# lucadellalib/audiocodecs

Hardware: AMD Instinct MI355X
Metric: encode+decode audio-sec/s, EnCodec-24k 8cb (higher is better)
Workload: dtype f32 (GEMM-shaped kernels and LSTM products: operands as two scaled fp16 planes, 3 partial products, fp32 accumulate -- split16.h)

## Files before the change

audiocodecs_amd/csrc/ac_api.hip:

```cpp
#include "core.h"
#include "tap_route.h"

extern "C" {

int ac_version(void) { return 400; }

int ac_create(const ac_config* cfg, ac_handle** out) {
    if (!cfg || !out) return AC_EINVAL;
    *out = nullptr;
    if (cfg->struct_size != (int32_t)sizeof(ac_config)) return AC_EINVAL;
    if (cfg->num_ratios < 1 || cfg->num_ratios > AC_MAX_RATIOS || cfg->num_filters < 1 || cfg->hidden_size < 16 ||
        cfg->hidden_size % 16 || cfg->compress < 1 || cfg->num_lstm_layers < 1 || cfg->num_lstm_layers > 2 || cfg->codebook_size % 32 ||
        cfg->codebook_size < 16 || cfg->num_quantizers < 1 || cfg->kernel_size < 1 || cfg->kernel_size > 8 ||
        cfg->last_kernel_size < 1 || cfg->last_kernel_size > 8 || cfg->residual_kernel_size < 1 || cfg->residual_kernel_size > 8)
        return AC_EINVAL;
    int ndev = 0;
    if (hipGetDeviceCount(&ndev) != hipSuccess || ndev <= cfg->device || cfg->device < 0) return AC_ENODEV;
    ac_handle* h = new (std::nothrow) ac_handle();
    if (!h) return AC_ENOMEM;
    h->cfg = *cfg;
    h->hop = 1;
    for (int i = 0; i < cfg->num_ratios; ++i) h->hop *= cfg->upsampling_ratios[i];
    h->D = cfg->num_filters << cfg->num_ratios;
    *out = h;
    return AC_OK;
}







static std::string wavtok_key(const std::string& name) {
    static const std::string pre = "feature_extractor.encodec.encoder.model.";
    if (name.compare(0, pre.size(), pre) != 0) return name;
    std::string k = "encoder.layers." + name.substr(pre.size());
    const size_t cc = k.find(".conv.conv.");
    if (cc != std::string::npos) k = k.substr(0, cc) + ".conv." + k.substr(cc + 11);
    auto ends = [&](const char* sfx) { const size_t n = std::strlen(sfx); return k.size() >= n && k.compare(k.size() - n, n, sfx) == 0; };
    if (ends(".weight_g")) k = k.substr(0, k.size() - 9) + ".parametrizations.weight.original0";
    else if (ends(".weight_v")) k = k.substr(0, k.size() - 9) + ".parametrizations.weight.original1";
    return k;
}

int ac_load_weights(ac_handle* h, const char* name, const void* host_ptr, size_t bytes) {
    if (!h || !name || !host_ptr) return h ? fail(h, AC_EINVAL, "null argument") : AC_EINVAL;
    if (h->finalized) return fail(h, AC_ESTATE, "handle already finalized");
    if (bytes % 4) return fail(h, AC_EINVAL, "tensor '%s': byte size %zu is not a multiple of 4", name, bytes);
    const float* f = static_cast<const float*>(host_ptr);
    h->host[h->arch == ARCH_WAVTOK ? wavtok_key(name) : std::string(name)].assign(f, f + bytes / 4);
    return AC_OK;
}



static void latch_dev_switches(ac_handle* h) {
    auto num = [](const char* name, int dflt) { const char* v = std::getenv(name); return v && *v ? std::atoi(v) : dflt; };
    const char* e = std::getenv("AC_TAP_EPI");
    h->dev.tap_epi_staged = e && std::strcmp(e, "staged") == 0;
    h->dev.tap_dil = num("AC_TAP_DIL", 1);
    h->dev.tap_stagger = num("AC_TAP_STAGGER", 0);
    h->dev.tap_pick = num("AC_TAP_PICK", -1);
    h->dev.tap8 = num("AC_TAP8", -1);
    h->dev.tap8_form = num("AC_TAP8_FORM", 0);
    h->dev.tap8_spread = num("AC_TAP8_SPREAD", 1);
#ifdef AC_DEVELOPER
    h->dev.rb6_dbg = num("AC_RB6_DBG", 0);
    h->dev.lstm_dbg = num("AC_LSTM_DBG", 0);
#endif
    h->dev.rb_stream = num("AC_RB_STREAM", 1);
    h->dev.chain_stream = num("AC_CHAIN_STREAM", 1);
    h->dev.rb128_stream = num("AC_RB128_STREAM", 1);
    h->dev.rb256_fused = num("AC_RB256_FUSED", 1);
    h->dev.front_seg = std::max(0, num("AC_FRONT_SEG", 0));
    h->dev.tail_seg = std::max(0, num("AC_TAIL_SEG", 0));
    h->dev.front_ldspad = std::max(0, num("AC_FRONT_LDSPAD", 0));
    h->dev.lstm_fuse_in = num("AC_LSTM_FUSE_IN", 1);
    const char* r = std::getenv("AC_RVQ");
    h->dev.rvq_exact = r && std::strcmp(r, "fp32") == 0;
    h->dev.prof_detail = num("AC_PROF_DETAIL", 0);
    h->dev.head_seq = num("AC_HEAD_SEQ", 0);
    h->dev.attn_exact = num("AC_ATTN_EXACT", 0);
    h->dev.dac_unit = num("AC_DAC_UNIT", 1);
    h->dev.mimi_tail = num("AC_MIMI_TAIL", 1);
    h->dev.mstream_skinny = num("AC_MSTREAM_SKINNY", -1);
}

int ac_debug_set(ac_handle* h, const char* key, int value) {
    if (!h || !key) return AC_EINVAL;
    struct { const char* k; int* v; } tab[] = {
        {"tap_epi_staged", &h->dev.tap_epi_staged}, {"tap_dil", &h->dev.tap_dil}, {"tap_stagger", &h->dev.tap_stagger}, {"tap_pick", &h->dev.tap_pick}, {"tap8", &h->dev.tap8}, {"tap8_form", &h->dev.tap8_form}, {"tap8_spread", &h->dev.tap8_spread},
        {"rb6_dbg", &h->dev.rb6_dbg}, {"rb_stream", &h->dev.rb_stream}, {"chain_stream", &h->dev.chain_stream}, {"rb128_stream", &h->dev.rb128_stream}, {"rb256_fused", &h->dev.rb256_fused}, {"front_seg", &h->dev.front_seg}, {"tail_seg", &h->dev.tail_seg}, {"front_ldspad", &h->dev.front_ldspad},
        {"lstm_dbg", &h->dev.lstm_dbg}, {"lstm_fuse_in", &h->dev.lstm_fuse_in}, {"rvq_exact", &h->dev.rvq_exact}, {"prof_detail", &h->dev.prof_detail}, {"head_seq", &h->dev.head_seq}, {"attn_exact", &h->dev.attn_exact}, {"dac_unit", &h->dev.dac_unit}, {"mimi_tail", &h->dev.mimi_tail},
        {"mstream_skinny", &h->dev.mstream_skinny},
    };
#ifndef AC_DEVELOPER
    if (std::strcmp(key, "rb6_dbg") == 0 || std::strcmp(key, "lstm_dbg") == 0)
        return fail(h, AC_EINVAL, "ac_debug_set('%s'): a developer-build switch (timing modes with wrong results / fault injection); this is the product library", key);
#endif
    if (!h->finalized) return fail(h, AC_ESTATE, "ac_debug_set('%s'): the switches are latched by ac_finalize; set them afterwards", key);
    for (auto& t : tab)
        if (std::strcmp(t.k, key) == 0) {
            const bool nonneg = t.v == &h->dev.front_seg || t.v == &h->dev.tail_seg || t.v == &h->dev.front_ldspad || t.v == &h->dev.tap_stagger;
            if (nonneg && value < 0) return fail(h, AC_EINVAL, "ac_debug_set('%s', %d): the value must be >= 0", key, value);
            if (t.v == &h->dev.front_ldspad && value > 16384) return fail(h, AC_EINVAL, "ac_debug_set('front_ldspad', %d): at most 16384 bytes", value);
            if (t.v == &h->dev.tap8_form && (value < 0 || value > 5)) return fail(h, AC_EINVAL, "ac_debug_set('tap8_form', %d): 0 (cost model) .. 5", value);
            *t.v = value;
            return AC_OK;
        }
    return fail(h, AC_EINVAL, "ac_debug_set: unknown switch '%s'", key);
}

int ac_set_precision(ac_handle* h, int precision) {
    if (!h) return AC_EINVAL;
    if (h->finalized) return fail(h, AC_ESTATE, "ac_set_precision must precede ac_finalize (weights are packed for one arithmetic)");
    if (precision != AC_PRECISION_FP32 && precision != AC_PRECISION_FP32_EXACT) return fail(h, AC_EINVAL, "unknown precision %d", precision);
    h->precision = precision;
    return AC_OK;
}

int ac_finalize(ac_handle* h) {
    if (!h) return AC_EINVAL;
    if (h->finalized) return fail(h, AC_ESTATE, "handle already finalized");
    {
        int pr = h->precision;
        if (pr < 0) {
            const char* gm = std::getenv("AC_GEMM");
            if (gm && *gm && std::strcmp(gm, "fp32") != 0 && std::strcmp(gm, "split16") != 0)
                return fail(h, AC_EINVAL, "AC_GEMM=%s: unknown arithmetic (fp32 = exact fp32 products, split16 or unset = the default)", gm);
            pr = gm && std::strcmp(gm, "fp32") == 0 ? AC_PRECISION_FP32_EXACT : AC_PRECISION_FP32;
        }
        const char* fz = std::getenv("AC_FUSE");
        h->fuse_chains = !(fz && fz[0] == '0');
        latch_dev_switches(h);
        h->gemm_fp32 = pr == AC_PRECISION_FP32_EXACT;
    }
    if (h->arch == ARCH_MIMI) {
        Packer pk{h};
        if (int rc = mimi_finalize(h, pk)) return rc;
        return upload_blob(h, pk, h->mcfg.device);
    }
    if (h->arch == ARCH_DAC) {
        Packer pk{h};
        if (int rc = dac_finalize(h, pk)) return rc;
        return upload_blob(h, pk, h->dcfg.device);
    }
    if (h->arch == ARCH_WAVTOK) {
        Packer pk{h};
        if (int rc = wavtok_finalize(h, pk)) return rc;
        return upload_blob(h, pk, h->wcfg.device);
    }
    if (h->arch == ARCH_SPK) {
        Packer pk{h};
        if (int rc = spk_finalize(h, pk)) return rc;
        return upload_blob(h, pk, h->scfg.device);
    }
    if (h->arch == ARCH_LM) {
        Packer pk{h};
        if (int rc = lm_finalize(h, pk)) return rc;
        return upload_blob(h, pk, h->lcfg.device);
    }
    const ac_config& c = h->cfg;
    Arch a = make_arch(c);
    Packer pk{h};
    h->has_enc = h->has_dec = false;
    for (const auto& kv : h->host) {
        if (kv.first.compare(0, 8, "encoder.") == 0) h->has_enc = true;
        if (kv.first.compare(0, 8, "decoder.") == 0) h->has_dec = true;
    }
    bool has_q = false;
    for (const auto& kv : h->host) has_q = has_q || kv.first.compare(0, 10, "quantizer.") == 0;
    if (!h->has_enc && !h->has_dec && !has_q) return fail(h, AC_ESTATE, "no encoder.*, decoder.* or quantizer.* tensor was loaded");
    bool ok = true;
    h->enc_rb.resize(c.num_ratios);
    h->enc_down.resize(c.num_ratios);
    h->dec_up.resize(c.num_ratios);
    h->dec_rb.resize(c.num_ratios);
    if (h->has_enc) {
        ok = pk.conv(a.enc_stem, h->enc_stem);
        for (int i = 0; ok && i < c.num_ratios; ++i) {
            ok = ok && pk.resblock(a.enc_rb3[i], a.enc_rb1[i], a.enc_rbs[i], h->enc_rb[i]);
            ok = ok && pk.conv(a.enc_down[i], h->enc_down[i]);
        }
        ok = ok && pk.lstm(a.enc_lstm, a.D, c.num_lstm_layers, h->enc_lstm);
        ok = ok && pk.conv(a.enc_final, h->enc_final);
        if (ok) pk.chain_bounds(h->enc_stem, h->enc_rb[0], h->enc_down[0], h->enc_front);
        if (ok) pk.stream_enc(h->enc_stem, h->enc_rb[0], h->enc_down[0], h->simg);
    }
    if (h->has_dec) {
        ok = ok && pk.conv(a.dec_first, h->dec_first);
        ok = ok && pk.lstm(a.dec_lstm, a.D, c.num_lstm_layers, h->dec_lstm);
        for (int i = 0; ok && i < c.num_ratios; ++i) {
            ok = ok && pk.convtr(a.dec_up[i], h->dec_up[i]);
            ok = ok && pk.resblock(a.dec_rb3[i], a.dec_rb1[i], a.dec_rbs[i], h->dec_rb[i]);
        }
        ok = ok && pk.conv(a.dec_head, h->dec_head);
        if (ok) pk.tail_bounds(h->dec_up[c.num_ratios - 1], h->dec_rb[c.num_ratios - 1], h->dec_head, h->dec_tail);
        if (ok) pk.stream_dec(h->dec_up[c.num_ratios - 1], h->dec_rb[c.num_ratios - 1], h->dec_head, h->simg);
    }
    if (!ok) return pk.rc;
    const int C = c.codebook_size, H = c.hidden_size, Q = c.num_quantizers;
    h->cb_plain = pk.reserve((size_t)Q * C * H);
    h->cb_packed = pk.reserve((size_t)Q * C * H);
    h->cb_ee = pk.reserve((size_t)Q * C);
    for (int q = 0; q < Q; ++q) {
        const std::vector<float>* e = pk.get("quantizer.layers." + std::to_string(q) + ".codebook.embed", (size_t)C * H);
        if (!e) return pk.rc;
        std::copy(e->begin(), e->end(), pk.blob.begin() + h->cb_plain + (size_t)q * C * H);
        for (int code = 0; code < C; ++code) {
            double ss = 0.0;
            for (int d = 0; d < H; ++d) ss += (double)(*e)[(size_t)code * H + d] * (*e)[(size_t)code * H + d];
            pk.blob[h->cb_ee + (size_t)q * C + code] = (float)ss;
        }
        const int HV = H / 16;
        for (int ct = 0; ct < C / 16; ++ct)
            for (int v = 0; v < HV; ++v)
                for (int lane = 0; lane < 64; ++lane)
                    for (int u = 0; u < 4; ++u)
                        pk.blob[h->cb_packed + (size_t)q * C * H + (((size_t)ct * HV + v) * 64 + lane) * 4 + u] =
                            (*e)[(size_t)(ct * 16 + (lane & 15)) * H + v * 16 + 4 * (lane >> 4) + u];
    }
    if (pk.use16() && H % 32 == 0 && H / 16 == 8) pk.pack_cb16(h->cb_plain, Q, C, H, &h->cb16, &h->cb16_inv);
    return upload_blob(h, pk, c.device);
}

int ac_num_frames(const ac_handle* h, int T) {
    if (!h || T < 1) return AC_EINVAL;
    if (h->arch == ARCH_MIMI) return cdiv(mimi_num_frames25(h->mcfg, T), h->mcfg.resample_stride);
    if (h->arch == ARCH_DAC) return dac_num_frames(h->dcfg, T);
    long long L = T;
    for (int r = h->cfg.num_ratios - 1; r >= 0; --r) L = (L + h->cfg.upsampling_ratios[r] - 1) / h->cfg.upsampling_ratios[r];
    return (int)L;
}
long long ac_num_samples(const ac_handle* h, int N) {
    if (!h || N < 1) return AC_EINVAL;
    return h->arch == ARCH_DAC ? dac_num_samples(h->dcfg, N) : (long long)N * h->hop;
}
int ac_hop_length(const ac_handle* h) { return h ? h->hop : AC_EINVAL; }
int ac_hidden_size(const ac_handle* h) {
    if (!h) return AC_EINVAL;
    return h->arch == ARCH_MIMI ? h->mcfg.hidden_size : h->arch == ARCH_DAC ? h->dac.H : h->cfg.hidden_size;
}
int ac_codebook_dim(const ac_handle* h) {
    if (!h) return AC_EINVAL;
    return h->arch == ARCH_MIMI ? h->mcfg.codebook_dim : h->arch == ARCH_DAC ? DAC_CODE_DIM : h->cfg.hidden_size;
}
// ... 524 lines not shown
```

audiocodecs_amd/csrc/core.h:

```cpp
#pragma once
#include <hip/hip_runtime.h>

#include <algorithm>
#include <cmath>
#include <cstdarg>
#include <cstdio>
#include <cstdlib>
#include <cstring>
#include <map>
#include <string>
#include <vector>

#include "../../include/audiocodecs_amd.h"
#include "lstm_consts.h"
#include "rvq_types.h"
#include "split16.h"
#include "tap_gemm.h"

using namespace ac;

namespace ac {
constexpr int THIN_MAXK = 8;
struct RbFused6Params;
}

namespace acimpl {


struct ConvSpec {
    std::string prefix;
    int transposed, cin, cout, k, s;
};

struct PackedGemm {
    size_t w_off = 0, b_off = 0;
    int N = 0, Ktot = 0;
    bool has_bias = true;
};

struct ResBlockPlan {
    int C;
    PackedGemm c3;
    PackedGemm fused;
    size_t w3f_off = 0, wff_off = 0;
    size_t winv3_off = 0, winvf_off = 0;
    size_t w3p_off = 0, wfp_off = 0;
    float hb0 = 0.f, hb1 = 0.f;
    bool has6 = false;
    bool hb256 = false;
};

struct LstmPlan {
    int D, layers;
    std::vector<PackedGemm> ih;
    std::vector<size_t> hh_off;
    std::vector<size_t> ihpk_off;
    size_t persist_off = 0;
    size_t persist16_off = 0;
    size_t persist16_inv = 0;
    bool has_persist = false;
};

struct MimiTfLayer {
    PackedGemm qkv, o, fc1, fc2;
    size_t ln1_w = 0, ln1_b = 0, ln2_w = 0, ln2_b = 0, sc_a = 0, sc_m = 0;
};

struct MimiPlan {
    PackedGemm enc_stem, enc_final, down, dec_first, dec_head;
    std::vector<ResBlockPlan> enc_rb, dec_rb;
    std::vector<PackedGemm> enc_down, dec_up;
    std::vector<MimiTfLayer> enc_tf, dec_tf;
    size_t up_w = 0;
    PackedGemm in_proj;
    PackedGemm out_proj;
    size_t cb_plain = 0, cb_packed = 0, cb_ee = 0;
    size_t cb16 = 0, cb16_inv = 0;
    size_t rope_cos = 0, rope_sin = 0;
    int rope_T = 0;
    int D = 0;
    struct StreamM { size_t stem_f = 0, stem_inv = 0, head_f = 0, head_inv = 0; float sb0 = 0.f, sb1 = 0.f, fb0 = 0.f, fb1h = 0.f; bool stem_ok = false, head_ok = false; } sm;
};

struct DacResUnitPlan {
    PackedGemm c7, c1;
    size_t a1 = 0, a1i = 0, a2 = 0, a2i = 0;
    int dil = 1;
};

struct DacBlockPlan {
    int C = 0, stride = 1;
    std::vector<DacResUnitPlan> ru;
    size_t a = 0, ai = 0;
    PackedGemm conv;
};

struct DacPlan {
    PackedGemm enc_stem, enc_final, dec_first, dec_head, in_proj0;
    std::vector<DacBlockPlan> enc, dec;
    size_t enc_a = 0, enc_ai = 0, dec_a = 0, dec_ai = 0;
    size_t win = 0, bin = 0, wout = 0, bout = 0, cb = 0, cbn = 0, c2 = 0, proj = 0;
    int H = 0;
};

struct WtResnetPlan {
    size_t n1w = 0, n1b = 0, n2w = 0, n2b = 0;
    PackedGemm c1, c2;
};
struct WtCnxPlan {
    size_t dww = 0, dwb = 0, sc = 0, sh = 0, gamma = 0;
    PackedGemm p1, p2;
};
struct WavtokPlan {
    PackedGemm embed, qkv, proj, head, istft;
    WtResnetPlan rn[4];
    size_t an_w = 0, an_b = 0;
    size_t g5w = 0, g5b = 0;
    size_t nsc = 0, nsh = 0;
    size_t flw = 0, flb = 0;
    size_t w2 = 0;
    std::vector<WtCnxPlan> cnx;
    int bins = 0, npad = 0, hop_pad = 0, taps = 0;
    bool vocos = false;
    int tables = 1;
};

struct SpkTfLayer {
    PackedGemm qkv, o, fc1, fc2;
    size_t ln1_w = 0, ln1_b = 0, ln2_w = 0, ln2_b = 0;
    size_t gate_w = 0, gate_b = 0, gate_c = 0;
};

struct SpkPlan {
    size_t stem_w = 0, gn_w = 0, gn_b = 0;
    std::vector<PackedGemm> conv;
    size_t fp_ln_w = 0, fp_ln_b = 0, enc_ln_w = 0, enc_ln_b = 0;
    PackedGemm fp;
    size_t pos_img = 0, pos_inv = 0, pos_b = 0;
    std::vector<SpkTfLayer> tf;
    size_t bias_tab = 0;
    int R = 0;
    std::vector<float> lw;
    PackedGemm proj, fe;
    std::vector<PackedGemm> tdnn;
    int shrink = 0;
};

struct LmLayer {
    size_t an = 0, fn = 0, wqkv = 0, wo = 0, w1 = 0, w3 = 0, w2 = 0;
};

struct LmPlan {
    size_t emb = 0, prompt = 0, norm = 0, head = 0;
    size_t rope_cos = 0, rope_sin = 0;
    std::vector<LmLayer> layers;
};

struct ProfRec {
    int name_id;
    int count;
    hipEvent_t e0, e1;
    double flops, bytes;
};


}
using namespace acimpl;

enum { ARCH_ENCODEC = 0, ARCH_MIMI = 1, ARCH_DAC = 2, ARCH_WAVTOK = 3, ARCH_SPK = 4, ARCH_LM = 5 };

struct ac_handle {
    int arch = ARCH_ENCODEC;
    ac_config cfg{};
    ac_mimi_config mcfg{};
    MimiPlan mimi;
    ac_dac_config dcfg{};
    DacPlan dac;
    ac_wavtok_config wcfg{};
    WavtokPlan wt;
    ac_spk_config scfg{};
    SpkPlan spk;
    ac_lm_config lcfg{};
    LmPlan lm;
    std::string err;
    std::map<std::string, std::vector<float>> host;
    bool finalized = false;
    float* blob = nullptr;
    size_t blob_floats = 0;
    int hop = 1, D = 0;
    PackedGemm enc_stem, enc_final;
    std::vector<ResBlockPlan> enc_rb;
    std::vector<PackedGemm> enc_down;
    LstmPlan enc_lstm, dec_lstm;
    PackedGemm dec_first, dec_head;
    std::vector<PackedGemm> dec_up;
    std::vector<ResBlockPlan> dec_rb;
    size_t cb_plain = 0, cb_packed = 0, cb_ee = 0;
    size_t cb16 = 0, cb16_inv = 0;
    struct ChainBounds { float sb0 = 0.f, sb1 = 0.f, fb0 = 0.f, fb1h = 0.f, fb1x = 0.f; bool ok = false; } enc_front, dec_tail;
    struct StreamImgs { size_t stem_f = 0, stem_inv = 0, down_f = 0, down_inv = 0, up_f = 0, up_inv = 0, head_f = 0, head_inv = 0; bool enc_ok = false, dec_ok = false; } simg;
    struct DevSwitches {
        int tap_epi_staged = 0;
        int tap_dil = 1;
        int tap_stagger = 0;
        int tap_pick = -1;
        int tap8 = -1;
        int tap8_form = 0;
        int tap8_spread = 1;
        int rb6_dbg = 0;
        int rb_stream = 1;
        int rb256_fused = 1;
        int rb128_stream = 1;
        int chain_stream = 1;
        int front_seg = 0, tail_seg = 0;
        int front_ldspad = 0;
        int lstm_dbg = 0;
        int lstm_fuse_in = 1;
        int rvq_exact = 0;
        int prof_detail = 0;
        int attn_exact = 0;
        int dac_unit = 1;
        int mimi_tail = 1;
        int head_seq = 0;
        int mstream_skinny = -1;
    } dev;
    bool fuse_chains = true;
    float* dbg = nullptr;
    size_t dbg_cap = 0, dbg_used = 0;
    std::vector<const void*> lds_opted;
    std::map<size_t, size_t> w6_of;
    std::map<size_t, size_t> t6_of;
    std::map<size_t, size_t> t6inv_of;
    bool noncausal = false;
    bool has_enc = true, has_dec = true;
    bool gemm_fp32 = false;
    std::map<size_t, size_t> winv_of;
    std::map<const void*, int> mimi_streams;
    std::map<const void*, int> mimi_dstreams;
    struct EStreamReg {
        int B;
        std::vector<uint8_t> fresh;
    };
    std::map<const void*, EStreamReg> encodec_streams, encodec_dstreams;
    unsigned* amax_buf = nullptr;
    int amax_B = 0, amax_next = 0;
    unsigned* row_buf = nullptr;
    size_t row_cap = 0, row_next = 0;
    void* own_pool = nullptr;
    size_t own_pool_rows = 0;
    int precision = -1;
    unsigned* lp_ctl = nullptr;
    int num_cus = 0;
    bool lstm_step_only = false;
    unsigned long long* clk_dev = nullptr;
    unsigned* sticky = nullptr;
    unsigned* sticky_dev = nullptr;
    bool prof = false;
    bool prof_detail = false;
    std::vector<ProfRec> recs;
    std::vector<std::string> prof_names;
    std::vector<hipEvent_t> ev_pool;
    size_t ev_used = 0;
};

namespace acimpl {

int fail(ac_handle* h, int code, const char* fmt, ...);


#define HIPCHK(h, call)                                                                         \
    do {                                                                                        \
        hipError_t e_ = (call);                                                                 \
        if (e_ != hipSuccess) return fail(h, AC_EHIP, "%s failed: %s", #call, hipGetErrorString(e_)); \
    } while (0)


inline int cdiv(int a, int b) { return (a + b - 1) / b; }

int ensure_lds(ac_handle* h, const void* func, size_t bytes);

inline size_t align_up(size_t v, size_t a) { return (v + a - 1) / a * a; }


struct Arch {
    std::vector<ConvSpec> enc_rb3, enc_rb1, enc_rbs, enc_down;
    ConvSpec enc_stem, enc_final, dec_first, dec_head;
    std::vector<ConvSpec> dec_up, dec_rb3, dec_rb1, dec_rbs;
    std::string enc_lstm, dec_lstm;
    int D;
};

Arch make_arch(const ac_config& c);


struct Packer {
    ac_handle* h;
    std::vector<float> blob;
    int rc = AC_OK;

    const std::vector<float>* get(const std::string& name, size_t n) {
        auto it = h->host.find(name);
        if (it == h->host.end()) {
            rc = fail(h, AC_ESTATE, "missing tensor '%s'", name.c_str());
            return nullptr;
        }
        if (it->second.size() != n) {
            rc = fail(h, AC_EINVAL, "tensor '%s' has %zu elements, expected %zu", name.c_str(), it->second.size(), n);
            return nullptr;
        }
        return &it->second;
    }
    bool weight(const ConvSpec& s, std::vector<float>& w) {
        const size_t n = (size_t)s.cin * s.cout * s.k;
        auto it = h->host.find(s.prefix + ".weight");
        if (it != h->host.end()) {
            if (it->second.size() != n) {
                rc = fail(h, AC_EINVAL, "tensor '%s.weight' has %zu elements, expected %zu", s.prefix.c_str(), it->second.size(), n);
                return false;
            }
            w = it->second;
            return true;
        }
        const int d0 = s.transposed ? s.cin : s.cout;
        const std::vector<float>* g = get(s.prefix + ".parametrizations.weight.original0", d0);
        if (!g) return false;
        const std::vector<float>* v = get(s.prefix + ".parametrizations.weight.original1", n);
        if (!v) return false;
        w.resize(n);
        const size_t inner = n / d0;
        for (int i = 0; i < d0; ++i) {
            double ss = 0.0;
            for (size_t j = 0; j < inner; ++j) ss += (double)(*v)[i * inner + j] * (*v)[i * inner + j];
            const float scale = (*g)[i] / (float)std::sqrt(ss);
            for (size_t j = 0; j < inner; ++j) w[i * inner + j] = (*v)[i * inner + j] * scale;
        }
        return true;
    }
    size_t reserve(size_t n) {
        const size_t off = align_up(blob.size(), 64);
        blob.resize(off + n, 0.f);
        return off;
    }
    static uint16_t bf16_rn(float v) {
        uint32_t b;
        std::memcpy(&b, &v, 4);
        if ((b & 0x7f800000u) == 0x7f800000u) return (uint16_t)(b >> 16);
        return (uint16_t)((b + 0x7fffu + ((b >> 16) & 1u)) >> 16);
    }
    static uint16_t f16_rn(float f) {
        uint32_t x;
        std::memcpy(&x, &f, 4);
        const uint16_t sign = (uint16_t)((x >> 16) & 0x8000u);
        x &= 0x7fffffffu;
        if (x >= 0x7f800000u) return (uint16_t)(sign | 0x7c00u | (x > 0x7f800000u ? 0x200u : 0u));
        if (x >= 0x477ff000u) return (uint16_t)(sign | 0x7c00u);
        if (x <= 0x33000000u) return sign;
        const int e = (int)(x >> 23) - 127;
        const uint32_t m = (x & 0x7fffffu) | 0x800000u;
        const int shift = e >= -14 ? 13 : 13 + (-14 - e);
        uint32_t q = m >> shift;
        const uint32_t rem = m & ((1u << shift) - 1u), half = 1u << (shift - 1);
        if (rem > half || (rem == half && (q & 1u))) ++q;
        if (e >= -14) return (uint16_t)(sign | (uint16_t)(((uint32_t)(e + 15) << 10) + (q - 0x400u)));
        return (uint16_t)(sign | (uint16_t)q);
    }
    static float f16_f32(uint16_t hbits) {
        const int e = (hbits >> 10) & 31, m = hbits & 0x3ff;
        float v;
        if (e == 0) v = std::ldexp((float)m, -24);
        else if (e == 31) v = m ? NAN : INFINITY;
// ... 223 lines not shown
            for (int k = 0; k < 7; ++k) k7[k] = k;
            sm.stem_f = frag16(stem.w_off, 64, 7, k7, &sm.stem_inv);
            sm.sb0 = sm.sb1 = 0.f;
            for (int n = 0; n < 64; ++n) {
                double l1 = 0.0;
                for (int k = 0; k < 7; ++k) l1 += std::fabs((double)blob[stem.w_off + (size_t)n * 7 + k]);
                sm.sb1 = std::max(sm.sb1, (float)(l1 * 1.000001));
                sm.sb0 = std::max(sm.sb0, std::fabs(blob[stem.b_off + n]));
            }
            sm.stem_ok = true;
        }
        if (head.N == 1 && head_k >= 1 && head_k <= 8 && head.Ktot == head_k * 64 && head.has_bias && dec_rb.C == 64 && dec_rb.w3p_off && dec_rb.fused.Ktot == 32) {
            std::vector<int> kh(64);
            for (int k = 0; k < 64; ++k) kh[k] = k;
            const size_t pad = reserve(16 * 64);
            for (int i = 0; i < 16 * 64; ++i) blob[pad + i] = i < head_k * 64 ? blob[head.w_off + i] : 0.f;
            sm.head_f = frag16(pad, 16, 64, perm32(kh), &sm.head_inv);
            sm.fb0 = sm.fb1h = 0.f;
            for (int n = 0; n < 64; ++n) {
                double lh = 0.0;
                for (int k = 0; k < 32; ++k) lh += std::fabs((double)blob[dec_rb.fused.w_off + (size_t)n * 32 + k]);
                sm.fb1h = std::max(sm.fb1h, (float)(lh * 1.000001));
                sm.fb0 = std::max(sm.fb0, std::fabs(blob[dec_rb.fused.b_off + n]));
            }
            sm.head_ok = true;
        }
    }
    void stream_enc(const PackedGemm& stem, const ResBlockPlan& rb, const PackedGemm& down, ac_handle::StreamImgs& si) {
        si.enc_ok = false;
        if (!use16() || !h->enc_front.ok || !rb.w3p_off || stem.N != 32 || stem.Ktot != 7 || down.N != 64 || down.Ktot != 128) return;
        std::vector<int> k7(32, -1), kd(128);
        for (int k = 0; k < 7; ++k) k7[k] = k;
        for (int k = 0; k < 128; ++k) kd[k] = k;
        si.stem_f = frag16(stem.w_off, 32, 7, k7, &si.stem_inv);
        si.down_f = frag16(down.w_off, 64, 128, perm32(kd), &si.down_inv);
        si.enc_ok = true;
    }
    void stream_dec(const PackedGemm& up, const ResBlockPlan& rb, const PackedGemm& head, ac_handle::StreamImgs& si) {
        si.dec_ok = false;
        if (!use16() || !h->dec_tail.ok || !rb.w3p_off || up.N != 64 || up.Ktot != 128 || head.N != 1 || head.Ktot != 7 * 32) return;
        std::vector<int> ku(128), kh(32);
        for (int k = 0; k < 128; ++k) ku[k] = k;
        for (int k = 0; k < 32; ++k) kh[k] = k;
        si.up_f = frag16(up.w_off, 64, 128, perm32(ku), &si.up_inv);
        const size_t pad = reserve(16 * 32);
        for (int i = 0; i < 16 * 32; ++i) blob[pad + i] = i < 7 * 32 ? blob[head.w_off + i] : 0.f;
        si.head_f = frag16(pad, 16, 32, perm32(kh), &si.head_inv);
        si.dec_ok = true;
    }
    void chain_bounds(const PackedGemm& stem, const ResBlockPlan& rb, const PackedGemm& down, ac_handle::ChainBounds& cb) {
        cb.ok = false;
        if (!use16() || !rb.has6 || !rb.winv3_off || rb.C != 32 || stem.N != 32 || !h->t6inv_of.count(down.w_off)) return;
        const int hid = rb.C / 2;
        cb.sb0 = cb.sb1 = cb.fb0 = cb.fb1h = cb.fb1x = 0.f;
        for (int n = 0; n < stem.N; ++n) {
            double l1 = 0.0;
            for (int k = 0; k < stem.Ktot; ++k) l1 += std::fabs((double)blob[stem.w_off + (size_t)n * stem.Ktot + k]);
            cb.sb1 = std::max(cb.sb1, (float)(l1 * 1.000001));
            cb.sb0 = std::max(cb.sb0, std::fabs(blob[stem.b_off + n]));
        }
        for (int n = 0; n < rb.C; ++n) {
            double lh = 0.0, lx = 0.0;
            for (int k = 0; k < hid; ++k) lh += std::fabs((double)blob[rb.fused.w_off + (size_t)n * rb.fused.Ktot + k]);
            for (int k = hid; k < rb.fused.Ktot; ++k) lx += std::fabs((double)blob[rb.fused.w_off + (size_t)n * rb.fused.Ktot + k]);
            cb.fb1h = std::max(cb.fb1h, (float)(lh * 1.000001));
            cb.fb1x = std::max(cb.fb1x, (float)(lx * 1.000001));
            cb.fb0 = std::max(cb.fb0, std::fabs(blob[rb.fused.b_off + n]));
        }
        cb.ok = true;
    }
    void tail_bounds(const PackedGemm& up, const ResBlockPlan& rb, const PackedGemm& head, ac_handle::ChainBounds& cb) {
        cb.ok = false;
        if (!use16() || !rb.has6 || !rb.winv3_off || rb.C != 32 || up.N != 64 || up.Ktot != 128 || !h->t6inv_of.count(up.w_off) || head.N != 1 || head.Ktot != 7 * 32) return;
        cb.sb0 = cb.sb1 = 0.f;
        for (int n = 0; n < up.N; ++n) {
            double l1 = 0.0;
            for (int k = 0; k < up.Ktot; ++k) l1 += std::fabs((double)blob[up.w_off + (size_t)n * up.Ktot + k]);
            cb.sb1 = std::max(cb.sb1, (float)(l1 * 1.000001));
            cb.sb0 = std::max(cb.sb0, std::fabs(blob[up.b_off + n]));
        }
        const int hid = rb.C / 2;
        cb.fb0 = cb.fb1h = cb.fb1x = 0.f;
        for (int n = 0; n < rb.C; ++n) {
            double lh = 0.0, lx = 0.0;
            for (int k = 0; k < hid; ++k) lh += std::fabs((double)blob[rb.fused.w_off + (size_t)n * rb.fused.Ktot + k]);
            for (int k = hid; k < rb.fused.Ktot; ++k) lx += std::fabs((double)blob[rb.fused.w_off + (size_t)n * rb.fused.Ktot + k]);
            cb.fb1h = std::max(cb.fb1h, (float)(lh * 1.000001));
            cb.fb1x = std::max(cb.fb1x, (float)(lx * 1.000001));
            cb.fb0 = std::max(cb.fb0, std::fabs(blob[rb.fused.b_off + n]));
        }
        cb.ok = true;
    }
    bool lstm(const std::string& prefix, int D, int layers, LstmPlan& lp) {
        lp.D = D;
        lp.layers = layers;
        for (int l = 0; l < layers; ++l) {
            const std::string sfx = "_l" + std::to_string(l);
            const std::vector<float>* wih = get(prefix + ".weight_ih" + sfx, (size_t)4 * D * D);
            const std::vector<float>* whh = get(prefix + ".weight_hh" + sfx, (size_t)4 * D * D);
            const std::vector<float>* bih = get(prefix + ".bias_ih" + sfx, (size_t)4 * D);
            const std::vector<float>* bhh = get(prefix + ".bias_hh" + sfx, (size_t)4 * D);
            if (!wih || !whh || !bih || !bhh) return false;
            PackedGemm g;
            g.N = 4 * D;
            g.Ktot = D;
            g.w_off = reserve((size_t)4 * D * D);
            std::copy(wih->begin(), wih->end(), blob.begin() + g.w_off);
            g.b_off = reserve((size_t)4 * D);
            for (int n = 0; n < 4 * D; ++n) blob[g.b_off + n] = (*bih)[n] + (*bhh)[n];
            if (l == 0) pack6(g);
            lp.ih.push_back(g);
            const size_t off = reserve((size_t)4 * D * D);
            for (int ug = 0; ug < D / 4; ++ug)
                for (int ks = 0; ks < D / 16; ++ks)
                    for (int lane = 0; lane < 64; ++lane)
                        for (int u = 0; u < 4; ++u) {
                            const int j = lane & 15, kq = lane >> 4;
                            const int row = (j >> 2) * D + ug * 4 + (j & 3);
                            const int k = ks * 16 + 4 * kq + u;
                            blob[off + (((size_t)ug * (D / 16) + ks) * 64 + lane) * 4 + u] = (*whh)[(size_t)row * D + k];
                        }
            lp.hh_off.push_back(off);
            const size_t off2 = reserve((size_t)4 * D * D);
            for (int ug = 0; ug < D / 4; ++ug)
                for (int ks = 0; ks < D / 16; ++ks)
                    for (int lane = 0; lane < 64; ++lane)
                        for (int u = 0; u < 4; ++u) {
                            const int j = lane & 15, kq = lane >> 4;
                            const int row = (j >> 2) * D + ug * 4 + (j & 3);
                            const int k = ks * 16 + 4 * kq + u;
                            blob[off2 + (((size_t)ug * (D / 16) + ks) * 64 + lane) * 4 + u] = (*wih)[(size_t)row * D + k];
                        }
            lp.ihpk_off.push_back(off2);
        }
        if (D == LP_D && layers == 2) {
            const std::vector<float>* mats[3] = {get(prefix + ".weight_hh_l0", (size_t)4 * D * D), get(prefix + ".weight_ih_l1", (size_t)4 * D * D),
                                                 get(prefix + ".weight_hh_l1", (size_t)4 * D * D)};
            const size_t mat = (size_t)LP_SLICES * 4 * 4 * 8 * 256;
            lp.persist_off = reserve(3 * mat);
            for (int m = 0; m < 3; ++m)
                for (int idx = 0; idx < LP_SLICES; ++idx)
                    for (int w = 0; w < 4; ++w)
                        for (int n = 0; n < 4; ++n)
                            for (int ks = 0; ks < 8; ++ks)
                                for (int lane = 0; lane < 64; ++lane)
                                    for (int e = 0; e < 4; ++e)
                                        blob[lp.persist_off + m * mat + ((((size_t)idx * 4 + w) * 4 + n) * 8 + ks) * 256 + lane * 4 + e] =
                                            (*mats[m])[(size_t)(n * D + idx * 16 + (lane & 15)) * D + (w * 8 + ks) * 16 + 4 * (lane >> 4) + e];
            const std::vector<float>* mats6[4] = {mats[0], mats[1], mats[2], get(prefix + ".weight_ih_l0", (size_t)4 * D * D)};
            if (use16()) {
                const size_t mat16 = (size_t)LP_SLICES * 4 * 4 * 4 * 2 * 512;
                lp.persist16_off = reserve((4 * mat16 + 1) / 2);
                lp.persist16_inv = reserve((size_t)2 * 4 * D);
                std::vector<int> sc((size_t)2 * 4 * D);
                const int layer_of[4] = {0, 1, 1, 0};
                for (int l = 0; l < 2; ++l)
                    for (int row = 0; row < 4 * D; ++row) {
                        uint32_t mx = 0;
                        for (int m = 0; m < 4; ++m)
                            if (layer_of[m] == l)
                                for (int k = 0; k < D; ++k) {
                                    uint32_t b;
                                    std::memcpy(&b, &(*mats6[m])[(size_t)row * D + k], 4);
                                    mx = std::max(mx, b & 0x7fffffffu);
                                }
                        sc[(size_t)l * 4 * D + row] = s16_exponent(mx, 40);
                        blob[lp.persist16_inv + (size_t)l * 4 * D + row] = s16_pow2(-sc[(size_t)l * 4 * D + row]);
                    }
                std::vector<uint16_t> pl16(4 * mat16);
                for (int m = 0; m < 4; ++m)
                    for (int idx = 0; idx < LP_SLICES; ++idx)
                        for (int w = 0; w < 4; ++w)
                            for (int n = 0; n < 4; ++n)
                                for (int ks = 0; ks < 4; ++ks)
                                    for (int lane = 0; lane < 64; ++lane)
                                        for (int e = 0; e < 8; ++e) {
                                            const int row = n * D + idx * 16 + (lane & 15);
                                            uint16_t t[3];
                                            split16h((*mats6[m])[(size_t)row * D + w * 128 + ks * 32 + 8 * (lane >> 4) + e], sc[(size_t)layer_of[m] * 4 * D + row], t);
                                            const size_t base = m * mat16 + (((((size_t)idx * 4 + w) * 4 + n) * 4 + ks) * 2) * 512 + (size_t)lane * 8 + e;
                                            pl16[base] = t[0];
                                            pl16[base + 512] = t[1];
                                        }
                std::memcpy(&blob[lp.persist16_off], pl16.data(), pl16.size() * 2);
            }
            lp.has_persist = true;
        }
        return true;
    }
};


struct Act {
    const float* p;
    long long bs, ts;
    int L, C;
    const unsigned* amax = nullptr;
    int amax_n = 0;
};

int prof_name(ac_handle* h, const char* nm);

hipEvent_t next_event(ac_handle* h);


struct ProfScope {
    ac_handle* h;
    hipStream_t st;
    ProfRec r{};
    bool on;
    ProfScope(ac_handle* h_, hipStream_t st_, const char* nm, double flops, double bytes, int count = 1)
        : h(h_), st(st_), on(h_->prof) {
        if (!on) return;
        r.name_id = prof_name(h, nm);
        r.count = count;
        r.flops = flops;
        r.bytes = bytes;
        r.e0 = next_event(h);
        r.e1 = next_event(h);
        (void)hipEventRecord(r.e0, st);
    }
    ~ProfScope() {
        if (!on) return;
        (void)hipEventRecord(r.e1, st);
        h->recs.push_back(r);
    }
};


constexpr int AMAX_SLOTS = 512;

inline size_t pool_bytes(int pool_B, size_t rows) {
    return (size_t)AMAX_SLOTS * std::max(pool_B, 1) * AMAX_STRIDE * 4 + 8 * align_up(std::max<size_t>(rows, 64), 64) * 4 + 256;
}

void pool_bind(ac_handle* h, void* mem, int pool_B, size_t rows);

int amax_begin(ac_handle* h, hipStream_t st, int B);

unsigned* amax_new(ac_handle* h);

const unsigned* amax_of(ac_handle* h, hipStream_t st, const float* x, long long bs, long long ts, int L, int C, int B, const unsigned* known);

unsigned* rowmax_new(ac_handle* h, hipStream_t st, long long rows, bool zero);

const unsigned* amax_plus(ac_handle* h, hipStream_t st, const Act& x, float add, int B);

TapSeg make_seg(const Act& x, int s, int J, int pad , int extra, int kofs, const float* rel_len, int left = -1, int right = 0);


inline bool aligned16(const void* p) { return (reinterpret_cast<uintptr_t>(p) & 15) == 0; }

int run_tap(ac_handle* h, hipStream_t st, TapGemmParams& p);


struct Out {
    float* raw = nullptr;
    float* elu = nullptr;
};

struct Act2 {
    Act raw{}, elu{};
};

int try_thin6(ac_handle* h, hipStream_t st, const PackedGemm& g, const Act& x, int width, int edge, Out out, int B, const unsigned** amax_out = nullptr);

int conv_fwd(ac_handle* h, hipStream_t st, const PackedGemm& g, const Act& x, int k, int s, const float* rel_len, Out out,
             long long out_bs, long long out_rs, int B, Act2* y);

int convtr_fwd(ac_handle* h, hipStream_t st, const PackedGemm& g, const Act& x, int s, Out out, int B, Act2* y);

bool rb128_ok(const ac_handle* h, const ResBlockPlan& rb);

int resblock_fwd(ac_handle* h, hipStream_t st, const ResBlockPlan& rb, const Act2& x, float* hbuf, Out out, int B, Act2* y);
bool rb256_ok(const ac_handle* h, const ResBlockPlan& rb, int L);

bool thin_ok(const ac_config& c, int k);

int thin_stem(ac_handle* h, hipStream_t st, const PackedGemm& g, int F, int k, int pad, const float* sig, const float* rel_len, int B, int T,
              Out out, Act2* y, int padl = -1, const float* alpha = nullptr, const float* alpha_inv = nullptr, int Lp = -1);

int stem_fwd(ac_handle* h, hipStream_t st, const float* sig, const float* rel_len, int B, int T, Out out, Act2* y);

int thin_head(ac_handle* h, hipStream_t st, const PackedGemm& g, int F, int k, int pad, const Act& x, int B, float* sig, int padl = -1,
              int tanh_out = 0);

int head_fwd(ac_handle* h, hipStream_t st, const Act& x, int B, float* sig);

bool enc_front_ok(const ac_handle* h, int T);

int enc_front_fwd(ac_handle* h, hipStream_t st, const float* sig, const float* rel_len, int B, int T, float* y, float* dbg_x0, float* dbg_y1, Act2* out);

bool dec_tail_ok(const ac_handle* h, const Act& xe);

int dec_tail_fwd(ac_handle* h, hipStream_t st, const Act& xe, int B, float* sig, float* dbg_u, float* dbg_v);

void capture(ac_handle* h, hipStream_t st, const Act& a, int B);


struct LstmWs {
    float *gin, *gin1, *hseq0, *hseq1, *c;
};

int lstm_fwd(ac_handle* h, hipStream_t st, const LstmPlan& lp, const Act& x, const LstmWs& ws, Out out, int B, Act2* y);

int rvq_encode_fwd(ac_handle* h, hipStream_t st, const float* feats, int F, int K, long long* toks);

int rvq_decode_fwd(ac_handle* h, hipStream_t st, const long long* toks, int F, int K, float* out);


constexpr int NACT = 6;


struct Workspace {
    size_t act_floats = 0;
    size_t gin = 0, hseq = 0, c = 0;
    int pool_B = 0;
    size_t pool_rows = 0;
    size_t total_bytes = 0;
};

inline void add_pool(Workspace& w, int pool_B, size_t rows) {
    w.pool_B = pool_B;
    w.pool_rows = rows;
    w.total_bytes += pool_bytes(pool_B, rows);
}

Workspace plan_ws(const ac_handle* h, int B, int T_in , int N_frames , bool enc);


struct WsPtrs {
    float* act[NACT];
    bool used[NACT];
    LstmWs lstm;
    float* take() {
        for (int i = 0; i < NACT; ++i)
            if (!used[i]) { used[i] = true; return act[i]; }
        return nullptr;
    }
    void give(const float* p) {
        for (int i = 0; i < NACT; ++i)
            if (act[i] == p) used[i] = false;
    }
    void give(const Act2& a) { give(a.raw.p); give(a.elu.p); }
};

int carve(ac_handle* h, const Workspace& w, void* ws, size_t ws_bytes, WsPtrs* o);

int check_ready(ac_handle* h);

int check_len(ac_handle* h, long long samples);

int encoder_fwd(ac_handle* h, hipStream_t st, const float* sig, const float* rel_len, int B, int T, float* feats, WsPtrs& ws);

int decoder_fwd(ac_handle* h, hipStream_t st, const long long* toks, int B, int N, int K, float* sig, WsPtrs& ws);

bool rb64_identity_head_fwd(ac_handle* h, hipStream_t st, const ResBlockPlan& rb, const Act2& x, const PackedGemm& head, int head_k, float* sig, int B, int* rc);
int enc_stream_fwd(ac_handle* h, hipStream_t st, const float* sig, const float* rel_len, int B, int T, float* y, float* dbg_x0, float* dbg_y1, const unsigned* amax_sig, unsigned* amax_out);
int dec_stream_fwd(ac_handle* h, hipStream_t st, const Act& xe, int B, float* sig, float* dbg_u, float* dbg_v, const unsigned* amax_x);
int launch_rb_stream6m(ac_handle* h, hipStream_t st, const ResBlockPlan& rb, const float* xr, const float* sig, int B, int L, Out out, float* head_y, int head_k,
                       const unsigned* amax_in, unsigned* amax_out);
int launch_rb_stream128m(ac_handle* h, hipStream_t st, RbFused6Params& p, const ResBlockPlan& rb, bool sc, Out out, int B);
int launch_rb_stream6(ac_handle* h, hipStream_t st, RbFused6Params& p, const ResBlockPlan& rb, bool sc, Out out, int B);
int rb64_identity_fwd(ac_handle* h, hipStream_t st, const ResBlockPlan& rb, const Act2& x, Out out, int B, const unsigned** amax_out);
int rb128_identity_fwd(ac_handle* h, hipStream_t st, const ResBlockPlan& rb, const Act2& x, Out out, int B, const unsigned** amax_out);
int rvq_encode_cdist_launch(ac_handle* h, hipStream_t st, const RvqEncParams& p, unsigned blocks, const _Float16* epk16 = nullptr, const float* einv = nullptr);
void rvq_decode_launch(hipStream_t st, const RvqDecParams& p, unsigned blocks);
void amax_fill_launch(hipStream_t st, unsigned* slot, unsigned bits, int B);
int resample_launch(const float* x, int B, int L, const float* kern, int n, int o, int taps, int width, float* y, int L_out, hipStream_t st);
constexpr int RSTREAM_MAX_TAPS = 8192;
long long resample_stream_groups(long long total, int o, int width);
long long resample_stream_out_len(long long consumed, int L, int n, int o, int width, int finish);
size_t resample_stream_state_bytes(int B, int taps);
int resample_stream_reset_launch(void* state, int B, int n, int o, int taps, int width, hipStream_t st);
int resample_stream_push_launch(void* state, const float* x, long long x_pitch, int B, int L, long long consumed, const float* kern, int n, int o, int taps,
                                int width, float* y, long long y_pitch, int m, int finish, hipStream_t st);
int resample_stream_reset_slots_launch(void* state, int B, int n, int o, int taps, int width, const int* slots_dev, int rows, hipStream_t st);
int resample_stream_push_slots_launch(void* state, int B, const int* slots_dev, const long long* consumed_dev, int rows, const float* x, long long x_pitch,
                                      int L, const float* kern, int n, int o, int taps, int width, float* y, long long y_pitch, int m, int finish,
                                      hipStream_t st);

struct Epi {
    const float* scale = nullptr;
    const float* res = nullptr;
    long long res_bs = 0, res_rs = 0;
    int gelu = 0;
    const unsigned* rowmax_in = nullptr;
    const unsigned** rowmax_out = nullptr;
};

int mimi_finalize(ac_handle* h, Packer& pk);
Workspace mimi_plan_ws(const ac_handle* h, int B, int T_in, int N_frames, bool enc);
int mimi_num_frames25(const ac_mimi_config& c, long long T);
int mimi_encoder_fwd(ac_handle* h, hipStream_t st, const float* sig, int B, int T, float* feats, WsPtrs& ws);
int mimi_decoder_fwd(ac_handle* h, hipStream_t st, const float* qfeats, int B, int N, float* sig, WsPtrs& ws);
int mimi_linear(ac_handle* h, hipStream_t st, const PackedGemm& g, const float* x, long long rows, int cin, int x_pitch, int kofs,
                float* y, int y_pitch, const Epi& epi = Epi{});
int layernorm_fwd(ac_handle* h, hipStream_t st, const float* x, size_t w_off, size_t b_off, float* y, long long rows, int H, float eps,
                  const unsigned** rows_out = nullptr);
int mimi_rvq_encode(ac_handle* h, hipStream_t st, const float* proj, int F, int K, long long* toks);
int mimi_rvq_decode(ac_handle* h, hipStream_t st, const long long* toks, int F, int K, float* qsum, float* qfeats);
int dac_finalize(ac_handle* h, Packer& pk);
Workspace dac_plan_ws(const ac_handle* h, int B, long long T_in, long long N_frames, bool enc);
int dac_chunk_clips(const ac_handle* h, int B, long long T_in, long long N_frames, bool enc);
int dac_num_frames(const ac_dac_config& c, long long T);
long long dac_num_samples(const ac_dac_config& c, long long N);
int dac_encoder_fwd(ac_handle* h, hipStream_t st, const float* sig, int B, int T, float* z, WsPtrs& ws);
int dac_decoder_fwd(ac_handle* h, hipStream_t st, const float* zq, int B, int N, float* sig, WsPtrs& ws);
int dac_latent_proj(ac_handle* h, hipStream_t st, const float* z, int N, int nb, float* zlat);
int dac_vq_encode(ac_handle* h, hipStream_t st, const float* z, int F, int K, long long* toks, float* qsum);
int dac_from_codes(ac_handle* h, hipStream_t st, const long long* toks, int F, int K, float* zq);
int wavtok_finalize(ac_handle* h, Packer& pk);
Workspace wavtok_plan_ws(const ac_handle* h, int B, int T_in, int N_frames, bool enc);
int wavtok_decoder_fwd(ac_handle* h, hipStream_t st, const float* feats, int B, int N, float* sig, WsPtrs& ws);
int spk_finalize(ac_handle* h, Packer& pk);
int lm_finalize(ac_handle* h, Packer& pk);
int upload_blob(ac_handle* h, Packer& pk, int device);
constexpr int DAC_CODE_DIM = 8;

}
```

audiocodecs_amd/csrc/core.hip:

```cpp
#include "core.h"
#include "split16_kernels.h"
#include "lstm.h"
#include "lstm_persist.h"
#include "lstm_persist16.h"
#include "rvq.h"
#include "rvq16.h"
#include "tap_gemm4.h"
#include "tap_gemm6.h"
#include "tap_gemm8.h"
#include "tap_route.h"
#include "thin.h"
#include "rb_fused.h"
#include "rb_fused6.h"
#include "thin_conv6.h"
#include "rb_fused6_128.h"
#include "rb256_fused.h"
#include "enc_front.h"
#include "dec_tail.h"

namespace acimpl {


int fail(ac_handle* h, int code, const char* fmt, ...) {
    char buf[1024];
// ... 56 lines not shown


int prof_name(ac_handle* h, const char* nm) {
    for (size_t i = 0; i < h->prof_names.size(); ++i)
        if (h->prof_names[i] == nm) return (int)i;
    h->prof_names.push_back(nm);
    return (int)h->prof_names.size() - 1;
}


hipEvent_t next_event(ac_handle* h) {
    if (h->ev_used == h->ev_pool.size()) {
        hipEvent_t e;
        (void)hipEventCreate(&e);
        h->ev_pool.push_back(e);
    }
    return h->ev_pool[h->ev_used++];
}

void pool_bind(ac_handle* h, void* mem, int pool_B, size_t rows) {
    h->amax_buf = reinterpret_cast<unsigned*>(mem);
    h->amax_B = mem ? std::max(pool_B, 1) : 0;
    h->amax_next = 0;
    h->row_buf = mem ? h->amax_buf + (size_t)AMAX_SLOTS * h->amax_B * AMAX_STRIDE : nullptr;
    h->row_cap = mem ? 8 * align_up(std::max<size_t>(rows, 64), 64) : 0;
    h->row_next = 0;
}


static void zero_words(hipStream_t st, unsigned* p, size_t words) {
    const size_t n16 = words / 4;
    const unsigned grid = (unsigned)std::min<size_t>(std::max<size_t>((n16 + 255) / 256, 1), 2048);
    hipLaunchKernelGGL(zero16_kernel, dim3(grid), dim3(256), 0, st, reinterpret_cast<s16_f32x4*>(p), n16);
}


int amax_begin(ac_handle* h, hipStream_t st, int B) {
    h->amax_next = 0;
    if (h->gemm_fp32 || !h->amax_buf) return AC_OK;
    if (B > h->amax_B) return fail(h, AC_ENOMEM, "workspace pool holds amax slots for %d clips, the pass has %d", h->amax_B, B);
    zero_words(st, h->amax_buf, (size_t)AMAX_SLOTS * h->amax_B * AMAX_STRIDE);
    HIPCHK(h, hipGetLastError());
    return AC_OK;
}

unsigned* amax_new(ac_handle* h) {
    if (h->gemm_fp32 || !h->amax_buf || h->amax_next >= AMAX_SLOTS) return nullptr;
    return h->amax_buf + (size_t)(h->amax_next++) * h->amax_B * AMAX_STRIDE;
}

const unsigned* amax_of(ac_handle* h, hipStream_t st, const float* x, long long bs, long long ts, int L, int C, int B, const unsigned* known) {
    if (known) return known;
    if (B > h->amax_B) return nullptr;
    unsigned* slot = amax_new(h);
    if (!slot) return nullptr;
    const long long n = (long long)L * C;
    const int gx = (int)std::max<long long>(1, std::min<long long>((n / 4 + 256 * 8 - 1) / (256 * 8), std::max(4, 8192 / std::max(1, B))));
    ProfScope ps(h, st, "amax_kernel", 0.0, (double)B * n * 4.0);
    hipLaunchKernelGGL(amax_kernel, dim3(gx, B), dim3(256), 0, st, x, bs, ts, L, C, slot);
    return slot;
}


unsigned* rowmax_new(ac_handle* h, hipStream_t st, long long rows, bool zero) {
    const size_t need = ((size_t)rows + 63) / 64 * 64;
    if (!h->row_buf || need > h->row_cap) return nullptr;
    if (h->row_next + need > h->row_cap) h->row_next = 0;
    unsigned* r = h->row_buf + h->row_next;
    h->row_next += need;
    if (zero) {
        zero_words(st, r, need);
        if (hipGetLastError() != hipSuccess) return nullptr;
    }
    return r;
}


const unsigned* amax_plus(ac_handle* h, hipStream_t st, const Act& x, float add, int B) {
    if (!x.amax || x.amax_n != B) return nullptr;
    unsigned* slot = amax_new(h);
    if (!slot) return nullptr;
    hipLaunchKernelGGL(amax_add_kernel, dim3(cdiv(B, 64)), dim3(64), 0, st, x.amax, add, slot, B);
    return slot;
}



template <int WGM, int WGN, int WM, int WN>
static int launch_tap(ac_handle* h, hipStream_t st, TapGemmParams p, TapFamily f, const char* name, double flops, double bytes) {
    ProfScope ps(h, st, name, flops, bytes);
    if (f == TapFamily::tap4) {
        using Cfg = Tap4Cfg<WGM, WGN, WM, WN>;
        p.mtiles = cdiv(p.M, Cfg::BM);
        p.ntiles = cdiv(p.N, Cfg::BN);
        if (int rc = ensure_lds(h, reinterpret_cast<const void*>(tap_gemm4_kernel<WGM, WGN, WM, WN>), Cfg::lds_bytes)) return rc;
        const long long blocks = (long long)p.B * p.mtiles * p.ntiles;
        hipLaunchKernelGGL((tap_gemm4_kernel<WGM, WGN, WM, WN>), dim3((unsigned)blocks), dim3(Cfg::NT), Cfg::lds_bytes, st, p);
        return AC_OK;
    }
    constexpr int BM = WGM * WM * 16, BN = WGN * WN * 16;
    p.mtiles = cdiv(p.M, BM);
    p.ntiles = cdiv(p.N, BN);
    const size_t lds = tap_gemm_lds_bytes<WGM, WGN, WM, WN>();
    const long long blocks = (long long)p.B * p.mtiles * p.ntiles;
    if (f == TapFamily::vec) hipLaunchKernelGGL((tap_gemm_kernel<WGM, WGN, WM, WN, true>), dim3((unsigned)blocks), dim3(WGM * WGN * 64), lds, st, p);
    else hipLaunchKernelGGL((tap_gemm_kernel<WGM, WGN, WM, WN, false>), dim3((unsigned)blocks), dim3(WGM * WGN * 64), lds, st, p);
    return AC_OK;
}

static int launch_tap_fp32(ac_handle* h, hipStream_t st, const TapGemmParams& p, const TapRoute& r, const char* name, double flops, double bytes) {
    switch (r.key()) {
    case tap_key(4, 1, 2, 1): return launch_tap<4, 1, 2, 1>(h, st, p, r.family, name, flops, bytes);
    case tap_key(4, 1, 2, 2): return launch_tap<4, 1, 2, 2>(h, st, p, r.family, name, flops, bytes);
    case tap_key(2, 2, 2, 2): return launch_tap<2, 2, 2, 2>(h, st, p, r.family, name, flops, bytes);
    case tap_key(2, 2, 4, 3): return launch_tap<2, 2, 4, 3>(h, st, p, r.family, name, flops, bytes);
    case tap_key(2, 2, 4, 4): return launch_tap<2, 2, 4, 4>(h, st, p, r.family, name, flops, bytes);
    }
    return fail(h, AC_EINVAL, "run_tap: no instantiation of %s", r.name);
}

template <int WGM, int WGN, int WMT, int WN, int HALO>
static int launch_tap6(ac_handle* h, hipStream_t st, TapGemmParams& p, const __bf16* w6, const char* name, double flops, double bytes) {
    using Cfg = Tap6Cfg<WGM, WGN, WMT, WN, HALO>;
    p.mtiles = cdiv(p.M, Cfg::BM);
    p.ntiles = p.N / Cfg::BN;
    const long long blocks = (long long)p.B * p.mtiles * p.ntiles;
    if (int rc = ensure_lds(h, reinterpret_cast<const void*>(tap_gemm6_kernel<WGM, WGN, WMT, WN, 2, HALO>), Cfg::lds_for(2))) return rc;
    ProfScope ps(h, st, name, flops, bytes);
    hipLaunchKernelGGL((tap_gemm6_kernel<WGM, WGN, WMT, WN, 2, HALO>), dim3((unsigned)blocks), dim3(Cfg::NT), Cfg::lds_for(2), st, p, w6);
    return AC_OK;
}

static int launch_tap6_family(ac_handle* h, hipStream_t st, TapGemmParams& p, const TapRoute& r, const __bf16* w6, const char* name, double flops, double bytes) {
    if (r.family == TapFamily::tap6_dil) {
        switch (r.key()) {
        case tap_key(1, 4, 4, 2): return launch_tap6<1, 4, 4, 2, T6_DIL_HALO>(h, st, p, w6, name, flops, bytes);
        case tap_key(1, 4, 4, 1): return launch_tap6<1, 4, 4, 1, T6_DIL_HALO>(h, st, p, w6, name, flops, bytes);
        case tap_key(2, 2, 2, 3): return launch_tap6<2, 2, 2, 3, T6_DIL_HALO>(h, st, p, w6, name, flops, bytes);
        case tap_key(4, 1, 1, 3): return launch_tap6<4, 1, 1, 3, T6_DIL_HALO>(h, st, p, w6, name, flops, bytes);
        }
    } else {
        switch (r.key()) {
        case tap_key(1, 4, 4, 2): return launch_tap6<1, 4, 4, 2, 7>(h, st, p, w6, name, flops, bytes);
        case tap_key(1, 8, 4, 1): return launch_tap6<1, 8, 4, 1, 7>(h, st, p, w6, name, flops, bytes);
        case tap_key(1, 4, 4, 1): return launch_tap6<1, 4, 4, 1, 7>(h, st, p, w6, name, flops, bytes);
        case tap_key(2, 2, 2, 3): return launch_tap6<2, 2, 2, 3, 7>(h, st, p, w6, name, flops, bytes);
        case tap_key(4, 1, 1, 3): return launch_tap6<4, 1, 1, 3, 7>(h, st, p, w6, name, flops, bytes);
        case tap_key(2, 2, 2, 1): return launch_tap6<2, 2, 2, 1, 7>(h, st, p, w6, name, flops, bytes);
        }
    }
    return fail(h, AC_EINVAL, "run_tap: no instantiation of %s", r.name);
}

template <int WGM, int WGN, int WMT, int WN, bool RM, bool J1, bool SP>
static int launch_tap8(ac_handle* h, hipStream_t st, TapGemmParams& p, const __bf16* w6, const char* name, double flops, double bytes) {
    using Cfg = Tap8Cfg<WGM, WGN, WMT, WN>;
    p.mtiles = cdiv(p.M, Cfg::BM);
    p.ntiles = p.N / Cfg::BN;
    const long long blocks = (long long)p.B * p.mtiles * p.ntiles;
    ProfScope ps(h, st, name, flops, bytes);
    if (int rc = ensure_lds(h, reinterpret_cast<const void*>(tap_gemm8_kernel<WGM, WGN, WMT, WN, RM, J1, SP>), Cfg::lds_bytes)) return rc;
    hipLaunchKernelGGL((tap_gemm8_kernel<WGM, WGN, WMT, WN, RM, J1, SP>), dim3((unsigned)blocks), dim3(Cfg::NT), Cfg::lds_bytes, st, p, w6);
    return AC_OK;
}

static int launch_tap8_family(ac_handle* h, hipStream_t st, TapGemmParams& p, const TapRoute& r, const __bf16* w6, const char* name, double flops, double bytes) {
    constexpr int RJ = TK_RM | TK_J1, J = TK_J1, S = TK_SPREAD;
    switch (r.key()) {
    case tap_key(2, 4, 4, 2, RJ): return launch_tap8<2, 4, 4, 2, true, true, false>(h, st, p, w6, name, flops, bytes);
    case tap_key(2, 4, 4, 2, RJ | S): return launch_tap8<2, 4, 4, 2, true, true, true>(h, st, p, w6, name, flops, bytes);
    case tap_key(2, 4, 4, 2, J): return launch_tap8<2, 4, 4, 2, false, true, false>(h, st, p, w6, name, flops, bytes);
    case tap_key(2, 4, 4, 2, J | S): return launch_tap8<2, 4, 4, 2, false, true, true>(h, st, p, w6, name, flops, bytes);
    case tap_key(2, 4, 4, 2): return launch_tap8<2, 4, 4, 2, false, false, false>(h, st, p, w6, name, flops, bytes);
    case tap_key(2, 4, 4, 2, S): return launch_tap8<2, 4, 4, 2, false, false, true>(h, st, p, w6, name, flops, bytes);
    case tap_key(2, 4, 2, 2, RJ): return launch_tap8<2, 4, 2, 2, true, true, false>(h, st, p, w6, name, flops, bytes);
    case tap_key(2, 4, 2, 2, RJ | S): return launch_tap8<2, 4, 2, 2, true, true, true>(h, st, p, w6, name, flops, bytes);
    case tap_key(2, 4, 2, 2, J): return launch_tap8<2, 4, 2, 2, false, true, false>(h, st, p, w6, name, flops, bytes);
    case tap_key(2, 4, 2, 2, J | S): return launch_tap8<2, 4, 2, 2, false, true, true>(h, st, p, w6, name, flops, bytes);
    case tap_key(2, 4, 2, 2): return launch_tap8<2, 4, 2, 2, false, false, false>(h, st, p, w6, name, flops, bytes);
    case tap_key(2, 4, 2, 2, S): return launch_tap8<2, 4, 2, 2, false, false, true>(h, st, p, w6, name, flops, bytes);
    case tap_key(4, 2, 2, 2, RJ): return launch_tap8<4, 2, 2, 2, true, true, false>(h, st, p, w6, name, flops, bytes);
    case tap_key(4, 2, 2, 2, RJ | S): return launch_tap8<4, 2, 2, 2, true, true, true>(h, st, p, w6, name, flops, bytes);
    case tap_key(4, 2, 2, 2, J): return launch_tap8<4, 2, 2, 2, false, true, false>(h, st, p, w6, name, flops, bytes);
    case tap_key(4, 2, 2, 2, J | S): return launch_tap8<4, 2, 2, 2, false, true, true>(h, st, p, w6, name, flops, bytes);
    case tap_key(4, 2, 2, 2): return launch_tap8<4, 2, 2, 2, false, false, false>(h, st, p, w6, name, flops, bytes);
    case tap_key(4, 2, 2, 2, S): return launch_tap8<4, 2, 2, 2, false, false, true>(h, st, p, w6, name, flops, bytes);
    }
    return fail(h, AC_EINVAL, "run_tap: no instantiation of %s", r.name);
}


TapSeg make_seg(const Act& x, int s, int J, int pad , int extra, int kofs, const float* rel_len, int left, int right) {
    TapSeg g{};
    g.x = x.p;
    g.amax = x.amax;
    g.amax_n = x.amax_n;
    g.bs = x.bs;
    g.ts = x.ts;
    g.rel_len = rel_len;
    g.L = x.L;
    g.cin = x.C;
    g.cin_shift = -1;
    for (int sh = 0; sh < 30; ++sh)
        if ((1 << sh) == x.C) g.cin_shift = sh;
    g.s = s;
    g.J = J;
    const int pad_left = left < 0 ? (J - 1) * s : left;
    const int max_pad = std::max(pad_left, right + extra);
    g.Lp = (pad == PAD_REFLECT && x.L <= max_pad) ? max_pad + 1 : x.L;
    g.lim = pad != PAD_ZERO ? x.L + right + extra : x.L;
    g.reflect = pad;
    g.elu = 0;
    g.kofs = kofs;
    g.pad = pad_left;
    g.dil = 1;
    return g;
}


int run_tap(ac_handle* h, hipStream_t st, TapGemmParams& p) {
    const auto w6_it = h->w6_of.find((size_t)(p.w - h->blob));
    const auto iv = h->winv_of.find((size_t)(p.w - h->blob));
    TapRouteInputs in;
    in.w6 = w6_it != h->w6_of.end();
    in.winv = iv != h->winv_of.end();
    in.want_rowmode = p.amax_rows != 0;
    in.want_rows = p.amax_out_rows != nullptr;
    in.gemm_fp32 = h->gemm_fp32;
    const TapRoute r = route_tap(p, in, h->dev);
    if (r.reject_taps) return fail(h, AC_EINVAL, "conv with %d taps exceeds the kernel limit of 8", r.reject_taps);
    double kk = 0, inb = 0;
    for (int i = 0; i < p.nseg; ++i) {
        kk += (double)p.seg[i].J * p.seg[i].s * p.seg[i].cin;
        inb += (double)p.B * p.seg[i].L * p.seg[i].cin * 4.0;
    }
    const double flops = 2.0 * p.B * (double)p.M * p.N * kk;
    const double bytes = inb + (double)p.B * p.M * p.N * 4.0 * ((p.y ? 1 : 0) + (p.y_elu ? 1 : 0)) + (double)p.N * p.Ktot * 4.0;
    std::string name = r.name;
    if (h->prof && h->prof_detail && r.family != TapFamily::scalar && r.family != TapFamily::vec) {
        char shape[64];
        std::snprintf(shape, sizeof shape, " B%d M%d N%d K%d J%d s%d%s", p.B, p.M, p.N, (int)kk, p.seg[0].J, p.seg[0].s, p.seg[0].dil == 1 ? "" : p.seg[0].dil == 3 ? " d3" : " d9");
        name += shape;
    }
    p.amax_out_rows = nullptr;
    p.amax_rows = 0;
    int rc;
    if (r.family == TapFamily::scalar || r.family == TapFamily::vec || r.family == TapFamily::tap4) {
        rc = launch_tap_fp32(h, st, p, r, name.c_str(), flops, bytes);
    } else {
        p.clk = h->clk_dev;
#ifdef T6_TRACE
        if (const char* ts = std::getenv("AC_TRACE_SHAPE")) {
            int tm = 0, tn = 0, tk = 0;
            if (std::sscanf(ts, "%d,%d,%d", &tm, &tn, &tk) == 3 && !((tm == 0 || tm == p.M) && tn == p.N && tk == (int)kk)) p.clk = nullptr;
        }
#endif
        if (r.rowmode) {
            TapSeg& sg = p.seg[0];
            if (!(sg.amax && sg.amax_n == -p.M)) {
                unsigned* rm = rowmax_new(h, st, p.M, false);
                if (!rm) return fail(h, AC_ENOMEM, "the workspace pool's row ring is too small for %d rows", p.M);
                ProfScope ps(h, st, "rowmax_kernel", 0.0, (double)p.M * sg.cin * 4.0);
                hipLaunchKernelGGL(rowmax_kernel, dim3((unsigned)cdiv(p.M, 4)), dim3(256), 0, st, sg.x, sg.ts, (long long)p.M, sg.cin, rm);
                sg.amax = rm;
            }
            p.amax_rows = 1;
            p.winv = h->blob + iv->second;
            if (r.rows_out) {
                p.amax_out_rows = rowmax_new(h, st, p.M, true);
                if (!p.amax_out_rows) return fail(h, AC_ENOMEM, "the workspace pool's row ring is too small for %d rows", p.M);
            }
        } else if (in.winv) {
            for (int i = 0; i < p.nseg; ++i) {
                TapSeg& sg = p.seg[i];
                sg.amax = amax_of(h, st, sg.x, sg.bs, sg.ts, sg.L, sg.cin, p.B, sg.amax_n == p.B ? sg.amax : nullptr);
                if (!sg.amax) return fail(h, AC_ESTATE, "out of amax slots (split16.h)");
            }
            p.winv = h->blob + iv->second;
            p.amax_out = amax_new(h);
            p.epi_direct = r.epi_direct;
        }
        p.stagger = h->dev.tap_stagger;
        const __bf16* w6 = reinterpret_cast<const __bf16*>(h->blob + w6_it->second);
        rc = r.family == TapFamily::tap8 ? launch_tap8_family(h, st, p, r, w6, name.c_str(), flops, bytes)
                                         : launch_tap6_family(h, st, p, r, w6, name.c_str(), flops, bytes);
    }
    if (rc) return rc;
    HIPCHK(h, hipGetLastError());
    return AC_OK;
}


int try_thin6(ac_handle* h, hipStream_t st, const PackedGemm& g, const Act& x, int width, int edge, Out out, int B, const unsigned** amax_out) {
    if (h->gemm_fp32 || g.N != 64 || g.Ktot != 128 || x.C != width || x.ts != width || x.bs != (long long)x.L * width ||
        (x.L * width) % 64 || x.L * width < 256 || !aligned16(x.p) || (long long)x.L * width * 4 > 0x70000000LL)
        return 1;
    auto it = h->t6_of.find(g.w_off);
    if (it == h->t6_of.end()) return 1;
    ThinConv6Params p{};
    p.x = x.p;
    p.wf = reinterpret_cast<const __bf16*>(h->blob + it->second);
    p.bias = h->blob + g.b_off;
    p.y = out.raw;
    p.y_elu = out.elu;
    p.B = B;
    p.Ls = x.L * width / 64;
    p.M = p.Ls;
    p.ntiles = cdiv(p.M, T6_BM);
    p.edge = edge;
    const bool s16 = h->t6inv_of.count(g.w_off) != 0;
    if (s16) {
        p.amax_in = amax_of(h, st, x.p, x.bs, x.ts, x.L, x.C, B, x.amax_n == B ? x.amax : nullptr);
        if (!p.amax_in) return fail(h, AC_ESTATE, "out of amax slots (split16.h)");
        p.winv = h->blob + h->t6inv_of[g.w_off];
        p.amax_out = amax_new(h);
        if (amax_out) *amax_out = p.amax_out;
    }
    const long long total = (long long)B * p.ntiles;
    const int grid = (int)std::min<long long>(total, 4 * 256);
    ProfScope ps(h, st, "thin_conv6_kernel<2>", 2.0 * B * p.M * 64.0 * 128.0,
                 (double)B * p.M * 256.0 * (1 + (out.raw ? 1 : 0) + (out.elu ? 1 : 0)));
    hipLaunchKernelGGL(thin_conv6_kernel<2>, dim3(grid), dim3(256), T6_LDS, st, p);
    return AC_OK;
}


int conv_fwd(ac_handle* h, hipStream_t st, const PackedGemm& g, const Act& x, int k, int s, const float* rel_len, Out out,
             long long out_bs, long long out_rs, int B, Act2* y) {
    const int M = cdiv(x.L, s);
    const int extra = M * s - x.L;
    if (s == 2 && k == 4 && !rel_len && extra == 0 && x.L >= 4 && out_rs == 64 && out_bs == (long long)M * 64 && !h->noncausal) {
        const unsigned* am = nullptr;
        const int rc = try_thin6(h, st, g, x, 32, 1, out, B, &am);
        if (rc <= 0) {
            if (y && !rc) {
                y->raw = Act{out.raw, out_bs, out_rs, M, g.N, am, B};
                y->elu = Act{out.elu, out_bs, out_rs, M, g.N, am, B};
            }
            if (!rc) HIPCHK(h, hipGetLastError());
            return rc;
        }
    }
    TapGemmParams p{};
    p.nseg = 1;
    if (s != 1 && k != 2 * s) return fail(h, AC_EINVAL, "strided conv needs kernel == 2*stride (got k=%d, s=%d)", k, s);
    if (h->noncausal) {
        const int total = k - s, right = total / 2;
        p.seg[0] = make_seg(x, s, s == 1 ? k : 2, PAD_REFLECT, extra, 0, rel_len, total - right, right);
    } else {
        p.seg[0] = make_seg(x, s, s == 1 ? k : 2, PAD_REFLECT, extra, 0, rel_len);
    }
    p.w = h->blob + g.w_off;
    p.bias = g.has_bias ? h->blob + g.b_off : nullptr;
    p.y = out.raw;
    p.y_elu = out.elu;
    p.y_bs = out_bs;
    p.y_rs = out_rs;
    p.B = B;
    p.M = M;
    p.N = g.N;
    p.Ktot = g.Ktot;
    const int rc = run_tap(h, st, p);
    if (y) {
        y->raw = Act{out.raw, out_bs, out_rs, M, g.N, p.amax_out, p.B};
        y->elu = Act{out.elu, out_bs, out_rs, M, g.N, p.amax_out, p.B};
    }
    return rc;
}


int convtr_fwd(ac_handle* h, hipStream_t st, const PackedGemm& g, const Act& x, int s, Out out, int B, Act2* y) {
    const int cout = g.N / s;
    if (s == 2) {
        const unsigned* am = nullptr;
        const int rc = try_thin6(h, st, g, x, 64, 0, out, B, &am);
        if (rc <= 0) {
            if (!rc) {
                y->raw = Act{out.raw, (long long)x.L * s * cout, cout, x.L * s, cout, am, B};
                y->elu = Act{out.elu, (long long)x.L * s * cout, cout, x.L * s, cout, am, B};
                HIPCHK(h, hipGetLastError());
            }
            return rc;
        }
    }
    TapGemmParams p{};
    p.nseg = 1;
    p.seg[0] = make_seg(x, 1, 2, PAD_ZERO, 0, 0, nullptr);
    p.w = h->blob + g.w_off;
    p.bias = h->blob + g.b_off;
    p.y = out.raw;
    p.y_elu = out.elu;
    p.y_bs = (long long)x.L * g.N;
    p.y_rs = g.N;
    p.B = B;
    p.M = x.L;
    p.N = g.N;
    p.Ktot = g.Ktot;
    const int rc = run_tap(h, st, p);
    y->raw = Act{out.raw, (long long)x.L * s * cout, cout, x.L * s, cout, p.amax_out, p.B};
    y->elu = Act{out.elu, (long long)x.L * s * cout, cout, x.L * s, cout, p.amax_out, p.B};
    return rc;
}


template <int C, int BM, int NSPLIT, bool SC = true>
int launch_rb_fused(ac_handle* h, hipStream_t st, const ResBlockPlan& rb, const Act2& x, Out out, int B, int pad = PAD_REFLECT) {
    using Cfg = RbCfg<C, BM, NSPLIT, SC>;
    RbFusedParams p{};
    p.xe = x.elu.p;
    p.xr = x.raw.p;
    p.w3 = h->blob + rb.c3.w_off;
    p.b3 = h->blob + rb.c3.b_off;
    p.wf = h->blob + rb.fused.w_off;
    p.bf = h->blob + rb.fused.b_off;
    p.y = out.raw;
    p.y_elu = out.elu;
    p.B = B;
    p.L = x.raw.L;
    p.Lp = x.raw.L > 2 ? x.raw.L : 3;
    p.ntiles = cdiv(x.raw.L, BM);
    p.pad = pad;
    if (int rc = ensure_lds(h, reinterpret_cast<const void*>(rb_fused_kernel<C, BM, NSPLIT, SC>), Cfg::lds_bytes)) return rc;
    const long long total = (long long)B * p.ntiles;
    const int grid = (int)std::min<long long>(total, 512);
    const size_t lds = Cfg::lds_bytes;
    const double L = x.raw.L;
    ProfScope ps(h, st, !SC ? "rb_fused_kernel<64, 64, 2, false>" : C == 32 ? "rb_fused_kernel<32, 128, 1>" : "rb_fused_kernel<64, 64, 2>",
                 2.0 * B * L * ((double)(C / 2) * 3 * C + (double)C * Cfg::KF),
                 (double)B * L * C * 4.0 * ((x.elu.p ? 2 : 1) + (out.raw ? 1 : 0) + (out.elu ? 1 : 0)));
    hipLaunchKernelGGL((rb_fused_kernel<C, BM, NSPLIT, SC>), dim3(grid), dim3(256), lds, st, p);
    return AC_OK;
}


bool rb_split16(ac_handle* h, hipStream_t st, const ResBlockPlan& rb, const Act2& x, int B, RbFused6Params& p, const unsigned** amax_out) {
    if (h->gemm_fp32 || !rb.winv3_off) return false;
    p.amax_in = amax_of(h, st, x.raw.p, x.raw.bs, x.raw.ts, x.raw.L, x.raw.C, B, x.raw.amax_n == B ? x.raw.amax : nullptr);
    p.winv3 = h->blob + rb.winv3_off;
    p.winvf = h->blob + rb.winvf_off;
    p.hb0 = rb.hb0;
    p.hb1 = rb.hb1;
    p.amax_out = amax_new(h);
    if (amax_out) *amax_out = p.amax_out;
    return true;
}


template <int C, bool SC>
int launch_rb_fused6(ac_handle* h, hipStream_t st, const ResBlockPlan& rb, const Act2& x, Out out, int B, int pad = PAD_REFLECT, const unsigned** amax_out = nullptr,
                     const PackedGemm* head = nullptr, int head_k = 0, float* head_y = nullptr) {
    using Cfg = Rb6Cfg<C, SC>;
    RbFused6Params p{};
    const bool with_head = head && C == 64 && !SC;
    if (with_head) {
        p.head_w = h->blob + head->w_off;
        p.head_b = h->blob + head->b_off;
        p.head_y = head_y;
        p.head_k = head_k;
    }
    p.xr = x.raw.p;
    p.w3f = reinterpret_cast<const __bf16*>(h->blob + rb.w3f_off);
    p.wff = reinterpret_cast<const __bf16*>(h->blob + rb.wff_off);
    p.b3 = h->blob + rb.c3.b_off;
    p.bf = h->blob + rb.fused.b_off;
    p.y = out.raw;
    p.y_elu = out.elu;
    p.B = B;
    p.L = x.raw.L;
    p.lpad = h->noncausal ? 1 : 2;
    p.Lp = x.raw.L > p.lpad ? x.raw.L : p.lpad + 1;
    p.ntiles = cdiv(x.raw.L, with_head ? Cfg::BM - (head_k - 1) : Cfg::BM);
    p.pad = pad;
    p.dbg = h->dev.rb6_dbg;
    if (!rb_split16(h, st, rb, x, B, p, amax_out)) return fail(h, AC_ESTATE, "fused residual block without split16 images");
    if (!p.amax_in) return fail(h, AC_ESTATE, "out of amax slots (split16.h)");
    if (with_head) p.amax_out = nullptr;
    const double L = x.raw.L;
    if (C == 64 && !with_head && h->dev.rb_stream && p.lpad == 2 && rb.w3p_off && (long long)x.raw.L * 256 < 0x70000000LL)
        return launch_rb_stream6(h, st, p, rb, SC, out, B);
    const size_t lds6 = with_head ? Cfg::lds_bytes16_head : Cfg::lds_bytes16;
    if (int rc = ensure_lds(h, with_head ? reinterpret_cast<const void*>(rb_fused6_head_kernel) : reinterpret_cast<const void*>(rb_fused6_kernel<C, SC, 2>), lds6)) return rc;
    const long long total = (long long)B * p.ntiles;
    const int per_cu = with_head ? RB6_HEAD_OCC : rb6_occupancy<C, SC, 2>();
    const int grid = (int)std::min<long long>(total, (long long)per_cu * 256);
    ProfScope ps(h, st, with_head ? "rb_fused6_head_kernel" : !SC ? "rb_fused6_kernel<64, false, 2>" : C == 32 ? "rb_fused6_kernel<32, true, 2>" : "rb_fused6_kernel<64, true, 2>",
                 2.0 * B * L * ((double)(C / 2) * 3 * C + (double)C * (C / 2 + (SC ? C : 0)) + (with_head ? (double)head_k * C : 0.0)),
                 with_head ? (double)B * L * (C + 1) * 4.0 : (double)B * L * C * 4.0 * (1 + (out.raw ? 1 : 0) + (out.elu ? 1 : 0)));
    if (with_head) hipLaunchKernelGGL(rb_fused6_head_kernel, dim3(grid), dim3(256), lds6, st, p);
    else hipLaunchKernelGGL((rb_fused6_kernel<C, SC, 2>), dim3(grid), dim3(256), lds6, st, p);
    return AC_OK;
}


template <bool SC>
int launch_rb128_fused6(ac_handle* h, hipStream_t st, const ResBlockPlan& rb, const Act2& x, Out out, int B, int pad = PAD_REFLECT, const unsigned** amax_out = nullptr) {
    using Cfg = Rb128Cfg<SC>;
    RbFused6Params p{};
    p.xr = x.raw.p;
    p.w3f = reinterpret_cast<const __bf16*>(h->blob + rb.w3f_off);
    p.wff = reinterpret_cast<const __bf16*>(h->blob + rb.wff_off);
    p.b3 = h->blob + rb.c3.b_off;
    p.bf = h->blob + rb.fused.b_off;
    p.y = out.raw;
    p.y_elu = out.elu;
    p.B = B;
    p.L = x.raw.L;
    p.lpad = h->noncausal ? 1 : 2;
    p.Lp = x.raw.L > p.lpad ? x.raw.L : p.lpad + 1;
    p.ntiles = cdiv(x.raw.L, Cfg::BM);
    p.pad = pad;
    if (!rb_split16(h, st, rb, x, B, p, amax_out)) return fail(h, AC_ESTATE, "fused residual block without split16 images");
    if (!p.amax_in) return fail(h, AC_ESTATE, "out of amax slots (split16.h)");
    if (h->dev.rb_stream && h->dev.rb128_stream && p.lpad == 2 && pad == (SC ? PAD_REFLECT : PAD_ZERO) && rb.w3p_off && (long long)x.raw.L * 512 < 0x70000000LL)
        return launch_rb_stream128m(h, st, p, rb, SC, out, B);
    if (int rc = ensure_lds(h, reinterpret_cast<const void*>(rb128_fused6_kernel<SC, 2>), Cfg::lds_bytes)) return rc;
    const long long total = (long long)B * p.ntiles;
    const int grid = (int)std::min<long long>(total, 256);
    const double L = x.raw.L;
    ProfScope ps(h, st, SC ? "rb128_fused6_kernel<true, 2>" : "rb128_fused6_kernel<false, 2>",
                 2.0 * B * L * (64.0 * 384 + 128.0 * (64 + (SC ? 128 : 0))),
                 (double)B * L * 128 * 4.0 * (1 + (out.raw ? 1 : 0) + (out.elu ? 1 : 0)));
    hipLaunchKernelGGL((rb128_fused6_kernel<SC, 2>), dim3(grid), dim3(512), Cfg::lds_bytes, st, p);
    return AC_OK;
}

// ... 180 lines not shown
        const size_t lds4 = ((size_t)(HEAD4_TT + THIN_MAXK) * (F + 4) + (size_t)THIN_MAXK * F) * sizeof(float);
        if (int rc = ensure_lds(h, reinterpret_cast<const void*>(head4_kernel), lds4)) return rc;
        ProfScope ps(h, st, "head4_kernel", 2.0 * B * (double)x.L * F * k, (double)B * x.L * 4.0 * (F + 1));
        hipLaunchKernelGGL(head4_kernel, dim3(cdiv(x.L, HEAD4_TT), B), dim3(256), lds4, st, p);
        HIPCHK(h, hipGetLastError());
        return AC_OK;
    }
    const size_t lds = ((size_t)(HEAD_TT + THIN_MAXK) * (F + 4) + (size_t)THIN_MAXK * F) * sizeof(float);
    if (int rc = ensure_lds(h, reinterpret_cast<const void*>(head_kernel), lds)) return rc;
    {
        ProfScope ps(h, st, "head_kernel", 2.0 * B * (double)x.L * F * k, (double)B * x.L * 4.0 * (F + 1));
        hipLaunchKernelGGL(head_kernel, dim3(cdiv(x.L, HEAD_TT), B), dim3(256), lds, st, p);
    }
    HIPCHK(h, hipGetLastError());
    return AC_OK;
}


int head_fwd(ac_handle* h, hipStream_t st, const Act& x, int B, float* sig) {
    return thin_head(h, st, h->dec_head, h->cfg.num_filters, h->cfg.last_kernel_size, PAD_REFLECT, x, B, sig);
}


bool enc_front_ok(const ac_handle* h, int T) {
    const ac_config& c = h->cfg;
    return h->fuse_chains && h->arch == ARCH_ENCODEC && !h->noncausal && !h->gemm_fp32 && h->enc_front.ok &&
           c.num_filters == 32 && c.kernel_size == 7 && c.residual_kernel_size == 3 && c.compress == 2 && c.num_ratios >= 1 &&
           c.upsampling_ratios[c.num_ratios - 1] == 2 && T >= 64 && (long long)T * 128 < 0x70000000LL;
}


int enc_front_fwd(ac_handle* h, hipStream_t st, const float* sig, const float* rel_len, int B, int T, float* y, float* dbg_x0, float* dbg_y1, Act2* out) {
    const ResBlockPlan& rb = h->enc_rb[0];
    const PackedGemm& gd = h->enc_down[0];
    EncFrontParams p{};
    p.sig = sig;
    p.rel_len = rel_len;
    p.w0 = h->blob + h->enc_stem.w_off;
    p.b0 = h->blob + h->enc_stem.b_off;
    p.w3f = reinterpret_cast<const __bf16*>(h->blob + rb.w3f_off);
    p.wff = reinterpret_cast<const __bf16*>(h->blob + rb.wff_off);
    p.wdf = reinterpret_cast<const __bf16*>(h->blob + h->t6_of[gd.w_off]);
    p.b3 = h->blob + rb.c3.b_off;
    p.winv3 = h->blob + rb.winv3_off;
    p.bf = h->blob + rb.fused.b_off;
    p.winvf = h->blob + rb.winvf_off;
    p.bd = h->blob + gd.b_off;
    p.winvd = h->blob + h->t6inv_of[gd.w_off];
    p.y = y;
    p.dbg_x0 = dbg_x0;
    p.dbg_y1 = dbg_y1;
    p.B = B;
    p.T = T;
    p.M = cdiv(T, 2);
    const int nchunks = cdiv(T, EF_ROWS);
    p.seg_chunks = std::max(8, cdiv(nchunks, std::max(1, 6144 / B)));
    if (h->dev.front_seg > 0) p.seg_chunks = h->dev.front_seg;
    p.segs_per_clip = cdiv(nchunks, p.seg_chunks);
    const bool v4 = T % 4 == 0 && aligned16(sig);
    p.amax_sig = amax_of(h, st, sig, T, v4 ? 4 : 1, v4 ? T / 4 : T, v4 ? 4 : 1, B, nullptr);
    if (!p.amax_sig) return fail(h, AC_ESTATE, "out of amax slots (split16.h)");
    p.amax_out = amax_new(h);
    p.sb0 = h->enc_front.sb0; p.sb1 = h->enc_front.sb1;
    p.hb0 = rb.hb0; p.hb1 = rb.hb1;
    p.fb0 = h->enc_front.fb0; p.fb1h = h->enc_front.fb1h; p.fb1x = h->enc_front.fb1x;
    if (h->dev.chain_stream && h->simg.enc_ok) {
        if (int rc = enc_stream_fwd(h, st, sig, rel_len, B, T, y, dbg_x0, dbg_y1, p.amax_sig, p.amax_out)) return rc;
        HIPCHK(h, hipGetLastError());
        out->raw = Act{y, (long long)p.M * 64, 64, p.M, 64, p.amax_out, B};
        out->elu = Act{nullptr, (long long)p.M * 64, 64, p.M, 64, p.amax_out, B};
        return AC_OK;
    }
    size_t lds = EF_LDS;
    lds += (size_t)h->dev.front_ldspad;
    if (int rc = ensure_lds(h, reinterpret_cast<const void*>(enc_front_kernel), lds)) return rc;
    const long long streams = (long long)B * p.segs_per_clip;
    {
        ProfScope ps(h, st, "enc_front_kernel", 2.0 * B * (double)T * (7.0 * 32 + 16.0 * 96 + 32.0 * 48 + 64.0 * 128 / 2),
                     (double)B * T * 4.0 + (double)B * p.M * 256.0);
        hipLaunchKernelGGL(enc_front_kernel, dim3((unsigned)cdiv((int)streams, EF_WAVES)), dim3(64 * EF_WAVES), lds, st, p);
    }
    HIPCHK(h, hipGetLastError());
    out->raw = Act{y, (long long)p.M * 64, 64, p.M, 64, p.amax_out, B};
    out->elu = Act{nullptr, (long long)p.M * 64, 64, p.M, 64, p.amax_out, B};
    return AC_OK;
}


bool dec_tail_ok(const ac_handle* h, const Act& xe) {
    const ac_config& c = h->cfg;
    return h->fuse_chains && h->arch == ARCH_ENCODEC && !h->noncausal && !h->gemm_fp32 && h->dec_tail.ok &&
           c.num_filters == 32 && c.last_kernel_size == 7 && c.residual_kernel_size == 3 && c.compress == 2 && c.num_ratios >= 1 &&
           c.upsampling_ratios[c.num_ratios - 1] == 2 && xe.p && xe.C == 64 && xe.ts == 64 && xe.bs == (long long)xe.L * 64 && aligned16(xe.p) &&
           xe.L >= 32 && (long long)xe.L * 256 < 0x70000000LL;
}


int dec_tail_fwd(ac_handle* h, hipStream_t st, const Act& xe, int B, float* sig, float* dbg_u, float* dbg_v) {
    const int last = h->cfg.num_ratios - 1;
    const ResBlockPlan& rb = h->dec_rb[last];
    const PackedGemm& gu = h->dec_up[last];
    DecTailParams p{};
    p.xe = xe.p;
    p.wuf = reinterpret_cast<const __bf16*>(h->blob + h->t6_of[gu.w_off]);
    p.w3f = reinterpret_cast<const __bf16*>(h->blob + rb.w3f_off);
    p.wff = reinterpret_cast<const __bf16*>(h->blob + rb.wff_off);
    p.bu = h->blob + gu.b_off;
    p.winvu = h->blob + h->t6inv_of[gu.w_off];
    p.b3 = h->blob + rb.c3.b_off;
    p.winv3 = h->blob + rb.winv3_off;
    p.bf = h->blob + rb.fused.b_off;
    p.winvf = h->blob + rb.winvf_off;
    p.wh = h->blob + h->dec_head.w_off;
    p.bh = h->blob + h->dec_head.b_off;
    p.sig = sig;
    p.dbg_u = dbg_u;
    p.dbg_v = dbg_v;
    p.B = B;
    p.L = xe.L;
    const int nchunks = cdiv(xe.L, DT_ROWS);
    p.seg_chunks = std::max(8, cdiv(nchunks, std::max(1, 6144 / B)));
    if (h->dev.tail_seg > 0) p.seg_chunks = h->dev.tail_seg;
    p.segs_per_clip = cdiv(nchunks, p.seg_chunks);
    p.amax_x = amax_of(h, st, xe.p, xe.bs, xe.ts, xe.L, xe.C, B, xe.amax_n == B ? xe.amax : nullptr);
    if (!p.amax_x) return fail(h, AC_ESTATE, "out of amax slots (split16.h)");
    p.ub0 = h->dec_tail.sb0; p.ub1 = h->dec_tail.sb1;
    p.hb0 = rb.hb0; p.hb1 = rb.hb1;
    if (h->dev.chain_stream && h->simg.dec_ok) {
        if (int rc = dec_stream_fwd(h, st, xe, B, sig, dbg_u, dbg_v, p.amax_x)) return rc;
        HIPCHK(h, hipGetLastError());
        return AC_OK;
    }
    if (int rc = ensure_lds(h, reinterpret_cast<const void*>(dec_tail_kernel), DT_LDS)) return rc;
    const long long streams = (long long)B * p.segs_per_clip;
    {
        ProfScope ps(h, st, "dec_tail_kernel", 2.0 * B * (double)xe.L * (64.0 * 128 + 2.0 * (16.0 * 96 + 32.0 * 48 + 7.0 * 32)),
                     (double)B * xe.L * 256.0 + (double)B * xe.L * 8.0);
        hipLaunchKernelGGL(dec_tail_kernel, dim3((unsigned)cdiv((int)streams, 8)), dim3(512), DT_LDS, st, p);
    }
    HIPCHK(h, hipGetLastError());
    return AC_OK;
}


void capture(ac_handle* h, hipStream_t st, const Act& a, int B) {
    if (!h->dbg) return;
    const size_t n = (size_t)B * a.L * a.C;
    if (h->dbg_used + n <= h->dbg_cap)
        (void)hipMemcpyAsync(h->dbg + h->dbg_used, a.p, n * sizeof(float), hipMemcpyDeviceToDevice, st);
    h->dbg_used += n;
}


int lstm_fwd(ac_handle* h, hipStream_t st, const LstmPlan& lp, const Act& x, const LstmWs& ws, Out out, int B, Act2* y) {
    const int D = lp.D, T = x.L, L = lp.layers;
    if (D % 64 != 0 || D > 512) return fail(h, AC_EINVAL, "LSTM width %d unsupported (need 64, 128, 256 or 512)", D);
    if (L < 1 || L > 2) return fail(h, AC_EINVAL, "%d LSTM layers unsupported (1 or 2)", L);
    hipStreamCaptureStatus cap = hipStreamCaptureStatusNone;
    (void)hipStreamIsCapturing(st, &cap);
    const bool persist = lp.has_persist && h->lp_ctl && h->num_cus == 256 && !h->lstm_step_only && x.ts == D && cap == hipStreamCaptureStatusNone;
    const bool fuse_env = h->dev.lstm_fuse_in != 0;
    const bool fuse_in = persist && !h->gemm_fp32 && fuse_env && aligned16(x.p) && x.bs % 4 == 0;
    if (!fuse_in) {
        TapGemmParams p{};
        p.nseg = 1;
        p.seg[0] = make_seg(x, 1, 1, PAD_ZERO, 0, 0, nullptr);
        p.w = h->blob + lp.ih[0].w_off;
        p.bias = h->blob + lp.ih[0].b_off;
        p.y = ws.gin;
        p.y_bs = 4LL * D;
        p.y_rs = (long long)B * 4 * D;
        p.B = B;
        p.M = T;
        p.N = 4 * D;
        p.Ktot = D;
        int rc = run_tap(h, st, p);
        if (rc) return rc;
    }
    const int nroles = 2 * L - 1, nlaunch = T + 2 * (L - 1);
    const long long BD = (long long)((B + 31) / 32 * 32) * D, B4D = (long long)B * 4 * D;
    if (persist) {
        const int chunks = cdiv(B, 64);
        const unsigned* x_amax = nullptr;
        if (fuse_in && lp.persist16_inv) {
            x_amax = amax_of(h, st, x.p, x.bs, x.ts, x.L, x.C, B, x.amax_n == B ? x.amax : nullptr);
            if (!x_amax) return fail(h, AC_ESTATE, "out of amax slots (split16.h)");
        }
        int* poison = reinterpret_cast<int*>(ws.c);
        if (!h->gemm_fp32) HIPCHK(h, hipMemsetAsync(poison, 0x7f, (size_t)B * sizeof(int), st));
        ProfScope ps(h, st, h->gemm_fp32 ? "lstm_persist_kernel" : fuse_in ? "lstm_persist16_kernel<true>" : "lstm_persist16_kernel<false>", 2.0 * T * (double)B * 4 * D * D * (nroles + (fuse_in ? 1 : 0)),
                     (double)T * ((double)B * 4 * D * 4 + 3.0 * B * D * 4) + 12.0 * D * D * 4, chunks);
        auto tail = [&](int c0, int nb, const int* pz) {
            LstmTailParams tp{};
            tp.ctl = h->lp_ctl;
            tp.sticky = h->sticky_dev;
            tp.poison = pz;
            tp.yout = out.raw;
            tp.yout_elu = out.elu;
            tp.y_bs = (long long)T * D;
            tp.clip0 = c0;
            tp.B = nb;
            tp.T = T;
            tp.D = D;
            tp.xcds_used = 8;
            hipLaunchKernelGGL(lstm_tail_kernel, dim3(nb, 4), dim3(256), 0, st, tp);
        };
        for (int c0 = 0; c0 < B; c0 += 64) {
            LstmPersistParams q{};
            q.gin0 = ws.gin;
            q.w_pk = h->blob + lp.persist_off;
            q.bias1 = h->blob + lp.ih[1].b_off;
            q.hseq0 = ws.hseq0;
            q.hseq1 = ws.hseq1;
            q.skip = x.p;
            q.yout = out.raw;
            q.yout_elu = out.elu;
            q.ctl = h->lp_ctl;
            q.gin_ts = B4D;
            q.h_ts = BD;
            q.skip_bs = x.bs;
            q.y_bs = (long long)T * D;
            q.B = std::min(64, B - c0);
            q.T = T;
            q.group0 = c0 / 16;
            q.clip0 = c0;
            q.dbg = h->dev.lstm_dbg;
            if (!h->gemm_fp32) {
                LstmPersist16Params q6{};
                q6.base = q;
                q6.base.h_ts = (long long)((B + 31) / 32 * 2) * LP16_GROUP_BYTES;
                q6.winv = h->blob + lp.persist16_inv;
                q6.amax_x = fuse_in ? x_amax : nullptr;
                q6.w_pk6 = reinterpret_cast<const __bf16*>(h->blob + lp.persist16_off);
                q6.bias0 = h->blob + lp.ih[0].b_off;
                q6.fuse_in = fuse_in ? 1 : 0;
                q6.poison = poison;
                q6.hseq0_local = ws.gin1;
                HIPCHK(h, hipMemsetAsync(h->lp_ctl, 0, LP_CTL_WORDS * sizeof(unsigned), st));
                const size_t hbytes = (size_t)T * (size_t)q6.base.h_ts;
                const size_t rbytes = (size_t)std::min(T, LP16_RING) * (size_t)q6.base.h_ts;
                HIPCHK(h, hipMemsetAsync(ws.hseq0, 0xFF, hbytes, st));
                HIPCHK(h, hipMemsetAsync(ws.hseq1, 0xFF, rbytes, st));
                HIPCHK(h, hipMemsetAsync(ws.gin1, 0xFF, rbytes, st));
                void* args6[] = {&q6};
                const void* kfn = fuse_in ? reinterpret_cast<const void*>(lstm_persist16_kernel<true>) : reinterpret_cast<const void*>(lstm_persist16_kernel<false>);
                HIPCHK(h, hipLaunchCooperativeKernel(kfn, dim3(256), dim3(512), args6, 0, st));
                tail(c0, q.B, poison);
                if (AC_DEV_MODE(q.dbg, 32)) {
                    HIPCHK(h, hipStreamSynchronize(st));
                    std::vector<unsigned long long> tr(8 * 64);
                    HIPCHK(h, hipMemcpy(tr.data(), h->lp_ctl + LP_CTL_FLAGS, tr.size() * 8, hipMemcpyDeviceToHost));
                    for (int role = 0; role < 2; ++role) {
                        std::fprintf(stderr, "lstm trace role %d (layer %d), 10 ns units from step start: ", role, role & 1);
                        for (int s_ = 0; s_ < 4; ++s_) {
                            const unsigned long long* r = &tr[role * 64 + s_ * 8];
                            std::fprintf(stderr, "| t=%d:", 100 + s_);
                            for (int k = 1; k < 8; ++k) std::fprintf(stderr, " %lld", r[k] ? (long long)(r[k] - r[0]) : -1LL);
                            if (s_ < 3) std::fprintf(stderr, " next %lld ", (long long)(r[8] - r[0]));
                        }
                        const double us3 = (double)(tr[role * 64 + 24] - tr[role * 64]) * 0.01;
                        std::fprintf(stderr, " | steps that had to poll: %llu of %d | shader clock %.0f MHz\n", tr[role * 64 + 63], T,
                                     us3 > 0 ? (double)(tr[role * 64 + 33] - tr[role * 64 + 32]) / us3 : 0.0);
                    }
                }
                continue;
            }
            HIPCHK(h, hipMemsetAsync(h->lp_ctl, 0, LP_CTL_WORDS * sizeof(unsigned), st));
            void* args[] = {&q};
            HIPCHK(h, hipLaunchCooperativeKernel(reinterpret_cast<const void*>(lstm_persist_kernel), dim3(256), dim3(256), args, 0, st));
            tail(c0, q.B, nullptr);
        }
        HIPCHK(h, hipGetLastError());
        const unsigned* am = amax_plus(h, st, x, 1.0f, B);
        y->raw = Act{out.raw, (long long)T * D, D, T, D, am, B};
        y->elu = Act{out.elu, (long long)T * D, D, T, D, am, B};
        return AC_OK;
    }
    {
        ProfScope ps(h, st, "lstm_step_kernel", 2.0 * T * (double)B * 4 * D * D * nroles,
                     (double)T * nroles * ((double)B * 4 * D * 4 + 4.0 * D * D * 4 + 2.0 * B * D * 4), nlaunch);
        for (int s = 0; s < nlaunch; ++s) {
            LstmLaunchParams q{};
            q.B = B;
            q.D = D;
            auto fill_last = [&](LstmRole& r, int t) {
                r.skip = x.p + (long long)t * x.ts;
                r.skip_bs = x.bs;
                r.yout = out.raw ? out.raw + (long long)t * D : nullptr;
                r.yout_elu = out.elu ? out.elu + (long long)t * D : nullptr;
                r.y_bs = (long long)T * D;
            };
            {
                LstmRole& r = q.role[0];
                r.active = s < T;
                r.kind = 0;
                r.a = s > 0 ? ws.hseq0 + (long long)(s - 1) * BD : nullptr;
                r.wpk = h->blob + lp.hh_off[0];
                r.gin = ws.gin + (long long)s * B4D;
                r.hnext = ws.hseq0 + (long long)s * BD;
                r.c = ws.c;
                r.first = s == 0;
                if (L == 1 && r.active) fill_last(r, s);
            }
            if (L == 2) {
                const int t1 = s - 1, t2 = s - 2;
                LstmRole& pr = q.role[1];
                pr.active = t1 >= 0 && t1 < T;
                pr.kind = 1;
                pr.a = ws.hseq0 + (long long)std::max(t1, 0) * BD;
                pr.wpk = h->blob + lp.ihpk_off[1];
                pr.bias = h->blob + lp.ih[1].b_off;
                pr.gout = ws.gin1 + (long long)std::max(t1, 0) * B4D;
                LstmRole& r = q.role[2];
                r.active = t2 >= 0 && t2 < T;
                r.kind = 0;
                r.a = t2 > 0 ? ws.hseq1 + (long long)(t2 - 1) * BD : nullptr;
                r.wpk = h->blob + lp.hh_off[1];
                r.gin = ws.gin1 + (long long)std::max(t2, 0) * B4D;
                r.hnext = ws.hseq1 + (long long)std::max(t2, 0) * BD;
                r.c = ws.c + (long long)B * D;
                r.first = t2 == 0;
                if (r.active) fill_last(r, t2);
            }
            const dim3 grid(D / 4, cdiv(B, 32), nroles), block(256);
            switch (D / 32) {
                case 2: hipLaunchKernelGGL(lstm_step_kernel<2>, grid, block, 0, st, q); break;
                case 4: hipLaunchKernelGGL(lstm_step_kernel<4>, grid, block, 0, st, q); break;
                case 8: hipLaunchKernelGGL(lstm_step_kernel<8>, grid, block, 0, st, q); break;
                default: hipLaunchKernelGGL(lstm_step_kernel<16>, grid, block, 0, st, q); break;
            }
        }
    }
    HIPCHK(h, hipGetLastError());
    const unsigned* am = amax_plus(h, st, x, 1.0f, B);
    y->raw = Act{out.raw, (long long)T * D, D, T, D, am, B};
    y->elu = Act{out.elu, (long long)T * D, D, T, D, am, B};
    return AC_OK;
}


int rvq_encode_fwd(ac_handle* h, hipStream_t st, const float* feats, int F, int K, long long* toks) {
    RvqEncParams p{};
    p.x = feats;
    p.epk = h->blob + h->cb_packed;
    p.e = h->blob + h->cb_plain;
    p.ee = h->blob + h->cb_ee;
    p.toks = toks;
    p.F = F;
    p.H = h->cfg.hidden_size;
    p.C = h->cfg.codebook_size;
    p.K = K;
    p.xs = p.H;
    p.tK = K;
    p.tk0 = 0;
    const int HV = p.H / 16;
    const int MS = (HV <= 8 && F >= 1024 * 32) ? 3 : 1;
    const dim3 grid(cdiv(F, 16 * MS)), block(64);
    const bool exact_env = h->dev.rvq_exact != 0;
    if (h->cb16 && (HV == 8 || (HV == 32 && K == 1)) && !exact_env) {
        RvqEnc16Params q{};
        q.base = p;
        q.epk16 = reinterpret_cast<const _Float16*>(h->blob + h->cb16);
        q.einv = h->blob + h->cb16_inv;
        ProfScope ps(h, st, "rvq_encode16_kernel", 2.0 * F * (double)p.C * p.H * K,
                     (double)F * p.H * 4 + (double)F * K * 8 + (double)K * p.C * p.H * 4);
        if (HV == 32) hipLaunchKernelGGL((rvq_encode16_kernel<32, 1, false, true>), dim3(cdiv(F, 16)), block, 0, st, q);
        else if (MS == 3) hipLaunchKernelGGL((rvq_encode16_kernel<8, 3, false>), grid, block, 0, st, q);
        else if (F <= 4096 && p.C % 128 == 0) hipLaunchKernelGGL((rvq_encode16_kernel<8, 1, false, false, 4>), grid, dim3(256), 0, st, q);
        else hipLaunchKernelGGL((rvq_encode16_kernel<8, 1, false>), grid, block, 0, st, q);
        HIPCHK(h, hipGetLastError());
        return AC_OK;
    }
    ProfScope ps(h, st, "rvq_encode_kernel", 2.0 * F * (double)p.C * p.H * K,
                 (double)F * p.H * 4 + (double)F * K * 8 + (double)K * p.C * p.H * 4);
#define RVQ_CASE(HV_, MS_) hipLaunchKernelGGL((rvq_encode_kernel<HV_, MS_, false>), grid, block, 0, st, p)
    switch (HV * 10 + MS) {
        case 11: RVQ_CASE(1, 1); break;
        case 13: RVQ_CASE(1, 3); break;
        case 21: RVQ_CASE(2, 1); break;
        case 23: RVQ_CASE(2, 3); break;
        case 41: RVQ_CASE(4, 1); break;
        case 43: RVQ_CASE(4, 3); break;
        case 81: RVQ_CASE(8, 1); break;
        case 83: RVQ_CASE(8, 3); break;
        case 161: RVQ_CASE(16, 1); break;
        case 321: RVQ_CASE(32, 1); break;
        default: return fail(h, AC_EINVAL, "hidden_size %d unsupported by the RVQ kernel (need 16*{1,2,4,8,16,32})", p.H);
    }
#undef RVQ_CASE
    HIPCHK(h, hipGetLastError());
    return AC_OK;
}


int rvq_decode_fwd(ac_handle* h, hipStream_t st, const long long* toks, int F, int K, float* out) {
    RvqDecParams p{};
    p.toks = toks;
    p.e = h->blob + h->cb_plain;
    p.out = out;
    p.F = F;
    p.H = h->cfg.hidden_size;
    p.C = h->cfg.codebook_size;
    p.K = K;
    p.tK = K;
    p.tk0 = 0;
    p.os = p.H;
    const long long n = (long long)F * (p.H / 4);
    p.bad = h->sticky_dev ? h->sticky_dev + ST_BAD_TOKEN : nullptr;
    ProfScope ps(h, st, "rvq_decode_kernel", (double)F * p.H * K, (double)F * K * 8 + (double)F * p.H * 4 * (K + 1));
    hipLaunchKernelGGL(rvq_decode_kernel, dim3((unsigned)((n + 255) / 256)), dim3(256), 0, st, p);
    HIPCHK(h, hipGetLastError());
    return AC_OK;
}


Workspace plan_ws(const ac_handle* h, int B, int T_in , int N_frames , bool enc) {
    const ac_config& c = h->cfg;
    Workspace w;
    size_t mx = 0;
    int N;
    if (enc) {
        long long L = T_in;
        int ch = c.num_filters;
        mx = std::max(mx, (size_t)L * ch);
        for (int r = c.num_ratios - 1; r >= 0; --r) {
            L = (L + c.upsampling_ratios[r] - 1) / c.upsampling_ratios[r];
            ch *= 2;
            mx = std::max(mx, (size_t)L * ch);
        }
        N = (int)L;
    } else {
        N = N_frames;
        long long L = N;
        int ch = h->D;
        mx = std::max(mx, (size_t)L * ch);
        for (int r = 0; r < c.num_ratios; ++r) {
            L *= c.upsampling_ratios[r];
            ch /= 2;
            mx = std::max(mx, (size_t)L * ch);
        }
    }
    mx = std::max(mx, (size_t)N * std::max(h->D, c.hidden_size));
    w.act_floats = align_up(mx * B, 64);
    w.hseq = align_up((size_t)N * ((B + 31) / 32 * 32) * h->D * 3 / 2, 64);
    w.gin = std::max(align_up((size_t)N * B * 4 * h->D, 64), w.hseq);
    w.c = align_up((size_t)2 * B * h->D, 64);
    w.total_bytes = (NACT * w.act_floats + 2 * w.gin + 2 * w.hseq + w.c) * sizeof(float) + 256;
    add_pool(w, B, 0);
    return w;
}


int carve(ac_handle* h, const Workspace& w, void* ws, size_t ws_bytes, WsPtrs* o) {
    if (!ws) return fail(h, AC_EINVAL, "workspace pointer is null");
    if (ws_bytes < w.total_bytes) return fail(h, AC_ENOMEM, "workspace too small: %zu < %zu bytes", ws_bytes, w.total_bytes);
    char* base = reinterpret_cast<char*>(align_up(reinterpret_cast<uintptr_t>(ws), 256));
    pool_bind(h, base, w.pool_B, w.pool_rows);
    float* p = reinterpret_cast<float*>(base + align_up(pool_bytes(w.pool_B, w.pool_rows), 256));
    for (int i = 0; i < NACT; ++i) { o->act[i] = p; o->used[i] = false; p += w.act_floats; }
    o->lstm.gin = p; p += w.gin;
    o->lstm.gin1 = p; p += w.gin;
    o->lstm.hseq0 = p; p += w.hseq;
    o->lstm.hseq1 = p; p += w.hseq;
    o->lstm.c = p;
    return AC_OK;
}


int check_ready(ac_handle* h) {
    if (!h) return AC_EINVAL;
    if (!h->finalized) return fail(h, AC_ESTATE, "ac_finalize has not been called");
    if (h->sticky) {
        volatile unsigned* s = h->sticky;
        const unsigned a = s[ST_LSTM_TIMEOUT], b = s[ST_LSTM_PLACEMENT], t = s[ST_BAD_TOKEN];
        if (a || b || t) {
            s[ST_LSTM_TIMEOUT] = 0;
            s[ST_LSTM_PLACEMENT] = 0;
            s[ST_BAD_TOKEN] = 0;
            char lstm[400] = "", tok[200] = "";
            if (a || b) {
                h->lstm_step_only = true;
                std::snprintf(lstm, sizeof lstm,
                              "an EARLIER call's persistent LSTM launch failed (%u bounded waits expired, %u launches without 32 workgroups on "
                              "every XCD -- is the GPU shared?): that call's outputs were set to NaN; the handle now uses the per-step LSTM "
                              "kernels, repeat the call", a, b);
            }
            if (t) std::snprintf(tok, sizeof tok, "an EARLIER ac_decode / ac_dequantize call got %u token ids outside [0, codebook_size): those frames were set to NaN", t);
            return fail(h, (a || b) ? AC_EHIP : AC_EINVAL, "%s%s%s", lstm, (a || b) && t ? "; ALSO: " : "", tok);
        }
    }
    return AC_OK;
}


int check_len(ac_handle* h, long long samples) {
    if (h->arch == ARCH_SPK) return fail(h, AC_EINVAL, "a speaker-encoder handle has no codec entry points (ac_spk_embed)");
    if (h->arch == ARCH_LM) return fail(h, AC_EINVAL, "a Llama decoder handle has no codec entry points (ac_lm_forward, ac_lm_step)");
    const long long lim = 0x70000000LL / (h->arch == ARCH_DAC ? 512 : 256) - 1;
    if (samples > lim) return fail(h, AC_EINVAL, "clip of %lld samples is too long for one call (limit %lld): split it", samples, lim);
    return AC_OK;
}


int encoder_fwd(ac_handle* h, hipStream_t st, const float* sig, const float* rel_len, int B, int T, float* feats, WsPtrs& ws) {
    const ac_config& c = h->cfg;
    const bool dbg = h->dbg != nullptr;
    Act xin{sig, (long long)T, 1, T, 1};
    Act2 x, y;
    int rc;
    auto rb_self_elu = [&](int C) {
        if (h->noncausal && h->gemm_fp32) return false;
        return (C == 32 || C == 64 || (C == 128 && c.num_ratios > 2 && rb128_ok(h, h->enc_rb[2]))) && c.residual_kernel_size == 3 && c.compress == 2;
    };
    auto rb256_self_elu = [&](int i, int L) { return i < c.num_ratios && h->enc_rb[i].C == h->enc_down[i - 1].N && rb256_ok(h, h->enc_rb[i], L); };
    int i0 = 0;
    if (enc_front_ok(h, T)) {
        float* d0 = dbg ? ws.take() : nullptr;
        float* d1 = dbg ? ws.take() : nullptr;
        rc = enc_front_fwd(h, st, sig, rel_len, B, T, ws.take(), d0, d1, &x);
        if (rc) return rc;
        if (dbg) {
            capture(h, st, Act{d0, (long long)T * 32, 32, T, 32}, B);
            capture(h, st, Act{d1, (long long)T * 32, 32, T, 32}, B);
            ws.give(d0);
            ws.give(d1);
        }
        capture(h, st, x.raw, B);
        i0 = 1;
    } else {
    if (thin_ok(c, c.kernel_size))
        rc = stem_fwd(h, st, sig, rel_len, B, T, Out{ws.take(), rb_self_elu(c.num_filters) ? nullptr : ws.take()}, &x);
    else
        rc = conv_fwd(h, st, h->enc_stem, xin, c.kernel_size, 1, rel_len, Out{ws.take(), ws.take()},
                      (long long)T * c.num_filters, c.num_filters, B, &x);
    if (rc) return rc;
    capture(h, st, x.raw, B);
    }
    for (int i = i0; i < c.num_ratios; ++i) {
        const int ratio = c.upsampling_ratios[c.num_ratios - 1 - i];
        float* hb = ws.take();
        rc = resblock_fwd(h, st, h->enc_rb[i], x, hb, Out{dbg ? ws.take() : nullptr, ws.take()}, B, &y);
        if (rc) return rc;
        ws.give(hb);
        ws.give(x);
        if (dbg) { capture(h, st, y.raw, B); ws.give(y.raw.p); y.raw.p = nullptr; }
        x = y;
        const int M = cdiv(x.elu.L, ratio);
        const bool last = i == c.num_ratios - 1;
        rc = conv_fwd(h, st, h->enc_down[i], x.elu, 2 * ratio, ratio, nullptr,
                      Out{ws.take(), (last || rb_self_elu(h->enc_down[i].N) || rb256_self_elu(i + 1, M)) ? nullptr : ws.take()},
                      (long long)M * h->enc_down[i].N, h->enc_down[i].N, B, &y);
        if (rc) return rc;
        ws.give(x);
        x = y;
        capture(h, st, x.raw, B);
    }
    rc = lstm_fwd(h, st, h->enc_lstm, x.raw, ws.lstm, Out{dbg ? ws.take() : nullptr, ws.take()}, B, &y);
    if (rc) return rc;
    ws.give(x);
    if (dbg) { capture(h, st, y.raw, B); ws.give(y.raw.p); y.raw.p = nullptr; }
    x = y;
    rc = conv_fwd(h, st, h->enc_final, x.elu, c.last_kernel_size, 1, nullptr, Out{feats, nullptr},
                  (long long)x.elu.L * c.hidden_size, c.hidden_size, B, nullptr);
    ws.give(x);
    return rc;
}


int decoder_fwd(ac_handle* h, hipStream_t st, const long long* toks, int B, int N, int K, float* sig, WsPtrs& ws) {
    const ac_config& c = h->cfg;
    const bool dbg = h->dbg != nullptr;
    float* zb = ws.take();
    int rc = rvq_decode_fwd(h, st, toks, B * N, K, zb);
    if (rc) return rc;
    Act z{zb, (long long)N * c.hidden_size, c.hidden_size, N, c.hidden_size};
    Act2 x, y;
    rc = conv_fwd(h, st, h->dec_first, z, c.kernel_size, 1, nullptr, Out{ws.take(), nullptr}, (long long)N * h->D, h->D, B, &x);
    if (rc) return rc;
    ws.give(zb);
    capture(h, st, x.raw, B);
    rc = lstm_fwd(h, st, h->dec_lstm, x.raw, ws.lstm, Out{dbg ? ws.take() : nullptr, ws.take()}, B, &y);
    if (rc) return rc;
    ws.give(x);
    if (dbg) { capture(h, st, y.raw, B); ws.give(y.raw.p); y.raw.p = nullptr; }
    x = y;
    for (int i = 0; i < c.num_ratios; ++i) {
        if (i == c.num_ratios - 1 && dec_tail_ok(h, x.elu)) {
            const long long T2 = 2LL * x.elu.L;
            float* d0 = dbg ? ws.take() : nullptr;
            float* d1 = dbg ? ws.take() : nullptr;
            rc = dec_tail_fwd(h, st, x.elu, B, sig, d0, d1);
            if (rc) return rc;
            if (dbg) {
                capture(h, st, Act{d0, T2 * 32, 32, (int)T2, 32}, B);
                capture(h, st, Act{d1, T2 * 32, 32, (int)T2, 32}, B);
                ws.give(d0);
                ws.give(d1);
            }
            ws.give(x);
            return AC_OK;
        }
        const int cup = h->dec_up[i].N / c.upsampling_ratios[i];
        const bool self_elu = ((cup == 32 || cup == 64 || (cup == 128 && rb128_ok(h, h->dec_rb[i]))) && c.residual_kernel_size == 3 &&
                               c.compress == 2) ||
                              (cup == h->dec_rb[i].C && rb256_ok(h, h->dec_rb[i], x.elu.L * c.upsampling_ratios[i]));
        rc = convtr_fwd(h, st, h->dec_up[i], x.elu, c.upsampling_ratios[i], Out{ws.take(), self_elu ? nullptr : ws.take()}, B, &y);
        if (rc) return rc;
        ws.give(x);
        x = y;
        capture(h, st, x.raw, B);
        float* hb = ws.take();
        rc = resblock_fwd(h, st, h->dec_rb[i], x, hb, Out{dbg ? ws.take() : nullptr, ws.take()}, B, &y);
        if (rc) return rc;
        ws.give(hb);
        ws.give(x);
        if (dbg) { capture(h, st, y.raw, B); ws.give(y.raw.p); y.raw.p = nullptr; }
        x = y;
    }
    if (thin_ok(c, c.last_kernel_size) && x.elu.ts == c.num_filters)
        rc = head_fwd(h, st, x.elu, B, sig);
    else
        rc = conv_fwd(h, st, h->dec_head, x.elu, c.last_kernel_size, 1, nullptr, Out{sig, nullptr}, (long long)x.elu.L, 1, B, nullptr);
    ws.give(x);
    return rc;
}

int mimi_linear(ac_handle* h, hipStream_t st, const PackedGemm& g, const float* x, long long rows, int cin, int x_pitch, int kofs,
                float* y, int y_pitch, const Epi& epi) {
    const long long widest = std::max<long long>(std::max(x_pitch, y_pitch), g.N);
    long long chunk = ((1LL << 31) / 4 - 4096) / widest / 128 * 128;
    if (chunk < 128) return fail(h, AC_EINVAL, "linear layer too wide for the tap-GEMM (%lld)", widest);
    for (long long r0 = 0; r0 < rows; r0 += chunk) {
        const long long n = std::min(chunk, rows - r0);
        TapGemmParams p{};
        p.nseg = 1;
        Act xa{x + r0 * x_pitch, 0, x_pitch, (int)n, cin};
        const bool one = r0 == 0 && n == rows;
        if (one && epi.rowmax_in) { xa.amax = epi.rowmax_in; xa.amax_n = -(int)n; }
        p.seg[0] = make_seg(xa, 1, 1, PAD_ZERO, 0, kofs, nullptr);
        if (one && epi.rowmax_out) p.amax_out_rows = reinterpret_cast<unsigned*>(1);
        p.amax_rows = 1;
        p.w = h->blob + g.w_off;
        p.bias = g.has_bias ? h->blob + g.b_off : nullptr;
        p.y = y + r0 * y_pitch;
        p.y_bs = 0;
        p.y_rs = y_pitch;
        p.B = 1;
        p.M = (int)n;
        p.N = g.N;
        p.Ktot = g.Ktot;
        p.scale = epi.scale;
        p.res = epi.res ? epi.res + r0 * epi.res_rs : nullptr;
        p.res_bs = 0;
        p.res_rs = epi.res_rs;
        p.gelu = epi.gelu;
        if (int rc = run_tap(h, st, p)) return rc;
        if (epi.rowmax_out) *epi.rowmax_out = one ? p.amax_out_rows : nullptr;
    }
    return AC_OK;
}

int upload_blob(ac_handle* h, Packer& pk, int device) {
    HIPCHK(h, hipSetDevice(device));
    hipDeviceProp_t prop;
    HIPCHK(h, hipGetDeviceProperties(&prop, device));
    if (std::strncmp(prop.gcnArchName, "gfx950", 6) != 0)
        return fail(h, AC_ENODEV, "device %d is %s; this library is built for gfx950 only", device, prop.gcnArchName);
    h->num_cus = prop.multiProcessorCount;
    const char* lm = std::getenv("AC_LSTM");
    h->lstm_step_only = lm && std::strcmp(lm, "step") == 0;
    HIPCHK(h, hipMalloc(reinterpret_cast<void**>(&h->lp_ctl), LP_CTL_WORDS * sizeof(unsigned)));
    HIPCHK(h, hipMemset(h->lp_ctl, 0, LP_CTL_WORDS * sizeof(unsigned)));
    HIPCHK(h, hipHostMalloc(reinterpret_cast<void**>(&h->sticky), ST_WORDS * sizeof(unsigned), hipHostMallocMapped));
    std::memset(h->sticky, 0, ST_WORDS * sizeof(unsigned));
    HIPCHK(h, hipHostGetDevicePointer(reinterpret_cast<void**>(&h->sticky_dev), h->sticky, 0));
    if (h->num_cus == 256 && !h->lstm_step_only) {
        unsigned* hist = h->lp_ctl;
        void* args[] = {&hist};
        unsigned got[16] = {0};
        bool ok = hipLaunchCooperativeKernel(reinterpret_cast<const void*>(lstm_persist_probe_kernel), dim3(256), dim3(256), args, 0, nullptr) == hipSuccess &&
                  hipDeviceSynchronize() == hipSuccess && hipMemcpy(got, hist, sizeof got, hipMemcpyDeviceToHost) == hipSuccess;
        for (int i = 0; ok && i < 16; ++i) ok = got[i] == (i < 8 ? 32u : 0u);
        if (!ok) { (void)hipGetLastError(); h->lstm_step_only = true; }
        HIPCHK(h, hipMemset(h->lp_ctl, 0, LP_CTL_WORDS * sizeof(unsigned)));
    }
    if (h->arch == ARCH_MIMI) {
        h->own_pool_rows = (size_t)h->mcfg.codebook_size;
        HIPCHK(h, hipMalloc(&h->own_pool, pool_bytes(1, h->own_pool_rows)));
    }
    h->blob_floats = pk.blob.size();
    HIPCHK(h, hipMalloc(reinterpret_cast<void**>(&h->blob), h->blob_floats * sizeof(float)));
    HIPCHK(h, hipMemcpy(h->blob, pk.blob.data(), h->blob_floats * sizeof(float), hipMemcpyHostToDevice));
    h->host.clear();
    h->finalized = true;
    return AC_OK;
}

bool rb64_identity_head_fwd(ac_handle* h, hipStream_t st, const ResBlockPlan& rb, const Act2& x, const PackedGemm& head, int head_k, float* sig, int B, int* rc) {
    if (!rb.has6 || h->gemm_fp32 || h->dbg || h->dev.mimi_tail == 0 || head_k < 1 || head_k > 8 || head.N != 1 || head.Ktot != head_k * 64 || !head.has_bias) return false;
    *rc = launch_rb_fused6<64, false>(h, st, rb, x, Out{}, B, PAD_ZERO, nullptr, &head, head_k, sig);
    return true;
}
int rb64_identity_fwd(ac_handle* h, hipStream_t st, const ResBlockPlan& rb, const Act2& x, Out out, int B, const unsigned** amax_out) {
    return rb.has6 && !h->gemm_fp32 ? launch_rb_fused6<64, false>(h, st, rb, x, out, B, PAD_ZERO, amax_out) : launch_rb_fused<64, 64, 2, false>(h, st, rb, x, out, B, PAD_ZERO);
}
int rb128_identity_fwd(ac_handle* h, hipStream_t st, const ResBlockPlan& rb, const Act2& x, Out out, int B, const unsigned** amax_out) {
    return launch_rb128_fused6<false>(h, st, rb, x, out, B, PAD_ZERO, amax_out);
}
int rvq_encode_cdist_launch(ac_handle* h, hipStream_t st, const RvqEncParams& p, unsigned blocks, const _Float16* epk16, const float* einv) {
    const dim3 grid(blocks), block(64);
    if (epk16 && p.H == 256 && !h->dev.rvq_exact) {
        RvqEnc16Params q{};
        q.base = p;
        q.epk16 = epk16;
        q.einv = einv;
        hipLaunchKernelGGL((rvq_encode16_kernel<16, 1, true>), grid, block, 0, st, q);
        return AC_OK;
    }
    switch (p.H / 16) {
        case 1: hipLaunchKernelGGL((rvq_encode_kernel<1, 1, true>), grid, block, 0, st, p); break;
        case 2: hipLaunchKernelGGL((rvq_encode_kernel<2, 1, true>), grid, block, 0, st, p); break;
        case 4: hipLaunchKernelGGL((rvq_encode_kernel<4, 1, true>), grid, block, 0, st, p); break;
        case 8: hipLaunchKernelGGL((rvq_encode_kernel<8, 1, true>), grid, block, 0, st, p); break;
        case 16: hipLaunchKernelGGL((rvq_encode_kernel<16, 1, true>), grid, block, 0, st, p); break;
        default: return fail(h, AC_EINVAL, "codebook_dim %d unsupported by the RVQ kernel (need 16*{1,2,4,8,16})", p.H);
    }
    return AC_OK;
}
void rvq_decode_launch(hipStream_t st, const RvqDecParams& p, unsigned blocks) {
    hipLaunchKernelGGL(rvq_decode_kernel, dim3(blocks), dim3(256), 0, st, p);
}
int resample_launch(const float* x, int B, int L, const float* kern, int n, int o, int taps, int width, float* y, int L_out, hipStream_t st) {
    ResampleParams p{x, kern, y, B, L, L_out, n, o, taps, width};
    hipLaunchKernelGGL(resample_kernel, dim3((unsigned)((L_out + 255) / 256), B), dim3(256), 0, st, p);
// ... 56 lines not shown
```

audiocodecs_amd/csrc/lstm_persist.h:

```cpp
#pragma once
#include "lstm_consts.h"
#include <hip/hip_runtime.h>
#include "lstm.h"

namespace ac {


struct LstmPersistParams {
    const float* gin0;
    const float* w_pk;
    const float* bias1;
    float* hseq0;
    float* hseq1;
    const float* skip;
    float* yout;
    float* yout_elu;
    unsigned* ctl;
    long long gin_ts, h_ts, skip_bs, y_bs;
    int B, T;
    int group0;
    int clip0;
    int dbg;
};

constexpr int LP_CTL_SLOTS = 0;
constexpr int LP_CTL_TIMEOUT = 8 * 16;
constexpr int LP_CTL_FLAGS = 9 * 16;
constexpr int LP_CTL_WORDS = LP_CTL_FLAGS + 4 * 2 * LP_SLICES * LP_FLAG_STRIDE;

typedef unsigned u32x4_lp __attribute__((ext_vector_type(4)));
#define LP_RLX __ATOMIC_RELAXED, __HIP_MEMORY_SCOPE_AGENT
constexpr int LP_SC1 = 16;
constexpr int LP_SC0 = 1;

__device__ __forceinline__ unsigned lp_xcc_id() { return __builtin_amdgcn_s_getreg((3 << 11) | 20) & 0xf; }

__global__ __launch_bounds__(256) void lstm_persist_probe_kernel(unsigned* hist) {
    if (threadIdx.x == 0) atomicAdd(&hist[lp_xcc_id() & 15], 1u);
}

constexpr int LP_NEVER = 0x7f7f7f7f;

struct LstmTailParams {
    const unsigned* ctl;
    unsigned* sticky;
    const int* poison;
    float* yout;
    float* yout_elu;
    long long y_bs;
    int clip0, B, T, D;
    int xcds_used;
};

__global__ __launch_bounds__(256) void lstm_tail_kernel(const LstmTailParams p) {
    const int b = blockIdx.x;
    const unsigned tmo = p.ctl[LP_CTL_TIMEOUT];
    bool placed = true;
    for (int x = 0; x < 8; ++x) {
        const unsigned n = p.ctl[LP_CTL_SLOTS + x * 16];
        placed = placed && (x < p.xcds_used ? n == 32u : n <= 32u);
    }
    const bool failed = tmo != 0u || !placed;
    if (failed && b == 0 && blockIdx.y == 0 && threadIdx.x == 0)
        __hip_atomic_fetch_add(&p.sticky[(tmo == 2u || !placed) ? ST_LSTM_PLACEMENT : ST_LSTM_TIMEOUT], 1u, __ATOMIC_RELAXED, __HIP_MEMORY_SCOPE_SYSTEM);
    int t0 = p.T;
    if (failed) t0 = 0;
    else if (p.poison) {
        const int q = p.poison[p.clip0 + b];
        if (q < p.T) {
            t0 = q;
            if (blockIdx.y == 0 && threadIdx.x == 0)
                __hip_atomic_fetch_add(&p.sticky[ST_NONFINITE_CLIPS], 1u, __ATOMIC_RELAXED, __HIP_MEMORY_SCOPE_SYSTEM);
        }
    }
    if (t0 >= p.T) return;
    const float nan = __uint_as_float(0x7fc00000u);
    const long long n = (long long)(p.T - t0) * p.D;
    const long long o = (long long)(p.clip0 + b) * p.y_bs + (long long)t0 * p.D;
    for (long long i = (long long)blockIdx.y * 256 + threadIdx.x; i < n; i += 256LL * gridDim.y) {
        if (p.yout) p.yout[o + i] = nan;
        if (p.yout_elu) p.yout_elu[o + i] = nan;
    }
}

__device__ __forceinline__ bool lp_wait(unsigned* flags, unsigned want, unsigned* tmo, int lane, int dbg = 0) {
    if (AC_DEV_MODE(dbg, 4)) return true;
    for (unsigned spins = 0;; ++spins) {
        const unsigned f = lane < LP_SLICES ? __hip_atomic_load(&flags[lane * LP_FLAG_STRIDE], LP_RLX) : 0xffffffffu;
        if (__all(f >= want)) return true;
        if ((spins & 1023) == 1023 && __hip_atomic_load(tmo, LP_RLX)) return false;
        if (spins > (1u << 22)) { __hip_atomic_store(tmo, 1u, LP_RLX); return false; }
    }
}

__global__ __launch_bounds__(256) void lstm_persist_kernel(const LstmPersistParams p) {
    constexpr int D = LP_D;
    __shared__ float part[4][4][16][17];
    __shared__ unsigned s_x, s_slot;
    __shared__ int s_okp, s_okr;
    const int tid = threadIdx.x, lane = tid & 63, wave = tid >> 6;
    const int li = lane & 15, kq = lane >> 4;
    unsigned* tmo = p.ctl + LP_CTL_TIMEOUT;
    if (tid == 0) {
        s_x = lp_xcc_id();
        s_slot = __hip_atomic_fetch_add(&p.ctl[LP_CTL_SLOTS + (s_x & 7) * 16], 1u, LP_RLX);
    }
    __syncthreads();
    const int x = s_x & 7, slot = s_slot;
    const int g = x >> 1;
    const int G = (p.B + 15) >> 4;
    if (slot >= 32) {
        if (tid == 0) __hip_atomic_store(tmo, 2u, LP_RLX);
        return;
    }
    if (g >= G) return;
    if (AC_DEV_MODE(p.dbg, 1) && (slot >> 4) == 1) return;
    const int layer = slot >> 4, idx = (x & 1) * 16 + (slot & 15), u0 = idx * 16;

    f32x4 wa[4][8], wb[4][8];
    {
        const long long mat = (long long)LP_SLICES * 4 * 4 * 8 * 256;
        const float* base = p.w_pk + ((long long)idx * 4 + wave) * (4 * 8 * 256) + lane * 4;
        const float* pa = base + (layer == 0 ? 0 : mat);
        const float* pb = base + 2 * mat;
#pragma unroll
        for (int n = 0; n < 4; ++n)
#pragma unroll
            for (int ks = 0; ks < 8; ++ks) {
                wa[n][ks] = *reinterpret_cast<const f32x4*>(pa + (n * 8 + ks) * 256);
                wb[n][ks] = layer ? *reinterpret_cast<const f32x4*>(pb + (n * 8 + ks) * 256) : f32x4{0.f, 0.f, 0.f, 0.f};
            }
    }
    unsigned* flags0 = p.ctl + LP_CTL_FLAGS + ((g * 2 + 0) * LP_SLICES) * LP_FLAG_STRIDE;
    unsigned* flags1 = p.ctl + LP_CTL_FLAGS + ((g * 2 + 1) * LP_SLICES) * LP_FLAG_STRIDE;
    unsigned* myflag = (layer ? flags1 : flags0) + idx * LP_FLAG_STRIDE;
    float* hmine = layer ? p.hseq1 : p.hseq0;
    const long long goff = (long long)(p.group0 + g) * (D / 16) * 256;

    const int ec = tid >> 4, ej = tid & 15;
    const int eb = g * 16 + ec;
    const bool live = eb < p.B;
    const long long erow = (long long)(p.clip0 + eb);
    const int eu = u0 + ej;
    float cstate = 0.f;
    float bq[4] = {0.f, 0.f, 0.f, 0.f};
    if (layer == 1) {
#pragma unroll
        for (int q = 0; q < 4; ++q) bq[q] = p.bias1[q * D + eu];
    }
    const int hpos = (((ej >> 2) << 4) + ec) * 4 + (ej & 3);

    auto load_a = [&](const float* seq, int t, f32x4 (&a)[8]) {
        const float* src = seq + (long long)t * p.h_ts + goff + (long long)(wave * 8) * 256;
        const __amdgpu_buffer_rsrc_t rs = __builtin_amdgcn_make_buffer_rsrc((void*)src, 0, 8 * 1024, 0x00020000);
#pragma unroll
        for (int ks = 0; ks < 8; ++ks) a[ks] = __builtin_bit_cast(f32x4, __builtin_amdgcn_raw_buffer_load_b128(rs, (ks * 64 + lane) * 16, 0, LP_SC1));
    };
    f32x4 accP[4];
    auto project = [&](int t) -> bool {
        if (wave == 0) { const bool ok = lp_wait(flags0, (unsigned)(t + 1), tmo, lane, p.dbg); if (lane == 0) s_okp = ok; }
        __syncthreads();
        if (!s_okp) return false;
        f32x4 a[8];
        load_a(p.hseq0, t, a);
#pragma unroll
        for (int n = 0; n < 4; ++n) accP[n] = f32x4{0.f, 0.f, 0.f, 0.f};
#pragma unroll
        for (int ks = 0; ks < 8; ++ks)
#pragma unroll
            for (int u = 0; u < 4; ++u)
#pragma unroll
                for (int n = 0; n < 4; ++n) accP[n] = __builtin_amdgcn_mfma_f32_16x16x4f32(a[ks][u], wa[n][ks][u], accP[n], 0, 0, 0);
        return true;
    };
#pragma unroll
    for (int n = 0; n < 4; ++n) accP[n] = f32x4{0.f, 0.f, 0.f, 0.f};
    if (layer == 1 && !project(0)) return;

    for (int t = 0; t < p.T; ++t) {
        float gpre[4] = {bq[0], bq[1], bq[2], bq[3]};
        float skipv = 0.f;
        if (live) {
            if (layer == 0) {
                const float* gp = p.gin0 + (long long)t * p.gin_ts + erow * (4 * D);
#pragma unroll
                for (int q = 0; q < 4; ++q) gpre[q] = gp[q * D + eu];
            } else if (p.skip) {
                skipv = p.skip[erow * p.skip_bs + (long long)t * D + eu];
            }
        }
        f32x4 acc[4];
#pragma unroll
        for (int n = 0; n < 4; ++n) acc[n] = accP[n];
        if (t > 0) {
            if (wave == 0) { const bool ok = lp_wait(layer ? flags1 : flags0, (unsigned)t, tmo, lane, p.dbg); if (lane == 0) s_okr = ok; }
            __syncthreads();
            if (!s_okr) return;
            f32x4 a[8];
            load_a(hmine, t - 1, a);
            if (AC_DEV_MODE(p.dbg, 2)) {
                acc[0] += a[0] + a[7];
            } else if (layer == 0) {
#pragma unroll
                for (int ks = 0; ks < 8; ++ks)
#pragma unroll
                    for (int u = 0; u < 4; ++u)
#pragma unroll
                        for (int n = 0; n < 4; ++n) acc[n] = __builtin_amdgcn_mfma_f32_16x16x4f32(a[ks][u], wa[n][ks][u], acc[n], 0, 0, 0);
            } else {
#pragma unroll
                for (int ks = 0; ks < 8; ++ks)
#pragma unroll
                    for (int u = 0; u < 4; ++u)
#pragma unroll
                        for (int n = 0; n < 4; ++n) acc[n] = __builtin_amdgcn_mfma_f32_16x16x4f32(a[ks][u], wb[n][ks][u], acc[n], 0, 0, 0);
            }
        }
#pragma unroll
        for (int n = 0; n < 4; ++n)
#pragma unroll
            for (int r = 0; r < 4; ++r) part[wave][n][kq * 4 + r][li] = acc[n][r];
        __syncthreads();
        float pre[4];
#pragma unroll
        for (int q = 0; q < 4; ++q) pre[q] = gpre[q] + ((part[0][q][ec][ej] + part[1][q][ec][ej]) + (part[2][q][ec][ej] + part[3][q][ec][ej]));
        const float ig = sigmoidf_(pre[0]), fg = sigmoidf_(pre[1]), gg = tanhf_(pre[2]), og = sigmoidf_(pre[3]);
        cstate = fg * cstate + ig * gg;
        const float hn = og * tanhf_(cstate);
        {
            float* dst = hmine + (long long)t * p.h_ts + goff + (long long)idx * 256;
            const __amdgpu_buffer_rsrc_t rs = __builtin_amdgcn_make_buffer_rsrc((void*)dst, 0, 1024, 0x00020000);
            __builtin_amdgcn_raw_buffer_store_b32(__builtin_bit_cast(unsigned, hn), rs, hpos * 4, 0, LP_SC1);
        }
        asm volatile("s_waitcnt vmcnt(0)" ::: "memory");
// ... 16 lines not shown
```

audiocodecs_amd/csrc/lstm_persist16.h:

```cpp
#pragma once
#include "lstm_persist.h"
#include "tap_gemm6.h"
#include "rb_fused6.h"
#include <type_traits>

namespace ac {

constexpr int LP16_SLICE_BYTES = 2 * 16 * 16 * 2;
constexpr long long LP16_GROUP_BYTES = (long long)LP_SLICES * LP16_SLICE_BYTES;
#ifndef LP16_RING_N
#define LP16_RING_N 8
#endif
constexpr int LP16_RING = LP16_RING_N;
static_assert(LP16_RING >= 4 && (LP16_RING & (LP16_RING - 1)) == 0, "ring of the recurrent exchange: a power of two, >= 4 (see above)");

struct LstmPersist16Params {
    LstmPersistParams base;
    const __bf16* w_pk6;
    const float* bias0;
    int fuse_in;
    int* poison;
    const float* winv;
    const unsigned* amax_x;
    void* hseq0_local;
};

#ifndef LP16_HEXP
#define LP16_HEXP 1
#endif
constexpr float LP16_HSCALE = LP16_HEXP ? 2.0f : 1.0f, LP16_HINV = LP16_HEXP ? 0.5f : 1.0f;
#ifndef LP16_BATCH_N
#define LP16_BATCH_N 4
#endif
constexpr int LP16_BATCH = LP16_BATCH_N;
#ifndef LP16_PART_PITCH
#define LP16_PART_PITCH 16
#endif
#ifndef LP16_LATE_FLAG
#define LP16_LATE_FLAG 1
#endif
#ifndef LP16_LATE_SLEEP
#define LP16_LATE_SLEEP 0
#endif

template <bool FUSE>
__global__ __launch_bounds__(512) void lstm_persist16_kernel(const LstmPersist16Params pp) {
    const LstmPersistParams& p = pp.base;
    constexpr int D = LP_D, NP = 2;
    constexpr int SLICE_BYTES = LP16_SLICE_BYTES;
    constexpr long long GROUP_BYTES = LP16_GROUP_BYTES;
    __shared__ f32x4 part[2][8][16][LP16_PART_PITCH];
    __shared__ unsigned s_x, s_slot;
    __shared__ __attribute__((aligned(16))) unsigned pubflag[4];
    __shared__ unsigned short hist[LP16_BATCH][2][256];
    const int tid = threadIdx.x, lane = tid & 63;
    const int wave = __builtin_amdgcn_readfirstlane(tid >> 6);
    const int li = lane & 15, kq = lane >> 4;
    unsigned* tmo = p.ctl + LP_CTL_TIMEOUT;
    if (tid < 4) pubflag[tid] = 0;
    if (tid == 0) {
        s_x = lp_xcc_id();
        s_slot = __hip_atomic_fetch_add(&p.ctl[LP_CTL_SLOTS + (s_x & 7) * 16], 1u, LP_RLX);
    }
    __syncthreads();
    const int x = s_x & 7, slot = s_slot;
    const int g = x >> 1;
    const int G = (p.B + 15) >> 4;
    if (slot >= 32) {
        if (tid == 0) __hip_atomic_store(tmo, 2u, LP_RLX);
        return;
    }
    if (g >= G) return;
    if (AC_DEV_MODE(p.dbg, 16)) {
        if (tid == 0) __hip_atomic_store(tmo, 1u, LP_RLX);
        return;
    }
    if (AC_DEV_MODE(p.dbg, 1) && (x & 1) == 1) return;
    const int layer_rt = x & 1, idx = slot, u0 = idx * 16;
    auto body = [&](auto layer_tag, auto late_tag) {
    constexpr int layer = decltype(layer_tag)::value;
    constexpr bool LATE = decltype(late_tag)::value;
    auto await_publish = [&](int t) {
#if LP16_LATE_FLAG
        for (int spins = 0; spins < (1 << 12); ++spins) {
            const u32x4_t f = *reinterpret_cast<volatile u32x4_t*>(pubflag);
            const unsigned lo = f.x < f.y ? f.x : f.y, lo2 = f.z < f.w ? f.z : f.w;
            if ((lo < lo2 ? lo : lo2) > (unsigned)t) break;
            if ((spins & 63) == 63 && __hip_atomic_load(tmo, LP_RLX)) break;
            __builtin_amdgcn_s_sleep(1);
        }
#else
        (void)t;
#endif
        __builtin_amdgcn_s_sleep(LP16_LATE_SLEEP);
    };

    bf16x8 wa[4][2][2], wb[4][2][2];
    {
        const long long mat = (long long)LP_SLICES * 4 * 4 * 4 * NP * 512;
        const __bf16* base = pp.w_pk6 + ((long long)idx * 4 + (wave >> 1)) * (4 * 4 * NP * 512) + lane * 8;
        const __bf16* pa = base + (layer == 0 ? 0 : mat);
        const __bf16* pb = base + (layer == 0 ? 3 : 2) * mat;
#pragma unroll
        for (int n = 0; n < 4; ++n)
#pragma unroll
            for (int ks = 0; ks < 2; ++ks)
#pragma unroll
                for (int pl = 0; pl < NP; ++pl) {
                    const int o = ((n * 4 + (wave & 1) * 2 + ks) * NP + pl) * 512;
                    wa[n][ks][pl] = *reinterpret_cast<const bf16x8*>(pa + o);
                    if (layer || FUSE) wb[n][ks][pl] = *reinterpret_cast<const bf16x8*>(pb + o);
                    else wb[n][ks][pl] = wa[n][ks][pl];
                }
    }
    char* h0b = reinterpret_cast<char*>(p.hseq0);
    char* h1b = reinterpret_cast<char*>(p.hseq1);
    char* hmine = layer ? h1b : reinterpret_cast<char*>(pp.hseq0_local);
    const long long goff = (long long)(p.group0 + g) * GROUP_BYTES;
    auto rt = [](int t) { return t & (LP16_RING - 1); };

    const bool gate_thr = tid < 256;
    const int ec = (tid & 255) >> 4, ej = tid & 15;
    const int eb = g * 16 + ec;
    const bool live = gate_thr && eb < p.B;
    const long long erow = (long long)(p.clip0 + eb);
    const int eu = u0 + ej;
    float cstate = 0.f;
    float bq[4] = {0.f, 0.f, 0.f, 0.f};
    const bool fuse0 = layer == 0 && FUSE;
    if (layer == 1 || fuse0) {
#pragma unroll
        for (int q = 0; q < 4; ++q) bq[q] = (layer ? p.bias1 : pp.bias0)[q * D + eu];
    }
    float wiv[4];
#pragma unroll
    for (int q = 0; q < 4; ++q) wiv[q] = LP16_HINV * pp.winv[layer * 4 * D + q * D + eu];
    const int hpos = ec * 32 + ej * 2;

    auto load_a = [&](const char* seq, int t, bf16x8 (&a)[2][2]) {
        const char* src = seq + (long long)t * p.h_ts + goff + (long long)(wave * 4) * SLICE_BYTES;
        const __amdgpu_buffer_rsrc_t rs = __builtin_amdgcn_make_buffer_rsrc((void*)src, 0, 4 * SLICE_BYTES, 0x00020000);
        const int lo = (kq >> 1) * SLICE_BYTES + li * 32 + (kq & 1) * 16;
#pragma unroll
        for (int ks = 0; ks < 2; ++ks)
#pragma unroll
            for (int pl = 0; pl < NP; ++pl)
                a[ks][pl] = __builtin_bit_cast(bf16x8, __builtin_amdgcn_raw_buffer_load_b128(rs, ks * 2 * SLICE_BYTES + pl * 512 + lo, 0, LP_SC1));
    };
    auto mac = [&](const bf16x8 (&a)[2][2], const bf16x8 (&w)[4][2][2], f32x4 (&acc)[4], int ks0 = 0, int ks1 = 2) {
#pragma unroll
        for (int ks = ks0; ks < ks1; ++ks)
#pragma unroll
            for (int n = 0; n < 4; ++n) {
                f32x4 v = acc[n];
                v = __builtin_amdgcn_mfma_f32_16x16x32_f16(__builtin_bit_cast(f16x8, a[ks][1]), __builtin_bit_cast(f16x8, w[n][ks][0]), v, 0, 0, 0);
                v = __builtin_amdgcn_mfma_f32_16x16x32_f16(__builtin_bit_cast(f16x8, a[ks][0]), __builtin_bit_cast(f16x8, w[n][ks][1]), v, 0, 0, 0);
                acc[n] = __builtin_amdgcn_mfma_f32_16x16x32_f16(__builtin_bit_cast(f16x8, a[ks][0]), __builtin_bit_cast(f16x8, w[n][ks][0]), v, 0, 0, 0);
            }
    };
    auto valid = [&](const bf16x8 (&a)[2][2]) -> bool {
        unsigned bad = 0;
#pragma unroll
        for (int ks = 0; ks < 2; ++ks)
#pragma unroll
            for (int pl = 0; pl < NP; ++pl) {
                const u32x4_t w = __builtin_bit_cast(u32x4_t, a[ks][pl]);
                bad |= (w.x | w.y) | (w.z | w.w);
            }
        return __all((bad & 0x40004000u) == 0u);
    };
    auto load_valid = [&](const char* seq, int t, bf16x8 (&a)[2][2]) -> bool {
        for (unsigned spins = 0;; ++spins) {
            load_a(seq, t, a);
            if (valid(a) || AC_DEV_MODE(p.dbg, 4)) return true;
            if ((spins & 63) == 63 && __hip_atomic_load(tmo, LP_RLX)) return false;
            if (spins > (1u << 18)) { __hip_atomic_store(tmo, 1u, LP_RLX); return false; }
            __builtin_amdgcn_s_sleep(4);
        }
    };
    bf16x8 arec[2][2];
    float skip_next = 0.f;
    f32x4 accP[4];
    const bool xlive = g * 16 + li < p.B;
    const __amdgpu_buffer_rsrc_t xrs = __builtin_amdgcn_make_buffer_rsrc(
        (void*)(p.skip + (long long)(p.clip0 + g * 16) * p.skip_bs), 0, (int)(((long long)(p.B - g * 16 < 16 ? p.B - g * 16 : 16)) * p.skip_bs * 4), 0x00020000);
    const int xoff = xlive ? (int)((long long)li * p.skip_bs * 4) + (wave * 64 + 8 * kq) * 4 : 0x7fff0000;
    f32x4 xr[2][2];
    auto fetch0 = [&](int t) {
#pragma unroll
        for (int ks = 0; ks < 2; ++ks)
#pragma unroll
            for (int hf = 0; hf < 2; ++hf)
                xr[ks][hf] = bufload16(xrs, xlive ? xoff + (t * D + ks * 32 + hf * 4) * 4 : 0x7fff0000, 0);
    };
    float xsc = 1.f, xcr[4] = {1.f, 1.f, 1.f, 1.f};
    if (fuse0) {
        const int cb = p.clip0 + g * 16, cl = p.clip0 + p.B - 1;
        xsc = s16_pow2(s16_exponent(*amax_at(pp.amax_x, cb + li <= cl ? cb + li : cl)));
#pragma unroll
        for (int r = 0; r < 4; ++r) xcr[r] = s16_pow2(LP16_HEXP - s16_exponent(*amax_at(pp.amax_x, cb + kq * 4 + r <= cl ? cb + kq * 4 + r : cl)));
    }
    bf16x8 xa[2][2];
    auto convert0 = [&]() {
        bf16x8 (&a)[2][2] = xa;
#pragma unroll
        for (int ks = 0; ks < 2; ++ks) {
            typedef _Float16 f16x4v __attribute__((ext_vector_type(4)));
            const f32x4 s0 = xr[ks][0] * xsc, s1 = xr[ks][1] * xsc;
            const f16x4v h0 = __builtin_convertvector(s0, f16x4v), h1 = __builtin_convertvector(s1, f16x4v);
            const f16x4v l0 = __builtin_convertvector(s0 - __builtin_convertvector(h0, f32x4), f16x4v);
            const f16x4v l1 = __builtin_convertvector(s1 - __builtin_convertvector(h1, f32x4), f16x4v);
            a[ks][0] = __builtin_bit_cast(bf16x8, __builtin_shufflevector(h0, h1, 0, 1, 2, 3, 4, 5, 6, 7));
            a[ks][1] = __builtin_bit_cast(bf16x8, __builtin_shufflevector(l0, l1, 0, 1, 2, 3, 4, 5, 6, 7));
        }
    };
    auto project0 = [&](int t, int trec, auto rec_tag) {
        bf16x8 (&a)[2][2] = xa;
#pragma unroll
        for (int n = 0; n < 4; ++n) accP[n] = f32x4{0.f, 0.f, 0.f, 0.f};
        if constexpr (decltype(rec_tag)::value && !LATE) load_a(hmine, rt(trec), arec);
        mac(a, wb, accP, 0, 1);
        mac(a, wb, accP, 1, 2);
#pragma unroll
        for (int n = 0; n < 4; ++n)
#pragma unroll
            for (int r = 0; r < 4; ++r) accP[n][r] *= xcr[r];
        if constexpr (decltype(rec_tag)::value && LATE) {
            __builtin_amdgcn_sched_barrier(0);
            await_publish(trec);
            load_a(hmine, rt(trec), arec);
        }
        (void)t;
    };
    auto project = [&](int t) -> bool {
        bf16x8 a[2][2];
        if (!load_valid(h0b, t, a)) return false;
#pragma unroll
        for (int n = 0; n < 4; ++n) accP[n] = f32x4{0.f, 0.f, 0.f, 0.f};
        mac(a, wa, accP);
        return true;
    };
#pragma unroll
    for (int n = 0; n < 4; ++n) accP[n] = f32x4{0.f, 0.f, 0.f, 0.f};
    if (layer == 1 && !project(0)) return;
    if (fuse0) {
        fetch0(0);
        convert0();
        project0(0, 0, std::false_type{});
        fetch0(p.T > 1 ? 1 : 0);
    }
    const float* skip_row = p.skip + (live ? erow : (long long)p.clip0) * p.skip_bs + eu;
    if (layer == 1) skip_next = skip_row[0];
    bf16x8 ap[2][2];
    if (layer == 1) load_a(h0b, p.T > 1 ? 1 : 0, ap);

    const bool trc = AC_DEV_MODE(p.dbg, 32) && idx == 0 && tid == 0;
    unsigned long long* trw = reinterpret_cast<unsigned long long*>(p.ctl + LP_CTL_FLAGS) + (g * 2 + layer) * 64;
#define LP16_TRC(pt_) do { if (trc && t >= 100 && t < 104) trw[(t - 100) * 8 + (pt_)] = __builtin_amdgcn_s_memrealtime(); } while (0)
    auto step = [&](int t) -> bool {
        if (trc && t >= 100 && t < 104) { trw[(t - 100) * 8 + 6] = 0; trw[(t - 100) * 8 + 7] = 0; }
        LP16_TRC(0);
        if (trc && (t == 100 || t == 103)) trw[32 + (t == 103)] = __builtin_amdgcn_s_memtime();
        float gpre[4] = {bq[0], bq[1], bq[2], bq[3]};
        const float skipv = skip_next;
        if (live && layer == 0 && !FUSE) {
            const float* gp = p.gin0 + (long long)t * p.gin_ts + erow * (4 * D);
#pragma unroll
            for (int q = 0; q < 4; ++q) gpre[q] = gp[q * D + eu];
        }
        f32x4 acc[4];
#pragma unroll
        for (int n = 0; n < 4; ++n) acc[n] = accP[n];
        if (t > 0) {
            const bool first_ok = (layer == 1 || fuse0) && (valid(arec) || AC_DEV_MODE(p.dbg, 4));
            if (trc && !first_ok) trw[63] += 1;
            if (!first_ok && !load_valid(hmine, rt(t - 1), arec)) return false;
            LP16_TRC(1);
            if (layer == 0) mac(arec, wa, acc);
            else mac(arec, wb, acc);
        }
        bool ap_ok = true;
        if (fuse0) {
            convert0();
            fetch0(t + 2 < p.T ? t + 2 : p.T - 1);
        }
        if (layer == 1) ap_ok = valid(ap) || AC_DEV_MODE(p.dbg, 4);
        LP16_TRC(2);
        f32x4 (&pt)[8][16][LP16_PART_PITCH] = part[t & 1];
#pragma unroll
        for (int r = 0; r < 4; ++r) pt[wave][kq * 4 + r][li] = f32x4{acc[0][r], acc[1][r], acc[2][r], acc[3][r]};
        lds_barrier();
        LP16_TRC(3);
        float hn = 0.f;
        if (gate_thr) {
            float pre[4];
            f32x4 pv[8];
#pragma unroll
            for (int w = 0; w < 8; ++w) pv[w] = pt[w][ec][ej];
#pragma unroll
            for (int q = 0; q < 4; ++q) {
                const float sum = ((pv[0][q] + pv[1][q]) + (pv[2][q] + pv[3][q])) + ((pv[4][q] + pv[5][q]) + (pv[6][q] + pv[7][q]));
                pre[q] = __fmaf_rn(sum, wiv[q], gpre[q]);
            }
            const float ig = sigmoid_rcp(pre[0]), fg = sigmoid_rcp(pre[1]), gg = tanh_rcp(pre[2]), og = sigmoid_rcp(pre[3]);
            cstate = fg * cstate + ig * gg;
            hn = og * tanh_rcp(cstate);
            LP16_TRC(6);
            const bool nonfinite = !(fabsf(hn) < 2.0f);
            if (nonfinite && live) atomicMin(pp.poison + erow, t);
            const float hp = nonfinite ? 0.f : hn;
            const float h2 = LP16_HSCALE * hp;
            _Float16 hh = (_Float16)h2;
            if (LP16_HEXP && fabsf((float)hh) >= 2.0f) hh = (_Float16)copysignf(1.9990234375f, h2);
            const _Float16 hl = (_Float16)(h2 - (float)hh);
            char* dst = hmine + (long long)rt(t) * p.h_ts + goff + (long long)idx * SLICE_BYTES;
            const __amdgpu_buffer_rsrc_t rs = __builtin_amdgcn_make_buffer_rsrc((void*)dst, 0, SLICE_BYTES, 0x00020000);
            __builtin_amdgcn_raw_buffer_store_b16(__builtin_bit_cast(unsigned short, hh), rs, hpos, 0, LP_SC0);
            __builtin_amdgcn_raw_buffer_store_b16(__builtin_bit_cast(unsigned short, hl), rs, 512 + hpos, 0, LP_SC0);
            LP16_TRC(7);
            if (lane == 0) pubflag[wave] = (unsigned)t + 1u;
            if (t >= 2) {
                char* old = hmine + (long long)rt(t - 2) * p.h_ts + goff + (long long)idx * SLICE_BYTES;
                const __amdgpu_buffer_rsrc_t ro = __builtin_amdgcn_make_buffer_rsrc((void*)old, 0, SLICE_BYTES, 0x00020000);
                __builtin_amdgcn_raw_buffer_store_b16((unsigned short)0xFFFFu, ro, hpos, 0, LP_SC0);
                __builtin_amdgcn_raw_buffer_store_b16((unsigned short)0xFFFFu, ro, 512 + hpos, 0, LP_SC0);
            }
            if (layer == 0) {
                hist[t % LP16_BATCH][0][tid] = __builtin_bit_cast(unsigned short, hh);
                hist[t % LP16_BATCH][1][tid] = __builtin_bit_cast(unsigned short, hl);
            }
        }
        LP16_TRC(4);
        if (layer == 0 && gate_thr && ((t + 1) % LP16_BATCH == 0 || t + 1 == p.T)) {
            for (int tb = t - (t % LP16_BATCH); tb <= t; ++tb) {
                const __amdgpu_buffer_rsrc_t rx = __builtin_amdgcn_make_buffer_rsrc((void*)(h0b + (long long)tb * p.h_ts + goff + (long long)idx * SLICE_BYTES), 0, SLICE_BYTES, 0x00020000);
#pragma unroll
                for (int pl = 0; pl < NP; ++pl) __builtin_amdgcn_raw_buffer_store_b16(hist[tb % LP16_BATCH][pl][tid], rx, pl * 512 + hpos, 0, LP_SC1);
            }
        }
        if (layer == 1) {
            if (live) {
                const float yv = hn + skipv;
                const long long o = erow * p.y_bs + (long long)t * D + eu;
                if (p.yout) p.yout[o] = yv;
                if (p.yout_elu) p.yout_elu[o] = elu1(yv);
            }
            const int t1 = t + 1 < p.T ? t + 1 : t;
            if (!ap_ok && !load_valid(h0b, t1, ap)) return false;
#pragma unroll
            for (int n = 0; n < 4; ++n) accP[n] = f32x4{0.f, 0.f, 0.f, 0.f};
            if constexpr (!LATE) load_a(hmine, rt(t), arec);
            mac(ap, wa, accP, 0, 1);
            if constexpr (!LATE) skip_next = skip_row[(long long)t1 * D];
            mac(ap, wa, accP, 1, 2);
            if constexpr (LATE) {
                __builtin_amdgcn_sched_barrier(0);
                await_publish(t);
                load_a(hmine, rt(t), arec);
                skip_next = skip_row[(long long)t1 * D];
            }
            load_a(h0b, t + 2 < p.T ? t + 2 : t1, ap);
        } else if (fuse0) {
            project0(t + 1 < p.T ? t + 1 : t, t, std::true_type{});
        }
        LP16_TRC(5);
        return true;
    };
    for (int t = 0; t < p.T; ++t)
        if (!step(t)) return;
#undef LP16_TRC
    };
    if (wave < 4) {
        if (layer_rt == 0) body(std::integral_constant<int, 0>{}, std::false_type{});
        else body(std::integral_constant<int, 1>{}, std::false_type{});
    } else {
        if (layer_rt == 0) body(std::integral_constant<int, 0>{}, std::true_type{});
        else body(std::integral_constant<int, 1>{}, std::true_type{});
    }
}

}
```

audiocodecs_amd/csrc/tap_gemm.h:

```cpp
#pragma once
#include <hip/hip_runtime.h>
#include <stdint.h>

namespace ac {

typedef float f32x4 __attribute__((ext_vector_type(4)));

struct TapSeg {
    const float* x;
    long long bs;
    long long ts;
    const float* rel_len;
    int L;
    int cin;
    int cin_shift;
    int s;
    int J;
    int Lp;
    int lim;
    int reflect;
    int elu;
    int kofs;
    int pad;
    int dil;
    const unsigned* amax;
    int amax_n;
};

struct TapGemmParams {
    TapSeg seg[2];
    int nseg;
    const float* w;
    const float* bias;
    float* y;
    float* y_elu;
    long long y_bs, y_rs;
    int B, M, N, Ktot;
    int mtiles, ntiles;
    const float* scale;
    const float* res;
    long long res_bs, res_rs;
    int gelu;
    const float* alpha;
    const float* alpha_inv;
    int alpha_n;
    int tanh_out;
    long long y_off, y_len;
    int n_valid;
    const float* winv;
    unsigned* amax_out;
    int amax_rows;
    unsigned* amax_out_rows;
    int epi_direct;
    int stagger;
    unsigned long long* clk;
};

enum { PAD_ZERO = 0, PAD_REFLECT = 1, PAD_REPLICATE = 2 };

__device__ __forceinline__ float gelu1(float v) {
    const float u = v * 0.70710678118654752440f;
    const float t = fabsf(u);
    float p = 4.536090636975132e-05f;
    p = fmaf(p, t, -0.00044552396866492927f);
    p = fmaf(p, t, 0.001489486894570291f);
    p = fmaf(p, t, 0.0007745670736767352f);
    p = fmaf(p, t, -0.02825363539159298f);
    p = fmaf(p, t, 0.1484815925359726f);
    p = fmaf(p, t, 0.9184163808822632f);
    p = fmaf(p, t, 1.6279085874557495f);
    const float er = copysignf(1.0f - __builtin_amdgcn_exp2f(-(p * t)), u);
    const float hv = 0.5f * v;
    return fmaf(hv, er, hv);
}

__device__ __forceinline__ float elu1(float v) { return v > 0.f ? v : (__expf(v) - 1.0f); }

__device__ __forceinline__ f32x4 elu4(f32x4 v) {
    v.x = elu1(v.x); v.y = elu1(v.y); v.z = elu1(v.z); v.w = elu1(v.w);
    return v;
}

__device__ __forceinline__ float sin2_f32(float t) {
    if (__builtin_expect(!(__builtin_fabsf(t) < 32768.f), 0)) {
        const float s = sinf(t);
        return __fmul_rn(s, s);
    }
    const float k = __builtin_rintf(__fmul_rn(t, 0.636619747f));
    float r = __fmaf_rn(k, -0x1.921fb6p+0f, t);
    r = __fmaf_rn(k, 0x1.777a5cp-25f, r);
    r = __fmaf_rn(k, 0x1.ee59dap-50f, r);
    const float z = __fmul_rn(r, r);
    float q = __fmaf_rn(2.7181215500604594e-06f, z, -0.00019839312881231308f);
    q = __fmaf_rn(q, z, 0.008333329111337662f);
    q = __fmaf_rn(q, z, -0.1666666716337204f);
    const float sn = __fmaf_rn(__fmul_rn(r, z), q, r);
    const float s2 = __fmul_rn(sn, sn);
    return ((int)k & 1) ? __fsub_rn(1.f, s2) : s2;
}
__device__ __forceinline__ float snake1(float v, float a, float ainv) {
    return __fadd_rn(v, __fmul_rn(ainv, sin2_f32(__fmul_rn(a, v))));
}

__device__ __forceinline__ float act1(const TapGemmParams& p, float v, int n) {
    if (p.alpha) {
        const int c = n % p.alpha_n;
        return snake1(v, p.alpha[c], p.alpha_inv[c]);
    }
    return elu1(v);
}

__device__ __forceinline__ float epilogue1(const TapGemmParams& p, float v, int n, long long res_off) {
    if (p.gelu) v = gelu1(v);
    if (p.scale) v = __fmul_rn(p.scale[n], v);
    if (p.res) v = __fadd_rn(p.res[res_off], v);
    if (p.tanh_out) v = tanhf(v);
    return v;
}

constexpr int GEN_EXTRA = 56;
constexpr int KC = 32;
constexpr int KCP = KC + 4;
constexpr int T6_DIL_HALO = 56;

__device__ __forceinline__ long long src_index(const TapSeg& sg, int i) {
    if (i >= sg.lim) return -1;
    int j = i;
    if (sg.reflect == PAD_REFLECT) {
        if (j < 0) j = -j;
        else if (j >= sg.Lp) j = 2 * (sg.Lp - 1) - j;
    } else if (sg.reflect == PAD_REPLICATE) {
        j = j < 0 ? 0 : (j >= sg.L ? sg.L - 1 : j);
    }
    if (j < 0 || j >= sg.L) return -1;
    return j;
}

template <int WGM, int WGN, int WM, int WN, bool VEC>
__global__ __launch_bounds__(WGM* WGN * 64) void tap_gemm_kernel(const TapGemmParams p) {
    constexpr int BM = WGM * WM * 16, BN = WGN * WN * 16, NT = WGM * WGN * 64;
    extern __shared__ __attribute__((aligned(16))) float smem[];
    float* As = smem;
    float* Ws = smem + (BM + GEN_EXTRA) * KCP;

    const int tid = threadIdx.x, lane = tid & 63, wave = tid >> 6;
    const int wm = wave / WGN, wn = wave % WGN;
    const int li = lane & 15, kq = lane >> 4;

    int id = blockIdx.x;
    const int nt = id % p.ntiles; id /= p.ntiles;
    const int mt = id % p.mtiles;
    const int b = id / p.mtiles;
    const int m0 = mt * BM, n0 = nt * BN;

    f32x4 acc[WM][WN];
#pragma unroll
    for (int a = 0; a < WM; ++a)
#pragma unroll
        for (int c = 0; c < WN; ++c) acc[a][c] = f32x4{0.f, 0.f, 0.f, 0.f};

    for (int si = 0; si < p.nseg; ++si) {
        const TapSeg& sg = p.seg[si];
        const int Cw = sg.s * sg.cin;
        const int R = BM + (sg.J - 1) * sg.dil;
        const float* xb = sg.x + (long long)b * sg.bs;
        float alen = 3.0e38f;
        if (sg.rel_len) alen = (float)sg.L * sg.rel_len[b];
        for (int c0 = 0; c0 < Cw; c0 += KC) {
            if (VEC) {
                for (int e = tid; e < R * (KC / 4); e += NT) {
                    const int row = e / (KC / 4), q = e % (KC / 4);
                    const int c = c0 + 4 * q;
                    f32x4 v = f32x4{0.f, 0.f, 0.f, 0.f};
                    if (c < Cw) {
                        const int r = m0 + row;
                        const int tp = sg.cin_shift >= 0 ? (c >> sg.cin_shift) : (c / sg.cin);
                        const int ci = c - tp * sg.cin;
                        const long long j = src_index(sg, r * sg.s + tp - sg.pad);
                        if (j >= 0 && (float)j < alen) {
// ... 93 lines not shown
```

audiocodecs_amd/csrc/tap_gemm8.h:

```cpp
#pragma once
#include "tap_gemm6.h"

namespace ac {

template <int WGM, int WGN, int WMT, int WN>
struct Tap8Cfg {
    using C6 = Tap6Cfg<WGM, WGN, WMT, WN, 7>;
    static_assert(WGM * WGN == 8, "8 waves");
    static constexpr int BM = C6::BM, BN = C6::BN, NT = C6::NT, A_ROWS = C6::A_ROWS, A_SLOTS = C6::A_SLOTS, PLANE = C6::PLANE;
    static constexpr int NTILES = BN / 32;
    static constexpr int B_PIECES = 2 * NTILES * 2;
    static constexpr int B_SLOT = B_PIECES * 512;
    static constexpr int PPW = B_PIECES / 8;
    static_assert(B_PIECES % 8 == 0, "fragments divide over the 8 waves");
    static constexpr size_t a_bytes = (size_t)2 * 2 * PLANE * 2;
    static constexpr size_t b_bytes = (size_t)2 * B_SLOT * 2;
    static_assert(a_bytes % 16 == 0, "ring base alignment");
    static constexpr size_t main_bytes = a_bytes + b_bytes;
    static constexpr size_t lds_bytes = main_bytes > C6::epi_bytes ? main_bytes : C6::epi_bytes;
    static_assert(lds_bytes <= 160 * 1024, "one workgroup per CU: slabs + weight ring (or the staged epilogue's tile) within 160 KB of LDS");
};

__device__ __forceinline__ void t8_glds16(const void* gsrc, unsigned lds_dst) {
#ifdef T8_ABL_NODMA
    return;
#endif
    unsigned keep;
    asm volatile("s_mov_b32 %0, m0\n\ts_mov_b32 m0, %2\n\ts_nop 0\n\tglobal_load_lds_dwordx4 %1, off\n\ts_mov_b32 m0, %0"
                 : "=&s"(keep) : "v"(gsrc), "s"(lds_dst) : "memory");
}
template <int N>
__device__ __forceinline__ void t8_wait() {
    asm volatile("s_waitcnt vmcnt(%0)" ::"n"(N) : "memory");
}

template <int WGM, int WGN, int WMT, int WN, bool RM, bool J1, bool SPREAD = true>
__global__ __launch_bounds__(512, 1) void tap_gemm8_kernel(const TapGemmParams p, const __bf16* __restrict__ wp) {
    using Cfg = Tap8Cfg<WGM, WGN, WMT, WN>;
    constexpr int BM = Cfg::BM, BN = Cfg::BN, NT = Cfg::NT, A_SLOTS = Cfg::A_SLOTS, PLANE = Cfg::PLANE, NTILES = Cfg::NTILES;
    constexpr int HALO = 7;
    unsigned long long clk_t0 = 0, clk_r0 = 0;
    if (p.clk) { clk_t0 = __builtin_amdgcn_s_memtime(); clk_r0 = __builtin_amdgcn_s_memrealtime(); }
    extern __shared__ __attribute__((aligned(16))) float smem[];
    __bf16* As0 = reinterpret_cast<__bf16*>(smem);
    __bf16* Bs0 = reinterpret_cast<__bf16*>(reinterpret_cast<char*>(smem) + Cfg::a_bytes);
    const unsigned bs_lds = (unsigned)(size_t)Bs0;

    const int tid = threadIdx.x, lane = tid & 63;
    const int wave = __builtin_amdgcn_readfirstlane(tid >> 6);
    const int wm = wave / WGN, wn = wave % WGN;
    const int i32 = lane & 31, kh = lane >> 5;

    int id;
    {
        const int total = gridDim.x, q = total >> 3, r = total & 7, xcd = blockIdx.x & 7, pos = blockIdx.x >> 3;
        id = (xcd < r ? xcd * (q + 1) : r * (q + 1) + (xcd - r) * q) + pos;
    }
    const int nt = id % p.ntiles; id /= p.ntiles;
    const int mt = id % p.mtiles;
    const int b = id / p.mtiles;
    const int m0 = mt * BM, n0 = nt * BN;
#ifdef T6_TRACE
    const bool t6_ph = p.clk && mt == p.mtiles / 2 && nt == 0 && b == p.B / 2 && tid == 64;
    const bool t8_on = p.clk && mt == p.mtiles / 2 && nt == 0 && b == p.B / 2 && lane == 0;
    int t8_stage = 0;
    if (t6_ph) p.clk[4] = clk_t0;
#define T8_STAMP(k) do { if (t8_on && t8_stage < 16) p.clk[16 + (wave * 16 + t8_stage) * 8 + (k)] = __builtin_amdgcn_s_memtime(); } while (0)
#define T8_USTAMP(u) do { if (t8_on && (t8_stage == 2 || t8_stage == 3) && (u) < 8) p.clk[16 + (wave * 16 + 8 + (u)) * 8 + 3 + t8_stage] = __builtin_amdgcn_s_memtime(); } while (0)
    T6_PHASE(1);
#else
    const bool t6_ph = false;
#define T8_STAMP(k) do { } while (0)
#define T8_USTAMP(u) do { } while (0)
#endif

    const TapSeg& sg = p.seg[0];
    const unsigned am_early = RM ? 0u : *amax_at(sg.amax, b);
    const int seg_J = sg.J, seg_Cw = sg.s * sg.cin, seg_kofs = sg.kofs, rowstep = sg.dil;
    const int NC = seg_Cw / KC;
    const long long lo_t = (long long)m0 * sg.s - sg.pad;
    const long long hi_t = (long long)(m0 + BM - 1 + (sg.J - 1) * sg.dil) * sg.s + (sg.s - 1) - sg.pad;
    const bool inside = lo_t >= 0 && hi_t < sg.L;
    const bool seg_interior = inside || sg.s == 1;
    const int tsf = sg.s == 1 ? (int)sg.ts : sg.cin;
    const __amdgpu_buffer_rsrc_t a_rs = __builtin_amdgcn_make_buffer_rsrc((void*)(sg.x + (long long)b * sg.bs), 0,
                                                                             (int)(((long long)(sg.L - 1) * sg.ts + sg.cin) * 4), 0x00020000);
    const int R = BM + (sg.J - 1) * sg.dil;
    int a_boff[A_SLOTS];
    const int a_lds0 = (tid / (KC / 4)) * T6_PITCH + 4 * (tid % (KC / 4));
    const bool last_slot_ok = (tid + (A_SLOTS - 1) * NT) / (KC / 4) < Cfg::A_ROWS;
    unsigned a_zero = 0;
#pragma unroll
    for (int i = 0; i < A_SLOTS; ++i) {
        const int e = tid + i * NT;
        const int row = e / (KC / 4), q = e % (KC / 4);
        long long t = (long long)(m0 + (row < R ? row : 0)) * sg.s - sg.pad;
        if (!inside) {
            if (sg.s == 1) {
                const long long jj = row < R ? src_index(sg, (int)t) : 0;
                if (jj < 0) a_zero |= 1u << i;
                t = jj < 0 ? 0 : jj;
            } else {
                t = 0;
            }
        }
        a_boff[i] = (int)((t * tsf + 4 * q) * 4);
    }
    __builtin_amdgcn_sched_barrier(0);
    float a_scale = 1.f, a_inv = 1.f;
    float a_rsc[RM ? A_SLOTS : 1];
    constexpr bool rowmode = RM;
    if (!RM) {
        unsigned am = am_early;
        asm volatile("" : "+v"(am));
        const int se = s16_exponent(am);
        a_scale = s16_pow2(se);
        a_inv = s16_pow2(-se);
        a_rsc[0] = a_scale;
    } else {
#pragma unroll
        for (int i = 0; i < A_SLOTS; ++i) {
            const int m = m0 + (tid + i * NT) / (KC / 4);
            a_rsc[RM ? i : 0] = s16_pow2(s16_exponent(sg.amax[m < p.M ? m : p.M - 1]));
        }
    }

    f32x16 acc[WMT][WN];
#pragma unroll
    for (int a = 0; a < WMT; ++a)
#pragma unroll
        for (int c = 0; c < WN; ++c)
#pragma unroll
            for (int r = 0; r < 16; ++r) acc[a][c][r] = 0.f;

    constexpr int A_OOB = 0x7fff0000;
    const __amdgpu_buffer_rsrc_t a_rs_null = __builtin_amdgcn_make_buffer_rsrc((void*)(sg.x + (long long)b * sg.bs), 0, 0, 0x00020000);
    auto load_a = [&](int c, bool live, f32x4 (&ra)[A_SLOTS]) {
#ifdef T8_ABL_NOALOAD
        live = false;
#endif
        const int c_ = c * KC;
        if (seg_interior || !live) {
            const int soff = __builtin_amdgcn_readfirstlane(live ? c_ * 4 : 0);
            const __amdgpu_buffer_rsrc_t rs = live ? a_rs : a_rs_null;
#pragma unroll
            for (int i = 0; i < A_SLOTS; ++i) ra[i] = bufload16(rs, a_boff[i], soff);
        } else {
            int voff[A_SLOTS];
#pragma unroll
            for (int i = 0; i < A_SLOTS; ++i) {
                const int e = tid + i * NT;
                const int row = e / (KC / 4), q = e % (KC / 4);
                const int cc = c_ + 4 * q;
                const int tp = sg.cin_shift >= 0 ? (cc >> sg.cin_shift) : (cc / sg.cin);
                const long long jj = row < R ? src_index(sg, (m0 + row) * sg.s + tp - sg.pad) : -1;
                voff[i] = jj < 0 ? A_OOB : (int)((jj * sg.ts + (cc - tp * sg.cin)) * 4);
            }
#pragma unroll
            for (int i = 0; i < A_SLOTS; ++i) ra[i] = bufload16(a_rs, voff[i], 0);
        }
    };
    auto load_slot = [&](int c, bool live, f32x4 (&ra)[A_SLOTS], int i) {
#ifdef T8_ABL_NOALOAD
        live = false;
#endif
        const int c_ = c * KC;
        if (seg_interior || !live) {
            const int soff = __builtin_amdgcn_readfirstlane(live ? c_ * 4 : 0);
            const __amdgpu_buffer_rsrc_t rs = live ? a_rs : a_rs_null;
            ra[i] = bufload16(rs, a_boff[i], soff);
        } else {
            const int e = tid + i * NT;
            const int row = e / (KC / 4), q = e % (KC / 4);
            const int cc = c_ + 4 * q;
            const int tp = sg.cin_shift >= 0 ? (cc >> sg.cin_shift) : (cc / sg.cin);
            const long long jj = row < R ? src_index(sg, (m0 + row) * sg.s + tp - sg.pad) : -1;
            ra[i] = bufload16(a_rs, jj < 0 ? A_OOB : (int)((jj * sg.ts + (cc - tp * sg.cin)) * 4), 0);
        }
    };
    auto store_slot = [&](const f32x4 (&ra)[A_SLOTS], __bf16* dst, int i) {
        if (i + 1 == A_SLOTS) asm volatile("" ::"v"(ra[i]));
#ifdef T8_ABL_NOSTORE
        return;
#endif
        if (i + 1 < A_SLOTS || last_slot_ok) {
            const f32x4 v = (a_zero & (1u << i)) ? f32x4{0.f, 0.f, 0.f, 0.f} : ra[i];
            split16_store4s(v, a_rsc[RM ? i : 0], dst, PLANE, a_lds0 + i * (NT / (KC / 4)) * T6_PITCH);
        }
    };
    auto store_a = [&](const f32x4 (&ra)[A_SLOTS], __bf16* dst) {
#pragma unroll
        for (int i = 0; i < A_SLOTS; ++i) store_slot(ra, dst, i);
    };
    const int ksteps = p.Ktot >> 4;
    const __bf16* wtile = wp + (long long)(n0 >> 5) * ksteps * 1024 + lane * 8;
    auto issue_b = [&](int c, int j, int slot) {
        const int k0 = (seg_kofs + j * seg_Cw + c * KC) >> 4;
#pragma unroll
        for (int i = 0; i < Cfg::PPW; ++i) {
            const int f = wave * Cfg::PPW + i;
            const int ks = f / (2 * NTILES), t = (f / 2) % NTILES, pl = f % 2;
            t8_glds16(wtile + ((long long)t * ksteps + k0 + ks) * 1024 + pl * 512, bs_lds + (unsigned)((slot * Cfg::B_PIECES + f) * 1024));
        }
    };

    auto issue_piece = [&](int c, int j, int slot, int i) {
        const int k0 = (seg_kofs + j * seg_Cw + c * KC) >> 4;
        const int f = wave * Cfg::PPW + i;
        const int ks = f / (2 * NTILES), t = (f / 2) % NTILES, pl = f % 2;
        t8_glds16(wtile + ((long long)t * ksteps + k0 + ks) * 1024 + pl * 512, bs_lds + (unsigned)((slot * Cfg::B_PIECES + f) * 1024));
    };

    const int a_frag = (wm * WMT * 32 + i32) * T6_PITCH + 8 * kh;
    auto compute = [&](int abuf, int jr, int slot, auto&& hook) {
        const __bf16* Ac = As0 + abuf * 2 * PLANE + a_frag + jr * T6_PITCH;
        const __bf16* Bc = Bs0 + slot * Cfg::B_SLOT + lane * 8;
        f16x8 bf[2][2][WN], af[2][2];
        auto read_b = [&](int ks, f16x8 (&dst)[2][WN]) {
#pragma unroll
            for (int c = 0; c < WN; ++c)
#pragma unroll
                for (int pl = 0; pl < 2; ++pl) dst[pl][c] = *reinterpret_cast<const f16x8*>(Bc + ((ks * NTILES + wn * WN + c) * 2 + pl) * 512);
        };
        auto read_a = [&](int ks, int a, f16x8 (&dst)[2]) {
#pragma unroll
            for (int pl = 0; pl < 2; ++pl) dst[pl] = *reinterpret_cast<const f16x8*>(Ac + pl * PLANE + a * 32 * T6_PITCH + ks * 16);
        };
        read_b(0, bf[0]);
        read_a(0, 0, af[0]);
#pragma unroll
        for (int u = 0; u < 2 * WMT; ++u) {
            const int ks = u / WMT, a = u % WMT;
            if (u + 1 < 2 * WMT) read_a((u + 1) / WMT, (u + 1) % WMT, af[(u + 1) & 1]);
            if (a == WMT - 1 && ks == 0) read_b(1, bf[1]);
#pragma unroll
            for (int c = 0; c < WN; ++c) {
#ifdef T8_ABL_NOMFMA
                asm volatile("" ::"v"(af[u & 1][0]), "v"(af[u & 1][1]), "v"(bf[ks][0][c]), "v"(bf[ks][1][c]));
#else
                f32x16 v = acc[a][c];
                v = __builtin_amdgcn_mfma_f32_32x32x16_f16(af[u & 1][1], bf[ks][0][c], v, 0, 0, 0);
                v = __builtin_amdgcn_mfma_f32_32x32x16_f16(af[u & 1][0], bf[ks][1][c], v, 0, 0, 0);
                acc[a][c] = __builtin_amdgcn_mfma_f32_32x32x16_f16(af[u & 1][0], bf[ks][0][c], v, 0, 0, 0);
#endif
            }
            hook(u);
            __builtin_amdgcn_sched_barrier(0);
            T8_USTAMP(u);
        }
    };
    auto no_hook = [](int) {};
    constexpr int UNITS = 2 * WMT;
    constexpr int SPU = (A_SLOTS + UNITS - 1) / UNITS, SU0 = UNITS - (A_SLOTS + SPU - 1) / SPU;
    auto store_hook = [&](const f32x4 (&ra)[A_SLOTS], __bf16* dst, bool st, int u) {
        if (u >= SU0 && st) {
#pragma unroll
            for (int k = 0; k < SPU; ++k)
                if ((u - SU0) * SPU + k < A_SLOTS) store_slot(ra, dst, (u - SU0) * SPU + k);
        }
    };

    auto tasks = [&](int u, bool has_next, int nc, int nj, int nslot, bool issue, int creq, f32x4 (&ra_req)[A_SLOTS], bool store, const f32x4 (&ra_st)[A_SLOTS], __bf16* dst,
                     auto issue_tag, auto store_tag) {
        constexpr bool ISSUE = decltype(issue_tag)::value, STORE = decltype(store_tag)::value;
        constexpr int NTASK = Cfg::PPW + (ISSUE ? A_SLOTS : 0) + (STORE ? A_SLOTS : 0);
        const int lo = u * NTASK / UNITS, hi = (u + 1) * NTASK / UNITS;
#pragma unroll
        for (int t = 0; t < NTASK; ++t) {
            if (t < lo || t >= hi) continue;
            if (t < Cfg::PPW) {
                if (has_next) issue_piece(nc, nj, nslot, t);
            } else if (ISSUE && t < Cfg::PPW + A_SLOTS) {
                load_slot(creq, issue, ra_req, t - Cfg::PPW);
            } else {
                if (store) store_slot(ra_st, dst, t - Cfg::PPW - (ISSUE ? A_SLOTS : 0));
            }
        }
    };

    using T = std::true_type;
    using F = std::false_type;
#pragma unroll
    for (int i = 0; i < (RM ? A_SLOTS : 1); ++i) asm volatile("" ::"v"(a_rsc[i]));
#ifdef T6_TRACE
    T6_PHASE(2);
#endif
    if constexpr (J1) {
        f32x4 raA[A_SLOTS], raB[A_SLOTS];
        issue_b(0, 0, 0);
        load_a(0, true, raA);
        load_a(1, NC > 1, raB);
        store_a(raA, As0);
        t8_wait<A_SLOTS>();
        lds_barrier();
#ifdef T6_TRACE
        T6_PHASE(6);
#endif
        auto stage = [&](int c, f32x4 (&ra_next)[A_SLOTS], f32x4 (&ra_free)[A_SLOTS]) {
            T8_STAMP(0);
            const bool st = c + 1 < NC;
            __bf16* dst = As0 + ((c + 1) & 1) * 2 * PLANE;
            if constexpr (SPREAD) {
                T8_STAMP(1);
                compute(c & 1, 0, c & 1, [&](int u) { tasks(u, c + 1 < NC, c + 1, 0, (c + 1) & 1, c + 2 < NC, c + 2, ra_free, st, ra_next, dst, T{}, T{}); });
            } else {
                if (c + 1 < NC) issue_b(c + 1, 0, (c + 1) & 1);
                load_a(c + 2, c + 2 < NC, ra_free);
                __builtin_amdgcn_sched_barrier(0);
                T8_STAMP(1);
                compute(c & 1, 0, c & 1, [&](int u) { store_hook(ra_next, dst, st, u); });
            }
            __builtin_amdgcn_sched_barrier(0);
            T8_STAMP(2);
            t8_wait<A_SLOTS>();
            T8_STAMP(3);
            lds_barrier();
            T8_STAMP(4);
#ifdef T6_TRACE
            ++t8_stage;
#endif
        };
        for (int c = 0; c < NC; c += 2) {
            stage(c, raB, raA);
            if (c + 1 < NC) stage(c + 1, raA, raB);
        }
    } else {
        f32x4 ra[A_SLOTS];
        issue_b(0, 0, 0);
        load_a(0, true, ra);
        store_a(ra, As0);
        load_a(1, NC > 1, ra);
        t8_wait<A_SLOTS>();
        lds_barrier();
#ifdef T6_TRACE
        T6_PHASE(6);
#endif
        auto stage = [&](int c, int j, auto store_tag, auto issue_tag) {
            constexpr bool STORE = decltype(store_tag)::value, ISSUE = decltype(issue_tag)::value;
            const int s = c * seg_J + j;
            int nc = c, nj = j + 1;
            if (nj == seg_J) { nj = 0; nc = c + 1; }
            T8_STAMP(0);
            if constexpr (SPREAD) {
                T8_STAMP(1);
                const bool st = c + 1 < NC;
                __bf16* dst = As0 + ((c + 1) & 1) * 2 * PLANE;
                compute(c & 1, j * rowstep, s & 1, [&](int u) { tasks(u, nc < NC, nc, nj, (s + 1) & 1, c + 2 < NC, c + 2, ra, st, ra, dst, issue_tag, store_tag); });
            } else {
            if (nc < NC) issue_b(nc, nj, (s + 1) & 1);
            if (ISSUE) load_a(c + 2, c + 2 < NC, ra);
            __builtin_amdgcn_sched_barrier(0);
            T8_STAMP(1);
            if constexpr (STORE) {
                const bool st = c + 1 < NC;
                __bf16* dst = As0 + ((c + 1) & 1) * 2 * PLANE;
                compute(c & 1, j * rowstep, s & 1, [&](int u) { store_hook(ra, dst, st, u); });
            } else {
                compute(c & 1, j * rowstep, s & 1, no_hook);
            }
            }
            __builtin_amdgcn_sched_barrier(0);
            T8_STAMP(2);
            if (ISSUE) t8_wait<A_SLOTS>(); else t8_wait<0>();
            T8_STAMP(3);
            lds_barrier();
            T8_STAMP(4);
#ifdef T6_TRACE
            ++t8_stage;
#endif
        };
        for (int c = 0; c < NC; ++c) {
            stage(c, 0, T{}, F{});
            for (int j = 1; j < seg_J - 1; ++j) stage(c, j, F{}, F{});
            stage(c, seg_J - 1, F{}, T{});
        }
    }

    tap6_epilogue<WGM, WGN, WMT, WN, HALO>(p, acc, smem, b, m0, n0, a_inv, rowmode, clk_t0, clk_r0, t6_ph);
#undef T8_STAMP
#undef T8_USTAMP
}

}
```

Measured before the change: 42260.

## Emit LSTM output as split16 planes consumed directly by tap8 GEMM

The persistent fp16 LSTM kernel can now write its ELU output pre-split into scaled hi/lo fp16 planes, using the amax slot it already computes. A new planes-in instantiation of the tap8 GEMM loads those planes straight into LDS with async global-to-LDS copies and a swizzled layout, instead of loading fp32 activations and splitting them in registers. The intent is to remove the fp32 load and split work in the consumer conv (encoder final conv, decoder first upsample). The cost is a new kernel variant, routing guards, and a dependency on matching amax slots between producer and consumer.

Result: no change. 42230 (median of 3 runs) (-0.1%).

```diff
diff --git a/audiocodecs_amd/csrc/ac_api.hip b/audiocodecs_amd/csrc/ac_api.hip
--- a/audiocodecs_amd/csrc/ac_api.hip
+++ b/audiocodecs_amd/csrc/ac_api.hip
@@ -77,6 +77,7 @@
     h->dev.tail_seg = std::max(0, num("AC_TAIL_SEG", 0));
     h->dev.front_ldspad = std::max(0, num("AC_FRONT_LDSPAD", 0));
     h->dev.lstm_fuse_in = num("AC_LSTM_FUSE_IN", 1);
+    h->dev.lstm_planes = num("AC_LSTM_PLANES", 1);
     const char* r = std::getenv("AC_RVQ");
     h->dev.rvq_exact = r && std::strcmp(r, "fp32") == 0;
     h->dev.prof_detail = num("AC_PROF_DETAIL", 0);
@@ -92,7 +93,7 @@
     struct { const char* k; int* v; } tab[] = {
         {"tap_epi_staged", &h->dev.tap_epi_staged}, {"tap_dil", &h->dev.tap_dil}, {"tap_stagger", &h->dev.tap_stagger}, {"tap_pick", &h->dev.tap_pick}, {"tap8", &h->dev.tap8}, {"tap8_form", &h->dev.tap8_form}, {"tap8_spread", &h->dev.tap8_spread},
         {"rb6_dbg", &h->dev.rb6_dbg}, {"rb_stream", &h->dev.rb_stream}, {"chain_stream", &h->dev.chain_stream}, {"rb128_stream", &h->dev.rb128_stream}, {"rb256_fused", &h->dev.rb256_fused}, {"front_seg", &h->dev.front_seg}, {"tail_seg", &h->dev.tail_seg}, {"front_ldspad", &h->dev.front_ldspad},
-        {"lstm_dbg", &h->dev.lstm_dbg}, {"lstm_fuse_in", &h->dev.lstm_fuse_in}, {"rvq_exact", &h->dev.rvq_exact}, {"prof_detail", &h->dev.prof_detail}, {"head_seq", &h->dev.head_seq}, {"attn_exact", &h->dev.attn_exact}, {"dac_unit", &h->dev.dac_unit}, {"mimi_tail", &h->dev.mimi_tail},
+        {"lstm_dbg", &h->dev.lstm_dbg}, {"lstm_fuse_in", &h->dev.lstm_fuse_in}, {"lstm_planes", &h->dev.lstm_planes}, {"rvq_exact", &h->dev.rvq_exact}, {"prof_detail", &h->dev.prof_detail}, {"head_seq", &h->dev.head_seq}, {"attn_exact", &h->dev.attn_exact}, {"dac_unit", &h->dev.dac_unit}, {"mimi_tail", &h->dev.mimi_tail},
         {"mstream_skinny", &h->dev.mstream_skinny},
     };
 #ifndef AC_DEVELOPER
diff --git a/audiocodecs_amd/csrc/core.h b/audiocodecs_amd/csrc/core.h
--- a/audiocodecs_amd/csrc/core.h
+++ b/audiocodecs_amd/csrc/core.h
@@ -58,6 +58,7 @@
     size_t persist_off = 0;
     size_t persist16_off = 0;
     size_t persist16_inv = 0;
+    size_t zero_off = 0;
     bool has_persist = false;
 };
 
@@ -216,6 +217,7 @@
         int front_ldspad = 0;
         int lstm_dbg = 0;
         int lstm_fuse_in = 1;
+        int lstm_planes = 1;
         int rvq_exact = 0;
         int prof_detail = 0;
         int attn_exact = 0;
@@ -745,6 +747,7 @@
                 const size_t mat16 = (size_t)LP_SLICES * 4 * 4 * 4 * 2 * 512;
                 lp.persist16_off = reserve((4 * mat16 + 1) / 2);
                 lp.persist16_inv = reserve((size_t)2 * 4 * D);
+                lp.zero_off = reserve(256);
                 std::vector<int> sc((size_t)2 * 4 * D);
                 const int layer_of[4] = {0, 1, 1, 0};
                 for (int l = 0; l < 2; ++l)
@@ -790,6 +793,8 @@
     int L, C;
     const unsigned* amax = nullptr;
     int amax_n = 0;
+    const void* planes = nullptr;
+    const void* pl_zero = nullptr;
 };
 
 int prof_name(ac_handle* h, const char* nm);
@@ -846,6 +851,8 @@
 
 int run_tap(ac_handle* h, hipStream_t st, TapGemmParams& p);
 
+bool tap_takes_planes(ac_handle* h, const PackedGemm& g, const Act& x, int taps, int pad , const float* y, long long y_bs, long long y_rs, bool y_elu, int B);
+
 
 struct Out {
     float* raw = nullptr;
@@ -895,7 +902,7 @@
     float *gin, *gin1, *hseq0, *hseq1, *c;
 };
 
-int lstm_fwd(ac_handle* h, hipStream_t st, const LstmPlan& lp, const Act& x, const LstmWs& ws, Out out, int B, Act2* y);
+int lstm_fwd(ac_handle* h, hipStream_t st, const LstmPlan& lp, const Act& x, const LstmWs& ws, Out out, int B, Act2* y, bool want_planes = false);
 
 int rvq_encode_fwd(ac_handle* h, hipStream_t st, const float* feats, int F, int K, long long* toks);
 
diff --git a/audiocodecs_amd/csrc/core.hip b/audiocodecs_amd/csrc/core.hip
--- a/audiocodecs_amd/csrc/core.hip
+++ b/audiocodecs_amd/csrc/core.hip
@@ -232,20 +232,34 @@
     return fail(h, AC_EINVAL, "run_tap: no instantiation of %s", r.name);
 }
 
-template <int WGM, int WGN, int WMT, int WN, bool RM, bool J1, bool SP>
+template <int WGM, int WGN, int WMT, int WN, bool RM, bool J1, bool SP, bool PL = false>
 static int launch_tap8(ac_handle* h, hipStream_t st, TapGemmParams& p, const __bf16* w6, const char* name, double flops, double bytes) {
     using Cfg = Tap8Cfg<WGM, WGN, WMT, WN>;
     p.mtiles = cdiv(p.M, Cfg::BM);
     p.ntiles = p.N / Cfg::BN;
     const long long blocks = (long long)p.B * p.mtiles * p.ntiles;
     ProfScope ps(h, st, name, flops, bytes);
-    if (int rc = ensure_lds(h, reinterpret_cast<const void*>(tap_gemm8_kernel<WGM, WGN, WMT, WN, RM, J1, SP>), Cfg::lds_bytes)) return rc;
-    hipLaunchKernelGGL((tap_gemm8_kernel<WGM, WGN, WMT, WN, RM, J1, SP>), dim3((unsigned)blocks), dim3(Cfg::NT), Cfg::lds_bytes, st, p, w6);
-    return AC_OK;
+    if (int rc = ensure_lds(h, reinterpret_cast<const void*>(tap_gemm8_kernel<WGM, WGN, WMT, WN, RM, J1, SP, PL>), Cfg::lds_bytes)) return rc;
+    hipLaunchKernelGGL((tap_gemm8_kernel<WGM, WGN, WMT, WN, RM, J1, SP, PL>), dim3((unsigned)blocks), dim3(Cfg::NT), Cfg::lds_bytes, st, p, w6);
+    return AC_OK;
+}
+
+static bool tap_route_takes_planes(const TapGemmParams& p, const TapRoute& r) {
+    const TapSeg& s = p.seg[0];
+    return r.family == TapFamily::tap8 && (r.key() == tap_key(2, 4, 4, 2) || r.key() == tap_key(4, 2, 2, 2)) && !r.rowmode && p.nseg == 1 && s.s == 1 &&
+           s.dil == 1 && s.J >= 2 && s.J <= 8 && s.cin % KC == 0 && s.cin * 2 <= 1024  && s.ts == s.cin &&
+           s.bs == (long long)s.L * s.cin && !s.rel_len && !s.elu;
 }
 
 static int launch_tap8_family(ac_handle* h, hipStream_t st, TapGemmParams& p, const TapRoute& r, const __bf16* w6, const char* name, double flops, double bytes) {
     constexpr int RJ = TK_RM | TK_J1, J = TK_J1, S = TK_SPREAD;
+    if (p.seg[0].pl) {
+        switch (r.key()) {
+        case tap_key(2, 4, 4, 2): return launch_tap8<2, 4, 4, 2, false, false, false, true>(h, st, p, w6, name, flops, bytes);
+        case tap_key(4, 2, 2, 2): return launch_tap8<4, 2, 2, 2, false, false, false, true>(h, st, p, w6, name, flops, bytes);
+        }
+        return fail(h, AC_EINVAL, "run_tap: no planes-in instantiation of %s", r.name);
+    }
     switch (r.key()) {
     case tap_key(2, 4, 4, 2, RJ): return launch_tap8<2, 4, 4, 2, true, true, false>(h, st, p, w6, name, flops, bytes);
     case tap_key(2, 4, 4, 2, RJ | S): return launch_tap8<2, 4, 4, 2, true, true, true>(h, st, p, w6, name, flops, bytes);
@@ -275,6 +289,9 @@
     g.x = x.p;
     g.amax = x.amax;
     g.amax_n = x.amax_n;
+    g.pl = x.planes;
+    g.pl_zero = x.pl_zero;
+    g.pl_amax = x.planes ? x.amax : nullptr;
     g.bs = x.bs;
     g.ts = x.ts;
     g.rel_len = rel_len;
@@ -309,6 +326,9 @@
     in.gemm_fp32 = h->gemm_fp32;
     const TapRoute r = route_tap(p, in, h->dev);
     if (r.reject_taps) return fail(h, AC_EINVAL, "conv with %d taps exceeds the kernel limit of 8", r.reject_taps);
+    for (int i = 0; i < p.nseg; ++i)
+        if (p.seg[i].pl && !(in.winv && tap_route_takes_planes(p, r) && p.seg[i].pl_zero && aligned16(p.seg[i].pl)))
+            return fail(h, AC_ESTATE, "run_tap: %s cannot read a tensor its producer left as split16 planes", r.name);
     double kk = 0, inb = 0;
     for (int i = 0; i < p.nseg; ++i) {
         kk += (double)p.seg[i].J * p.seg[i].s * p.seg[i].cin;
@@ -353,8 +373,10 @@
         } else if (in.winv) {
             for (int i = 0; i < p.nseg; ++i) {
                 TapSeg& sg = p.seg[i];
+                if (sg.pl && !(sg.amax && sg.amax_n == p.B)) return fail(h, AC_ESTATE, "run_tap: planes without their producer's amax slot");
                 sg.amax = amax_of(h, st, sg.x, sg.bs, sg.ts, sg.L, sg.cin, p.B, sg.amax_n == p.B ? sg.amax : nullptr);
                 if (!sg.amax) return fail(h, AC_ESTATE, "out of amax slots (split16.h)");
+                if (sg.pl && sg.amax != sg.pl_amax) return fail(h, AC_ESTATE, "run_tap: the planes were scaled by another amax slot than the segment's");
             }
             p.winv = h->blob + iv->second;
             p.amax_out = amax_new(h);
@@ -368,6 +390,28 @@
     if (rc) return rc;
     HIPCHK(h, hipGetLastError());
     return AC_OK;
+}
+
+
+bool tap_takes_planes(ac_handle* h, const PackedGemm& g, const Act& x, int taps, int pad , const float* y, long long y_bs, long long y_rs, bool y_elu, int B) {
+    if (h->gemm_fp32 || h->noncausal) return false;
+    TapGemmParams p{};
+    p.nseg = 1;
+    p.seg[0] = make_seg(x, 1, taps, pad, 0, 0, nullptr);
+    p.w = h->blob + g.w_off;
+    p.y = const_cast<float*>(y);
+    p.y_elu = y_elu ? const_cast<float*>(y) : nullptr;
+    p.y_bs = y_bs;
+    p.y_rs = y_rs;
+    p.B = B;
+    p.M = x.L;
+    p.N = g.N;
+    p.Ktot = g.Ktot;
+    TapRouteInputs in;
+    in.w6 = h->w6_of.count((size_t)(p.w - h->blob)) != 0;
+    in.winv = h->winv_of.count((size_t)(p.w - h->blob)) != 0;
+    const TapRoute r = route_tap(p, in, h->dev);
+    return !r.reject_taps && in.winv && tap_route_takes_planes(p, r);
 }
 
 
@@ -409,6 +453,7 @@
              long long out_bs, long long out_rs, int B, Act2* y) {
     const int M = cdiv(x.L, s);
     const int extra = M * s - x.L;
+    if (x.planes && (s != 1 || rel_len)) return fail(h, AC_ESTATE, "conv_fwd: a strided conv cannot read split16 planes");
     if (s == 2 && k == 4 && !rel_len && extra == 0 && x.L >= 4 && out_rs == 64 && out_bs == (long long)M * 64 && !h->noncausal) {
         const unsigned* am = nullptr;
         const int rc = try_thin6(h, st, g, x, 32, 1, out, B, &am);
@@ -451,6 +496,7 @@
 
 int convtr_fwd(ac_handle* h, hipStream_t st, const PackedGemm& g, const Act& x, int s, Out out, int B, Act2* y) {
     const int cout = g.N / s;
+    if (x.planes && s == 2) return fail(h, AC_ESTATE, "convtr_fwd: the x2 layer (thin_conv6.h) cannot read split16 planes");
     if (s == 2) {
         const unsigned* am = nullptr;
         const int rc = try_thin6(h, st, g, x, 64, 0, out, B, &am);
@@ -937,7 +983,7 @@
 }
 
 
-int lstm_fwd(ac_handle* h, hipStream_t st, const LstmPlan& lp, const Act& x, const LstmWs& ws, Out out, int B, Act2* y) {
+int lstm_fwd(ac_handle* h, hipStream_t st, const LstmPlan& lp, const Act& x, const LstmWs& ws, Out out, int B, Act2* y, bool want_planes) {
     const int D = lp.D, T = x.L, L = lp.layers;
     if (D % 64 != 0 || D > 512) return fail(h, AC_EINVAL, "LSTM width %d unsupported (need 64, 128, 256 or 512)", D);
     if (L < 1 || L > 2) return fail(h, AC_EINVAL, "%d LSTM layers unsupported (1 or 2)", L);
@@ -971,6 +1017,8 @@
             x_amax = amax_of(h, st, x.p, x.bs, x.ts, x.L, x.C, B, x.amax_n == B ? x.amax : nullptr);
             if (!x_amax) return fail(h, AC_ESTATE, "out of amax slots (split16.h)");
         }
+        const unsigned* am = amax_plus(h, st, x, 1.0f, B);
+        const bool planes = want_planes && h->dev.lstm_planes != 0 && !h->gemm_fp32 && am && out.elu && aligned16(out.elu) && lp.zero_off != 0;
         int* poison = reinterpret_cast<int*>(ws.c);
         if (!h->gemm_fp32) HIPCHK(h, hipMemsetAsync(poison, 0x7f, (size_t)B * sizeof(int), st));
         ProfScope ps(h, st, h->gemm_fp32 ? "lstm_persist_kernel" : fuse_in ? "lstm_persist16_kernel<true>" : "lstm_persist16_kernel<false>", 2.0 * T * (double)B * 4 * D * D * (nroles + (fuse_in ? 1 : 0)),
@@ -981,7 +1029,8 @@
             tp.sticky = h->sticky_dev;
             tp.poison = pz;
             tp.yout = out.raw;
-            tp.yout_elu = out.elu;
+            tp.yout_elu = planes ? nullptr : out.elu;
+            tp.yout_planes = planes ? reinterpret_cast<_Float16*>(out.elu) : nullptr;
             tp.y_bs = (long long)T * D;
             tp.clip0 = c0;
             tp.B = nb;
@@ -1021,6 +1070,11 @@
                 q6.fuse_in = fuse_in ? 1 : 0;
                 q6.poison = poison;
                 q6.hseq0_local = ws.gin1;
+                if (planes) {
+                    q6.base.yout_elu = nullptr;
+                    q6.yout_planes = reinterpret_cast<_Float16*>(out.elu);
+                    q6.amax_y = am;
+                }
                 HIPCHK(h, hipMemsetAsync(h->lp_ctl, 0, LP_CTL_WORDS * sizeof(unsigned), st));
                 const size_t hbytes = (size_t)T * (size_t)q6.base.h_ts;
                 const size_t rbytes = (size_t)std::min(T, LP16_RING) * (size_t)q6.base.h_ts;
@@ -1056,9 +1110,12 @@
             tail(c0, q.B, nullptr);
         }
         HIPCHK(h, hipGetLastError());
-        const unsigned* am = amax_plus(h, st, x, 1.0f, B);
         y->raw = Act{out.raw, (long long)T * D, D, T, D, am, B};
         y->elu = Act{out.elu, (long long)T * D, D, T, D, am, B};
+        if (planes) {
+            y->elu.planes = out.elu;
+            y->elu.pl_zero = h->blob + lp.zero_off;
+        }
         return AC_OK;
     }
     {
@@ -1340,7 +1397,12 @@
         x = y;
         capture(h, st, x.raw, B);
     }
-    rc = lstm_fwd(h, st, h->enc_lstm, x.raw, ws.lstm, Out{dbg ? ws.take() : nullptr, ws.take()}, B, &y);
+    {
+        const int Tl = x.raw.L, Dl = h->enc_lstm.D;
+        const Act ye{nullptr, (long long)Tl * Dl, Dl, Tl, Dl, nullptr, 0};
+        const bool pl = tap_takes_planes(h, h->enc_final, ye, c.last_kernel_size, PAD_REFLECT, feats, (long long)Tl * c.hidden_size, c.hidden_size, false, B);
+        rc = lstm_fwd(h, st, h->enc_lstm, x.raw, ws.lstm, Out{dbg ? ws.take() : nullptr, ws.take()}, B, &y, pl);
+    }
     if (rc) return rc;
     ws.give(x);
     if (dbg) { capture(h, st, y.raw, B); ws.give(y.raw.p); y.raw.p = nullptr; }
@@ -1364,7 +1426,13 @@
     if (rc) return rc;
     ws.give(zb);
     capture(h, st, x.raw, B);
-    rc = lstm_fwd(h, st, h->dec_lstm, x.raw, ws.lstm, Out{dbg ? ws.take() : nullptr, ws.take()}, B, &y);
+    {
+        const int Dl = h->dec_lstm.D;
+        const Act ye{nullptr, (long long)N * Dl, Dl, N, Dl, nullptr, 0};
+        const bool pl = c.num_ratios > 1 && c.upsampling_ratios[0] != 2 &&
+                        tap_takes_planes(h, h->dec_up[0], ye, 2, PAD_ZERO, ws.act[0], (long long)N * h->dec_up[0].N, h->dec_up[0].N, true, B);
+        rc = lstm_fwd(h, st, h->dec_lstm, x.raw, ws.lstm, Out{dbg ? ws.take() : nullptr, ws.take()}, B, &y, pl);
+    }
     if (rc) return rc;
     ws.give(x);
     if (dbg) { capture(h, st, y.raw, B); ws.give(y.raw.p); y.raw.p = nullptr; }
diff --git a/audiocodecs_amd/csrc/lstm_persist.h b/audiocodecs_amd/csrc/lstm_persist.h
--- a/audiocodecs_amd/csrc/lstm_persist.h
+++ b/audiocodecs_amd/csrc/lstm_persist.h
@@ -47,6 +47,7 @@
     const int* poison;
     float* yout;
     float* yout_elu;
+    _Float16* yout_planes;
     long long y_bs;
     int clip0, B, T, D;
     int xcds_used;
@@ -80,6 +81,11 @@
     for (long long i = (long long)blockIdx.y * 256 + threadIdx.x; i < n; i += 256LL * gridDim.y) {
         if (p.yout) p.yout[o + i] = nan;
         if (p.yout_elu) p.yout_elu[o + i] = nan;
+        if (p.yout_planes) {
+            const _Float16 hnan = __builtin_bit_cast(_Float16, (unsigned short)0x7e00u);
+            p.yout_planes[o + i + (long long)(p.clip0 + b) * p.y_bs] = hnan;
+            p.yout_planes[o + i + (long long)(p.clip0 + b + 1) * p.y_bs] = hnan;
+        }
     }
 }
 
diff --git a/audiocodecs_amd/csrc/lstm_persist16.h b/audiocodecs_amd/csrc/lstm_persist16.h
--- a/audiocodecs_amd/csrc/lstm_persist16.h
+++ b/audiocodecs_amd/csrc/lstm_persist16.h
@@ -23,6 +23,8 @@
     const float* winv;
     const unsigned* amax_x;
     void* hseq0_local;
+    _Float16* yout_planes;
+    const unsigned* amax_y;
 };
 
 #ifndef LP16_HEXP
@@ -136,6 +138,8 @@
 #pragma unroll
     for (int q = 0; q < 4; ++q) wiv[q] = LP16_HINV * pp.winv[layer * 4 * D + q * D + eu];
     const int hpos = ec * 32 + ej * 2;
+    float ysc = 1.f;
+    if (layer == 1 && pp.yout_planes) ysc = s16_pow2(s16_exponent(*amax_at(pp.amax_y, live ? (int)erow : p.clip0)));
 
     auto load_a = [&](const char* seq, int t, bf16x8 (&a)[2][2]) {
         const char* src = seq + (long long)t * p.h_ts + goff + (long long)(wave * 4) * SLICE_BYTES;
@@ -343,7 +347,16 @@
                 const float yv = hn + skipv;
                 const long long o = erow * p.y_bs + (long long)t * D + eu;
                 if (p.yout) p.yout[o] = yv;
-                if (p.yout_elu) p.yout_elu[o] = elu1(yv);
+                if (pp.yout_planes) {
+                    const float e = elu1(yv);
+                    const _Float16 hi = (_Float16)(e * ysc);
+                    const _Float16 lo = (_Float16)__builtin_fmaf(e, ysc, -(float)hi);
+                    _Float16* d = pp.yout_planes + 2 * erow * p.y_bs + (long long)t * D + eu;
+                    d[0] = hi;
+                    d[p.y_bs] = lo;
+                } else if (p.yout_elu) {
+                    p.yout_elu[o] = elu1(yv);
+                }
             }
             const int t1 = t + 1 < p.T ? t + 1 : t;
             if (!ap_ok && !load_valid(h0b, t1, ap)) return false;
diff --git a/audiocodecs_amd/csrc/tap_gemm.h b/audiocodecs_amd/csrc/tap_gemm.h
--- a/audiocodecs_amd/csrc/tap_gemm.h
+++ b/audiocodecs_amd/csrc/tap_gemm.h
@@ -25,6 +25,9 @@
     int dil;
     const unsigned* amax;
     int amax_n;
+    const void* pl;
+    const void* pl_zero;
+    const unsigned* pl_amax;
 };
 
 struct TapGemmParams {
diff --git a/audiocodecs_amd/csrc/tap_gemm8.h b/audiocodecs_amd/csrc/tap_gemm8.h
--- a/audiocodecs_amd/csrc/tap_gemm8.h
+++ b/audiocodecs_amd/csrc/tap_gemm8.h
@@ -34,10 +34,13 @@
     asm volatile("s_waitcnt vmcnt(%0)" ::"n"(N) : "memory");
 }
 
-template <int WGM, int WGN, int WMT, int WN, bool RM, bool J1, bool SPREAD = true>
+constexpr int T8_PL_GROUPS = 20, T8_PL_APW = 2 * T8_PL_GROUPS / 8;
+template <int WGM, int WGN, int WMT, int WN, bool RM, bool J1, bool SPREAD = true, bool PL = false>
 __global__ __launch_bounds__(512, 1) void tap_gemm8_kernel(const TapGemmParams p, const __bf16* __restrict__ wp) {
     using Cfg = Tap8Cfg<WGM, WGN, WMT, WN>;
     constexpr int BM = Cfg::BM, BN = Cfg::BN, NT = Cfg::NT, A_SLOTS = Cfg::A_SLOTS, PLANE = Cfg::PLANE, NTILES = Cfg::NTILES;
+    static_assert(!PL || (!RM && !J1 && !SPREAD), "planes: several taps, one scale per clip, the weight requests at the top of the stage");
+    static_assert(!PL || (T8_PL_GROUPS * 16 >= Cfg::A_ROWS && T8_PL_GROUPS * 16 * 32 <= PLANE && (PLANE * 2) % 16 == 0), "planes: the row groups cover the slab and stay inside a plane");
     constexpr int HALO = 7;
     unsigned long long clk_t0 = 0, clk_r0 = 0;
     if (p.clk) { clk_t0 = __builtin_amdgcn_s_memtime(); clk_r0 = __builtin_amdgcn_s_memrealtime(); }
@@ -106,6 +109,20 @@
         }
         a_boff[i] = (int)((t * tsf + 4 * q) * 4);
     }
+    const char* a_src[PL ? T8_PL_APW : 1];
+    const unsigned as_lds = (unsigned)(size_t)As0;
+    const unsigned a_dst0 = as_lds + (unsigned)((wave >> 2) * PLANE * 2 + (wave & 3) * T8_PL_APW * 1024);
+    if constexpr (PL) {
+        const char* pbase = reinterpret_cast<const char*>(sg.pl) + (long long)b * sg.bs * 4 + (long long)(wave >> 2) * sg.L * sg.cin * 2;
+#pragma unroll
+        for (int i = 0; i < T8_PL_APW; ++i) {
+            const int row = ((wave & 3) * T8_PL_APW + i) * 16 + (lane >> 2);
+            const int col = (lane & 3) ^ ((row >> 2) & 3);
+            const long long t = (long long)m0 + row - sg.pad;
+            const long long jj = row < R ? (inside ? t : src_index(sg, (int)t)) : -1;
+            a_src[i] = jj < 0 ? reinterpret_cast<const char*>(sg.pl_zero) + col * 16 : pbase + (jj * sg.cin + col * 8) * 2;
+        }
+    }
     __builtin_amdgcn_sched_barrier(0);
     float a_scale = 1.f, a_inv = 1.f;
     float a_rsc[RM ? A_SLOTS : 1];
@@ -211,9 +228,12 @@
         t8_glds16(wtile + ((long long)t * ksteps + k0 + ks) * 1024 + pl * 512, bs_lds + (unsigned)((slot * Cfg::B_PIECES + f) * 1024));
     };
 
-    const int a_frag = (wm * WMT * 32 + i32) * T6_PITCH + 8 * kh;
+    auto issue_a = [&](int c, int abuf, int i) { t8_glds16(a_src[PL ? i : 0] + c * (KC * 2), a_dst0 + (unsigned)(abuf * 2 * PLANE * 2 + i * 1024)); };
+
+    const int a_frag = PL ? (wm * WMT * 32 + i32) * KC : (wm * WMT * 32 + i32) * T6_PITCH + 8 * kh;
     auto compute = [&](int abuf, int jr, int slot, auto&& hook) {
-        const __bf16* Ac = As0 + abuf * 2 * PLANE + a_frag + jr * T6_PITCH;
+        const __bf16* Ac = As0 + abuf * 2 * PLANE + a_frag + jr * (PL ? KC : T6_PITCH);
+        const int pl_c0 = (kh ^ (((i32 + jr) >> 2) & 3)) * 8;
         const __bf16* Bc = Bs0 + slot * Cfg::B_SLOT + lane * 8;
         f16x8 bf[2][2][WN], af[2][2];
         auto read_b = [&](int ks, f16x8 (&dst)[2][WN]) {
@@ -224,7 +244,9 @@
         };
         auto read_a = [&](int ks, int a, f16x8 (&dst)[2]) {
 #pragma unroll
-            for (int pl = 0; pl < 2; ++pl) dst[pl] = *reinterpret_cast<const f16x8*>(Ac + pl * PLANE + a * 32 * T6_PITCH + ks * 16);
+            for (int pl = 0; pl < 2; ++pl)
+                dst[pl] = PL ? *reinterpret_cast<const f16x8*>(Ac + pl * PLANE + a * 32 * KC + (pl_c0 ^ (ks * 16)))
+                             : *reinterpret_cast<const f16x8*>(Ac + pl * PLANE + a * 32 * T6_PITCH + ks * 16);
         };
         read_b(0, bf[0]);
         read_a(0, 0, af[0]);
@@ -323,6 +345,49 @@
         for (int c = 0; c < NC; c += 2) {
             stage(c, raB, raA);
             if (c + 1 < NC) stage(c + 1, raA, raB);
+        }
+    } else if constexpr (PL) {
+        issue_b(0, 0, 0);
+#pragma unroll
+        for (int i = 0; i < T8_PL_APW; ++i) issue_a(0, 0, i);
+        t8_wait<0>();
+        lds_barrier();
+#ifdef T6_TRACE
+        T6_PHASE(6);
+#endif
+        auto stage = [&](int c, int j, auto areq_tag) {
+            constexpr bool AREQ = decltype(areq_tag)::value;
+            const int s = c * seg_J + j;
+            int nc = c, nj = j + 1;
+            if (nj == seg_J) { nj = 0; nc = c + 1; }
+            T8_STAMP(0);
+            if (nc < NC) issue_b(nc, nj, (s + 1) & 1);
+            const int ca = c + 1 < NC ? c + 1 : 0;
+            __builtin_amdgcn_sched_barrier(0);
+            T8_STAMP(1);
+            if (AREQ) {
+                compute(c & 1, j * rowstep, s & 1, [&](int u) {
+#pragma unroll
+                    for (int i = 0; i < T8_PL_APW; ++i)
+                        if (i * UNITS / T8_PL_APW == u) issue_a(ca, (c + 1) & 1, i);
+                });
+            } else {
+                compute(c & 1, j * rowstep, s & 1, no_hook);
+            }
+            __builtin_amdgcn_sched_barrier(0);
+            T8_STAMP(2);
+            if (AREQ) t8_wait<T8_PL_APW>(); else t8_wait<0>();
+            T8_STAMP(3);
+            lds_barrier();
+            T8_STAMP(4);
+#ifdef T6_TRACE
+            ++t8_stage;
+#endif
+        };
+        for (int c = 0; c < NC; ++c) {
+            for (int j = 0; j < seg_J - 2; ++j) stage(c, j, F{});
+            stage(c, seg_J - 2, T{});
+            stage(c, seg_J - 1, F{});
         }
     } else {
         f32x4 ra[A_SLOTS];
```
